# mmdagent/distantspeechrecognition-mirror

Measured on AMD Instinct MI355X. Metric: decoded_audio_hours_per_sec, higher is better.
Workload: dtype f32

## Files before the change

distantspeechrecognition-mirror_amd/csrc/decode_plan.h:

```cpp
#pragma once
#include <algorithm>
#include <cmath>
#include <cstddef>
#include <cstdlib>
#include <cstring>

namespace dsr {

struct VitEnv {
  int slots = 0;
  bool noFast = false;
  int seg = 125;
  double segSaveGB = 16.0;
  int segAny = 0;
  int segDrop = 0;
  bool segVerbose = false;
  bool pen = false;
  bool prof = false;
  bool noHash = false;
  bool noCnt = false;
  bool tableWide = false;
};

inline VitEnv read_vit_env()
{
  VitEnv e; const char* v;
  if ((v = getenv("DSR_VITERBI_SLOTS"))) e.slots = atoi(v);
  e.noFast = getenv("DSR_VITERBI_NOFAST") != nullptr;
  if ((v = getenv("DSR_VITERBI_SEG"))) e.seg = atoi(v);
  if ((v = getenv("DSR_VITERBI_SEG_SAVE_GB"))) e.segSaveGB = atof(v);
  if ((v = getenv("DSR_VITERBI_SEG_ANY"))) e.segAny = atoi(v) == 2 ? 2 : 1;
  if ((v = getenv("DSR_VITERBI_SEG_DROP"))) e.segDrop = (int) strtol(v, nullptr, 0);
  e.segVerbose = getenv("DSR_VITERBI_SEG_VERBOSE") != nullptr;
  e.pen = getenv("DSR_VITERBI_PEN") != nullptr;
  e.prof = getenv("DSR_VITERBI_PROF") != nullptr;
  e.noHash = getenv("DSR_VITERBI_NOHASH") != nullptr;
  e.noCnt = getenv("DSR_VITERBI_NOCNT") != nullptr;
  e.tableWide = (v = getenv("DSR_VITERBI_TABLE")) && !strcmp(v, "wide");
  return e;
}

struct PlanIn {
  int streams, maxActive; long long arenaTokens, latticeTokens; int topN; bool dumpOn;
  int nNodes, maxCnt;
  int U, Tmax, nDist;
  size_t staticLds;
};

struct DecodePlan {
  int slots, segFrames, segQueues, segCount, poolArenas; long arenaPer; int useLdsRow, hashN, cntCap, modes; size_t ldsBytes; bool narrow;
};

static constexpr size_t kPlanSideBytes = (size_t) 496 * 32;

inline int plan_base_modes(const PlanIn& in, const VitEnv& env) { return (env.prof ? 1 : 0) | ((in.latticeTokens > 0 || in.topN > 0 || in.dumpOn) ? 2 : 0); }

template <class RoundRobin> DecodePlan plan_decode(const PlanIn& in, const VitEnv& env, RoundRobin&& roundRobin)
{
  DecodePlan p;
  const int U = in.U, Tmax = in.Tmax, nDist = in.nDist;
  int slots = in.streams; if (slots > U) slots = U; if (in.dumpOn) slots = 1;
  const bool latOn = in.latticeTokens > 0;
  int segFrames = 0;
  if (!latOn && !in.dumpOn && in.topN <= 0 && U > slots) {
    segFrames = env.seg;
    if (segFrames < 0 || 2 * segFrames > Tmax + 1) segFrames = 0;
    const double saveGB = (double) U * (double) in.maxActive * 24.0 / 1e9;
    if (saveGB > env.segSaveGB) segFrames = 0;
  }
  int segQueues = 8;
  if (segFrames > 0 && !(slots >= 64 && slots % 8 == 0 && roundRobin())) { if (env.segAny) segQueues = 1; else segFrames = 0; }
  if (segFrames > 0 && env.segAny == 2) segQueues = 1;
  const long arenaPer = in.arenaTokens > 0 ? (long) in.arenaTokens : (long) 8192 * (long) (Tmax + 2);
  int poolArenas = 0;
  if (segFrames > 0) {
    const double want = (double) U * 1536.0 * (double) (Tmax + 2) / (double) arenaPer;
    poolArenas = (int) std::min<double>(std::ceil(want), (double) (0xFFFFFFF0u / (unsigned long long) arenaPer));
    if ((unsigned long long) std::max(poolArenas, slots) * (unsigned long long) arenaPer > 0xFFFFFFF0ull) segFrames = 0;
  }
  p.slots = slots; p.segFrames = segFrames; p.segQueues = segQueues; p.poolArenas = poolArenas; p.arenaPer = arenaPer;
  p.segCount = segFrames > 0 ? (Tmax + segFrames) / segFrames : 1;
  int modes = plan_base_modes(in, env);
  const size_t eoffB = kPlanSideBytes; const size_t ldsCap = (size_t) 160 * 1024 - in.staticLds;
  const int hashMax = 16384;
  int useLds = (size_t) nDist * sizeof(float) <= 64 * 1024;
  if (useLds && (size_t) ((nDist + 3) & ~3) * sizeof(float) + (size_t) hashMax * 8 + eoffB > ldsCap) useLds = 0;
  const size_t rowB = useLds ? (size_t) ((nDist + 3) & ~3) * sizeof(float) : 16;
  int hashN = hashMax; while (hashN > 0 && rowB + (size_t) hashN * 8 + eoffB > ldsCap) hashN >>= 1;
  if (env.noHash) hashN = 0;
  int cntCap = (hashN > 0 && in.maxCnt < 65536 && rowB + (size_t) hashN * 8 + eoffB + 4096 <= ldsCap) ? 2048 : 0;
  if (env.noCnt) cntCap = 0;
  p.ldsBytes = rowB + (size_t) hashN * 8 + eoffB + 2 * (size_t) cntCap;
  p.narrow = in.nNodes <= 65535 && hashN == hashMax && !env.tableWide;
  if (p.narrow) modes |= 4;
  p.useLdsRow = useLds; p.hashN = hashN; p.cntCap = cntCap; p.modes = modes;
  return p;
}

}
```

distantspeechrecognition-mirror_amd/csrc/decoder.cpp:

```cpp
#include "common.h"
#include "wfst_graph.h"
#include "lattice.h"
#include "lexicon.h"
#include "wordtrace.h"
#include "viterbi.h"
#include "decode_plan.h"
#include <algorithm>
#include <cmath>

namespace dsr {

static_assert(kPlanSideBytes == (size_t) kSideLds * sizeof(Side), "decode_plan.h budgets the side records of viterbi.h");

struct DecoderState {
  dsr_decoder_cfg cfg; bool haveGraph = false; int nSlots = 0; int nNodes = 0;
  WfstGraph::Csr csr; WfstGraph::Tables tab;
  DevBuf<int> d_xoff, d_xarc, d_xpathOff, d_eoff, d_path, d_nodeFinal, d_queue; DevBuf<float> d_pathCost;
  DevBuf<XRec> d_xrec; DevBuf<ERec> d_erec; DevBuf<float> d_arcCost, d_nodeCost; DevBuf<uint32_t> d_arcOut, d_arcIn;
  DevBuf<TokA> d_tokA, d_ctok; DevBuf<TokB> d_tokB; DevBuf<Side> d_side; DevBuf<XRecD> d_xrecD; DevBuf<XRecC> d_xrecC; double recLmScale = 0.0;  int fastOK = 0; int maxCnt = 0; DevBuf<int> d_tokOff, d_tokCnt, d_owner, d_rank, d_chead; DevBuf<unsigned> d_tags; DevBuf<CandA> d_cA; DevBuf<CandB> d_cB; DevBuf<unsigned> d_first; DevBuf<Bp> d_arena;
  DevBuf<long long> d_prof; DevBuf<dsr_decode_result> d_res; DevBuf<int> d_arcs; DevBuf<unsigned> d_words;
  long arenaCap = 0; int initial = 0; unsigned tokenMemoryLimit = 0;
  long lastPoolCap = 0;
  hipEvent_t evTrace = nullptr;
  DevBuf<TraceHead> d_heads; DevBuf<int> d_hopRec, d_hopOff;
  DevBuf<SegState> d_segState; DevBuf<int> d_segDone; DevBuf<unsigned long long> d_poolNext; DevBuf<TokA> d_saveA; DevBuf<TokB> d_saveB;
  DevBuf<WTok> w_tok; DevBuf<WCand> w_cand; DevBuf<int> w_tokOff, w_rank; DevBuf<unsigned long long> w_best; DevBuf<unsigned> w_first; DevBuf<int4> w_traces; size_t w_tablesFor = 0;
  bool costNegZero = false; double costMinAbs = HUGE_VAL;
  DevBuf<uint4> d_lat; DevBuf<double> d_latTtl; DevBuf<long> d_latFrameOff; DevBuf<int> d_arenaLat; DevBuf<int4> d_latFinal; DevBuf<int> d_latInfo;
  int latU = 0, latTmax = 0; long latArenaCap = 0; WfstGraph graphCopy; DevBuf<TokA> d_tokA3; DevBuf<TokB> d_tokB3;
  const dsr_lexicon* lexIn = nullptr; const dsr_lexicon* lexOut = nullptr; uint32_t eosX = 0; std::string eosSymbol;
  int lastU = 0; size_t lastMaxPath = 0; bool lastPaths = false;
  PinBuf<dsr_decode_result> h_res; PinBuf<int> h_arcs; PinBuf<unsigned> h_words; hipEvent_t evDone = nullptr;
  int pendingU = 0; size_t pendingPath = 0; int pendingSlots = 0; long long* pendingProf = nullptr;
  int dumpOn = 0; long dumpCap = 0; DevBuf<long> d_dumpFrameOff, d_dumpCount; DevBuf<int> d_dumpNode, d_dumpArc; DevBuf<float> d_dumpAc, d_dumpLm;
  std::vector<int64_t> h_dumpFrameOff; std::vector<int32_t> h_dumpNode, h_dumpArc; std::vector<float> h_dumpAc, h_dumpLm; int64_t h_dumpFrames = 0;
};

}

using namespace dsr;
struct dsr_decoder : DecoderState {};

extern "C" {

void dsr_decoder_default_cfg(dsr_decoder_cfg* c)
{ memset(c, 0, sizeof(*c)); c->beam = 100.0; c->lmScale = 12.0; c->lmPenalty = 0.0; c->silPenalty = 0.0; c->silenceX = 0xFFFFFFFFu;
  c->propagateN = 5; c->wordTraceLattice = 1; }

dsr_status dsr_decoder_create(const dsr_decoder_cfg* cfg, dsr_decoder** out)
{
  return guard([&] {
    if (!cfg || !out) throw Error(DSR_E_PARAMETER, "null argument");
    require_device();
    dsr_decoder* d = new dsr_decoder(); d->cfg = *cfg;
    if (d->cfg.maxActive <= 0) d->cfg.maxActive = 65536;
    if (d->cfg.maxCandidates <= 0) d->cfg.maxCandidates = 8 * d->cfg.maxActive;
    if (d->cfg.maxCandidates >= (1 << 24)) throw Error(DSR_E_PARAMETER, "maxCandidates must be < 2^24");
    if (d->cfg.streams <= 0) {
      hipDeviceProp_t prop; int dev = 0; DSR_HIP(hipGetDevice(&dev)); DSR_HIP(hipGetDeviceProperties(&prop, dev));
      d->cfg.streams = prop.multiProcessorCount;
      const int t = read_vit_env().slots; if (t > 0) d->cfg.streams = t;
    }
    *out = d;
  });
}
namespace {
std::mutex g_traceMu; std::map<int, std::pair<const dsr_decoder*, hipEvent_t>> g_lastTrace; std::map<int, int> g_cuCount;
void order_behind_last_traceback(int slots, hipStream_t st)
{
  std::lock_guard<std::mutex> lock(g_traceMu);
  int dev = 0; DSR_HIP(hipGetDevice(&dev));
  auto cu = g_cuCount.find(dev);
  if (cu == g_cuCount.end()) { int n = 0; DSR_HIP(hipDeviceGetAttribute(&n, hipDeviceAttributeMultiprocessorCount, dev)); cu = g_cuCount.emplace(dev, n).first; }
  if (slots < cu->second) return;
  const auto it = g_lastTrace.find(dev);
  if (it != g_lastTrace.end()) DSR_HIP(hipStreamWaitEvent(st, it->second.second, 0));
}
void publish_traceback(dsr_decoder* d, hipStream_t st)
{
  std::lock_guard<std::mutex> lock(g_traceMu);
  if (!d->evTrace) DSR_HIP(hipEventCreateWithFlags(&d->evTrace, hipEventDisableTiming));
  DSR_HIP(hipEventRecord(d->evTrace, st));
  int dev = 0; DSR_HIP(hipGetDevice(&dev));
  g_lastTrace[dev] = std::make_pair((const dsr_decoder*) d, d->evTrace);
}
void forget_traceback(const dsr_decoder* d)
{
  std::lock_guard<std::mutex> lock(g_traceMu);
  for (auto it = g_lastTrace.begin(); it != g_lastTrace.end(); ) { if (it->second.first == d) it = g_lastTrace.erase(it); else ++it; }
}
}

void dsr_decoder_destroy(dsr_decoder* d)
{
  if (!d) return;
  forget_traceback(d);
  if (d->evDone) (void) hipEventDestroy(d->evDone);
  if (d->evTrace) (void) hipEventDestroy(d->evTrace);
  delete d;
}

dsr_status dsr_decoder_set(dsr_decoder* d, const dsr_wfst* g)
{
  return guard([&] {
    if (!d || !g) throw Error(DSR_E_PARAMETER, "null argument");
    if (g->initial < 0) throw Error(DSR_E_CONSISTENCY, "the transducer has no arcs");
    d->csr = g->csr(); d->tab = g->tables(d->csr, (size_t) 1 << 28);
    d->nNodes = (int) g->nodes.size(); d->initial = g->initial; d->graphCopy = *g;
    std::vector<int> nf(d->nNodes); std::vector<float> nc(d->nNodes);
    for (int i = 0; i < d->nNodes; i++) { nf[i] = g->nodes[i].final_; nc[i] = g->nodes[i].cost; }
    d->d_xoff.upload(d->tab.xoff); d->d_eoff.upload(d->tab.eoff); d->d_path.upload(d->tab.path);
    if (d->tab.xrec.empty()) throw Error(DSR_E_CONSISTENCY, "the transducer has no emitting arcs");
    d->d_xrec.upload(d->tab.xrec); d->d_xarc.upload(d->tab.xarc); d->d_xpathOff.upload(d->tab.xpathOff);
    {
      const size_t nx = d->tab.xrec.size(); std::vector<XRecD> xd(nx); std::vector<XRecC> xc(nx); int maxCnt = 0; std::vector<float> pc(1, 0.0f);
      const double lmS = d->cfg.lmScale; d->recLmScale = lmS;
      for (size_t r = 0; r < nx; r++) {
        const XRec& x = d->tab.xrec[r]; XRecD& o = xd[r]; XRecC& oc = xc[r];
        o.dst = x.dst; o.dist = x.dist; o.lmCost = lmS * (double) x.cost; o.meta = x.meta;
        oc.dst = x.dst; oc.dstXoff = d->tab.xoff[x.dst]; oc.dstCnt = d->tab.xoff[x.dst + 1] - d->tab.xoff[x.dst]; oc.pad = 0;
        const int po = d->tab.xpathOff[r], plen = (int) (x.meta & 0xFFFFu); o.p2 = 0; float eps1 = 0.0f;
        if (x.meta >> 18) throw Error(DSR_E_CONSISTENCY, "expansion record %zu: meta bits above 17 are in use", r);
        if (plen) { const int a0 = d->tab.path[po]; eps1 = d->csr.cost[a0]; if (d->csr.out[a0] != 0) o.meta |= 0x20000u; }
        o.lmEps1 = lmS * (double) eps1;
        if (plen > 14) o.meta |= 0x80000000u;
        else if (plen > 1) {
          if (plen == 2) { const float c1 = d->csr.cost[d->tab.path[po + 1]]; memcpy(&o.p2, &c1, 4); }
          else { o.p2 = (int) pc.size(); for (int h = 1; h < plen; h++) pc.push_back(d->csr.cost[d->tab.path[po + h]]); }
          for (int h = 1; h < plen; h++) if (d->csr.out[d->tab.path[po + h]] != 0) o.meta |= 1u << (17 + h);
        }
        if (oc.dstCnt > maxCnt) maxCnt = oc.dstCnt;
      }
      d->d_xrecD.upload(xd); d->d_xrecC.upload(xc); d->d_pathCost.upload(pc);
      d->fastOK = (maxCnt < (1 << 19) && nx < ((size_t) 1 << 27)) ? 1 : 0; d->maxCnt = maxCnt;
      if (read_vit_env().noFast) d->fastOK = 0;
    }
    { std::vector<ERec> e = d->tab.erec; if (e.empty()) e.push_back(ERec{0, 0, 0, 0}); d->d_erec.upload(e); }
    d->d_arcCost.upload(d->csr.cost); d->d_arcOut.upload(d->csr.out); d->d_arcIn.upload(d->csr.in);
    d->costNegZero = false; d->costMinAbs = HUGE_VAL;
    for (size_t a = 0; a < d->csr.cost.size(); a++) {
      const float c = d->csr.cost[a]; uint32_t bits; memcpy(&bits, &c, 4);
      if (bits == 0x80000000u) d->costNegZero = true;
      if (c != 0.0f && std::fabs((double) c) < d->costMinAbs) d->costMinAbs = std::fabs((double) c);
    }
    d->d_nodeFinal.upload(nf); d->d_nodeCost.upload(nc);
    d->haveGraph = true; d->nSlots = 0;
  });
}
dsr_status dsr_decoder_set_symbols(dsr_decoder* d, const dsr_wfst* g, const char* silSymbol, const char* eosSymbol)
{
  return guard([&] {
    if (!d || !g) throw Error(DSR_E_PARAMETER, "null argument");
    uint32_t silX = d->cfg.silenceX, eosX = 0;
    if (silSymbol) { if (!g->lexIn) throw Error(DSR_E_KEY, "the transducer has no input lexicon to look '%s' up in", silSymbol); silX = g->lexIn->index(silSymbol); }
    if (eosSymbol) { if (!g->lexOut) throw Error(DSR_E_KEY, "the transducer has no output lexicon to look '%s' up in", eosSymbol); eosX = g->lexOut->index(eosSymbol); }
    const dsr_status s = dsr_decoder_set(d, g);
    if (s != DSR_OK) throw Error(s, "%s", dsr_last_error());
    d->cfg.silenceX = silX; d->eosX = eosX; d->lexIn = g->lexIn; d->lexOut = g->lexOut; d->eosSymbol = eosSymbol ? eosSymbol : "";
  });
}
uint32_t dsr_decoder_eos_index(const dsr_decoder* d) { return d ? d->eosX : 0; }

static void need_last(const dsr_decoder* d, int u, bool paths)
{
  if (!d) throw Error(DSR_E_PARAMETER, "null argument");
  if (d->lastU <= 0) throw Error(DSR_E_CONSISTENCY, "no decode has been collected yet");
  if (u < 0 || u >= d->lastU) throw Error(DSR_E_INDEX, "utterance %d of %d", u, d->lastU);
  if (paths && !d->lastPaths) throw Error(DSR_E_CONSISTENCY, "the last decode was collected without its paths");
  if (d->h_res.p[u].status != DSR_OK) throw Error(d->h_res.p[u].status, "utterance %d was not decoded (status %d)", u, d->h_res.p[u].status);
}
static std::vector<uint32_t> path_ids(const dsr_decoder* d, int u, int which)
{
  need_last(d, u, true);
  const dsr_decode_result& r = d->h_res.p[u];
  const int n = r.nArcs < (int) d->lastMaxPath ? r.nArcs : (int) d->lastMaxPath;
  const int* arcs = d->h_arcs.p + (size_t) u * d->lastMaxPath;
  std::vector<uint32_t> ids;
  if (which == 1) {
    uint32_t lastX = 0;
    for (int i = n - 1; i >= 0; i--) { const uint32_t inX = d->csr.in[arcs[i]]; if (inX != 0 && inX != lastX) { ids.push_back(inX); lastX = inX; } }
    std::reverse(ids.begin(), ids.end());
  } else for (int i = 0; i < n; i++) { const uint32_t v = which == 0 ? d->csr.out[arcs[i]] : d->csr.in[arcs[i]]; if (v != 0) ids.push_back(v); }
  return ids;
}
dsr_status dsr_decoder_path_ids(const dsr_decoder* d, int u, int which, uint32_t* ids, int cap, int* n)
{
  return guard([&] {
    if (!n || which < 0 || which > 2) throw Error(DSR_E_PARAMETER, "bad argument");
    const std::vector<uint32_t> v = path_ids(d, u, which);
    *n = (int) v.size();
    if (ids) { if ((int) v.size() > cap) throw Error(DSR_E_DIMENSION, "buffer holds %d ids, the path has %zu", cap, v.size()); if (!v.empty()) memcpy(ids, v.data(), 4 * v.size()); }
  });
}
static void put_string(const std::string& s, char* buf, size_t cap, size_t* need)
{
  if (need) *need = s.size() + 1;
  if (buf) { if (s.size() + 1 > cap) throw Error(DSR_E_DIMENSION, "buffer holds %zu bytes, the string needs %zu", cap, s.size() + 1); memcpy(buf, s.c_str(), s.size() + 1); }
}
dsr_status dsr_decoder_best_hypo(const dsr_decoder* d, int u, int useInputSymbols, char* buf, size_t cap, size_t* need)
{
  return guard([&] {
    const std::vector<uint32_t> v = path_ids(d, u, useInputSymbols ? 1 : 0);
    const dsr_lexicon* lex = useInputSymbols ? d->lexIn : d->lexOut;
    if (!lex) throw Error(DSR_E_KEY, "the transducer set on this decoder has no %s lexicon", useInputSymbols ? "input" : "output");
    std::string s; for (size_t i = 0; i < v.size(); i++) { s += lex->symbol(v[i]); s += " "; }
    put_string(s, buf, cap, need);
  });
}
dsr_status dsr_decoder_best_path(const dsr_decoder* d, int u, char* buf, size_t cap, size_t* need, int* count)
{
  return guard([&] {
    const std::vector<uint32_t> v = path_ids(d, u, 2);
    if (!d->lexIn) throw Error(DSR_E_KEY, "the transducer set on this decoder has no input lexicon");
    std::string s; for (size_t i = 0; i < v.size(); i++) { s += d->lexIn->symbol(v[i]); s += "\n"; }
    if (count) *count = (int) v.size();
    put_string(s, buf, cap, need);
  });
}
dsr_status dsr_decoder_final_states_n(const dsr_decoder* d, int u, int* n)
{ return guard([&] { if (!n) throw Error(DSR_E_PARAMETER, "null argument"); need_last(d, u, false); *n = d->h_res.p[u].finalStatesN; }); }
dsr_status dsr_decoder_trace_back_succeeded(const dsr_decoder* d, int u, int* ok)
{ return guard([&] { if (!ok) throw Error(DSR_E_PARAMETER, "null argument"); need_last(d, u, false); *ok = d->h_res.p[u].reachedFinal; }); }

dsr_status dsr_decoder_set_token_memory_limit(dsr_decoder* d, unsigned limit)
{ return guard([&] { if (!d) throw Error(DSR_E_PARAMETER, "null argument"); d->tokenMemoryLimit = limit; }); }
unsigned dsr_decoder_token_memory_limit(const dsr_decoder* d) { return d ? d->tokenMemoryLimit : 0u; }

dsr_status dsr_decoder_set_beam(dsr_decoder* d, double beam) { return guard([&] { if (!d) throw Error(DSR_E_PARAMETER, "null argument"); d->cfg.beam = beam; }); }

dsr_status dsr_decoder_enable_dump(dsr_decoder* d, int en) { return guard([&] { if (!d) throw Error(DSR_E_PARAMETER, "null argument"); d->dumpOn = en; }); }

static bool xcd_round_robin(hipStream_t st)
{
  static std::mutex mu; static std::map<int, bool> known;
  std::lock_guard<std::mutex> lock(mu);
  int dev = 0; DSR_HIP(hipGetDevice(&dev));
  const auto it = known.find(dev); if (it != known.end()) return it->second;
  DevBuf<int> o; o.reserve(64); int h[64];
  xcc_probe_launch(o.p, st);
  DSR_HIP(hipMemcpyAsync(h, o.p, sizeof(h), hipMemcpyDeviceToHost, st)); DSR_HIP(hipStreamSynchronize(st));
  bool ok = true; unsigned seen = 0;
  for (int i = 0; i < 64; i++) { if (h[i] < 0 || h[i] > 7 || h[i] != h[i & 7]) ok = false; }
  for (int i = 0; i < 8 && ok; i++) seen |= 1u << h[i];
  return known[dev] = ok && seen == 0xFFu;
}

static void ensure_scratch(dsr_decoder* d, int slots, int Tmax, int arenas)
{
  const dsr_decoder_cfg& c = d->cfg;
  long arena = c.arenaTokens > 0 ? (long) c.arenaTokens : (long) 8192 * (long) (Tmax + 2);
  if (arena > 0x7FFFFFF0L) arena = 0x7FFFFFF0L;
  if (slots <= d->nSlots && arena <= d->arenaCap && (size_t) (arenas > slots ? arenas : slots) * (size_t) d->arenaCap <= d->d_arena.n) return;
  if (slots < d->nSlots) slots = d->nSlots;
  if (arena < d->arenaCap) arena = d->arenaCap;
  const size_t S = (size_t) slots;
  d->d_tokA.reserve(S * 2 * c.maxActive); d->d_tokB.reserve(S * 2 * c.maxActive); d->d_ctok.reserve(S * 8192); d->d_side.reserve(S * kFastC);
  d->d_tokOff.reserve(S * (c.maxActive + 1));
  d->d_owner.reserve(S * c.maxCandidates); d->d_rank.reserve(S * c.maxCandidates);
  d->d_cA.reserve(S * c.maxCandidates); d->d_cB.reserve(S * c.maxCandidates);
  d->d_first.reserve(S * d->nNodes); d->d_tokCnt.reserve(S * (c.maxActive + 1)); d->d_chead.reserve(S * c.maxCandidates);
  d->d_tags.reserve(S); DSR_HIP(hipMemset(d->d_tags.p, 0, S * sizeof(unsigned)));
  d->d_arena.reserve((size_t) (arenas > slots ? arenas : slots) * (size_t) arena);
  d->d_queue.reserve(8);
  d->nSlots = slots; d->arenaCap = arena;
}

static void check_arc_inputs(const dsr_decoder* d, int nDist)
{ for (size_t a = 0; a < d->csr.in.size(); a++) if (d->csr.in[a] > (uint32_t) nDist) throw Error(DSR_E_INDEX, "arc input %u has no distribution (nDist=%d)", d->csr.in[a], nDist); }

static void enqueue_result_copies(dsr_decoder* d, int U, size_t nPath, hipStream_t st)
{
  d->h_res.reserve(U); d->h_arcs.reserve(nPath ? nPath : 1); d->h_words.reserve(nPath ? nPath : 1);
  DSR_HIP(hipMemcpyAsync(d->h_res.p, d->d_res.p, sizeof(dsr_decode_result) * U, hipMemcpyDeviceToHost, st));
  if (nPath) DSR_HIP(hipMemcpyAsync(d->h_arcs.p, d->d_arcs.p, sizeof(int) * nPath, hipMemcpyDeviceToHost, st));
  if (nPath) DSR_HIP(hipMemcpyAsync(d->h_words.p, d->d_words.p, sizeof(unsigned) * nPath, hipMemcpyDeviceToHost, st));
  if (!d->evDone) DSR_HIP(hipEventCreateWithFlags(&d->evDone, hipEventDisableTiming));
  DSR_HIP(hipEventRecord(d->evDone, st));
  d->pendingU = U; d->pendingPath = nPath;
}

static void launch_wordtrace(dsr_decoder* d, const float* score, const int32_t* nframes, int U, int Tmax, int nDist, int maxPath, int want_paths, hipStream_t st)
{
  if (d->cfg.wordTraceLattice) throw Error(DSR_E_CONSISTENCY, "DecoderWordTrace with generateLattice: not built (the shipped _placeOnList dereferences the null word trace of "
                                           "every token that has not crossed a word boundary, decoder.cc:239); construct it with generateLattice = false");
  if (d->cfg.topN > 0 || d->cfg.latticeTokens > 0 || d->dumpOn) throw Error(DSR_E_PARAMETER, "DecoderWordTrace: no topN (its frame loop has no such branch, decoder.cc:147-183), lattice bookkeeping or dump");
  check_arc_inputs(d, nDist);
  int slots = d->cfg.streams; if (slots > U) slots = U;
  const dsr_decoder_cfg& c = d->cfg; const size_t S = (size_t) slots;
  const long maxTraces = c.wordTraces > 0 ? (long) c.wordTraces : (long) 1 << 20;
  d->w_tok.reserve(S * 2 * c.maxActive); d->w_cand.reserve(S * c.maxCandidates); d->w_tokOff.reserve(S * (c.maxActive + 1)); d->w_rank.reserve(S * c.maxCandidates);
  d->w_traces.reserve((size_t) U * maxTraces); d->d_queue.reserve(8); d->d_res.reserve(U);
  if (d->w_tablesFor != S * d->nNodes) {
    d->w_best.reserve(S * d->nNodes); d->w_first.reserve(S * d->nNodes); d->w_tablesFor = S * d->nNodes;
    DSR_HIP(hipMemsetAsync(d->w_best.p, 0xFF, sizeof(unsigned long long) * S * d->nNodes, st)); DSR_HIP(hipMemsetAsync(d->w_first.p, 0xFF, sizeof(unsigned) * S * d->nNodes, st));
  }
  if (maxPath < 1) maxPath = 1;
  d->d_arcs.reserve((size_t) U * maxPath); d->d_words.reserve((size_t) U * maxPath);
  DSR_HIP(hipMemsetAsync(d->d_queue.p, 0, 8 * sizeof(int), st));
  WtArgs A; A.nNodes = d->nNodes; A.initial = d->initial; A.xoff = d->d_xoff.p; A.xrec = d->d_xrec.p; A.xarc = d->d_xarc.p; A.xpathOff = d->d_xpathOff.p; A.eoff = d->d_eoff.p;
  A.erec = d->d_erec.p; A.path = d->d_path.p; A.arcCost = d->d_arcCost.p; A.arcOut = d->d_arcOut.p; A.arcIn = d->d_arcIn.p; A.nodeFinal = d->d_nodeFinal.p; A.nodeCost = d->d_nodeCost.p;
  A.beam = c.beam; A.lmScale = c.lmScale; A.lmPenalty = c.lmPenalty; A.silPenalty = c.silPenalty; A.silenceX = c.silenceX; A.insertSilence = c.insertSilence;
  A.maxTok = c.maxActive; A.maxCand = c.maxCandidates; A.maxTraces = maxTraces;
  A.tok = d->w_tok.p; A.cand = d->w_cand.p; A.tokOff = d->w_tokOff.p; A.rank = d->w_rank.p; A.bestKey = d->w_best.p; A.firstSlot = d->w_first.p; A.traces = d->w_traces.p; A.queue = d->d_queue.p;
  A.scores = score; A.nframes = nframes; A.U = U; A.Tmax = Tmax; A.nDist = nDist; A.res = d->d_res.p; A.arcsOut = d->d_arcs.p; A.wordsOut = d->d_words.p; A.maxPath = maxPath;
  wordtrace_launch(A, slots, st);
  enqueue_result_copies(d, U, want_paths ? (size_t) U * maxPath : 0, st);
  d->pendingSlots = slots; d->pendingProf = nullptr; d->latU = 0;
}

static VitArgs fill_vit_args(dsr_decoder* d, const DecodePlan& P, const VitEnv& env, const float* score, const int32_t* nframes, int U, int Tmax, int nDist,
                             int maxPath, bool wantPaths, hipStream_t st)
{
  const int slots = P.slots; const bool latOn = d->cfg.latticeTokens > 0;
  d->d_res.reserve(U);
  if (wantPaths) { d->d_arcs.reserve((size_t) U * (maxPath > 0 ? maxPath : 1)); d->d_words.reserve((size_t) U * (maxPath > 0 ? maxPath : 1)); }
  DSR_HIP(hipMemsetAsync(d->d_queue.p, 0, 8 * sizeof(int), st));
  d->d_heads.reserve(U); DSR_HIP(hipMemsetAsync(d->d_heads.p, 0xFF, sizeof(TraceHead) * (size_t) U, st));
  if (d->dumpOn) {
    d->dumpCap = (long) d->cfg.maxActive * 64 < (long) 1 << 26 ? (long) 1 << 24 : (long) 1 << 26;
    d->d_dumpFrameOff.reserve(Tmax + 2); d->d_dumpCount.reserve(2);
    d->d_dumpNode.reserve(d->dumpCap); d->d_dumpArc.reserve(d->dumpCap); d->d_dumpAc.reserve(d->dumpCap); d->d_dumpLm.reserve(d->dumpCap);
    DSR_HIP(hipMemsetAsync(d->d_dumpCount.p, 0, 2 * sizeof(long), st));
  }
  VitArgs A; GraphDev& G = A.G; DecDev& D = A.D;
  G.nNodes = d->nNodes; G.initial = d->initial; G.xoff = d->d_xoff.p; G.xrec = d->d_xrec.p; G.xrecD = d->d_xrecD.p; G.xrecC = d->d_xrecC.p; G.xarc = d->d_xarc.p;
  G.xpathOff = d->d_xpathOff.p; G.eoff = d->d_eoff.p; G.erec = d->d_erec.p; G.path = d->d_path.p; G.pathCost = d->d_pathCost.p; G.arcCost = d->d_arcCost.p;
  G.arcOut = d->d_arcOut.p; G.arcIn = d->d_arcIn.p; G.nodeFinal = d->d_nodeFinal.p; G.nodeCost = d->d_nodeCost.p;
  if (memcmp(&d->recLmScale, &d->cfg.lmScale, sizeof(double)) != 0) throw Error(DSR_E_CONSISTENCY, "lmScale changed after the transducer was set");
  D.beam = d->cfg.beam; D.lmScale = d->cfg.lmScale; D.lmPenalty = d->cfg.lmPenalty; D.silPenalty = d->cfg.silPenalty;
  D.noPen = (d->cfg.lmScale > 0.0 && std::isfinite(d->cfg.lmScale) && d->cfg.lmScale * d->cfg.lmPenalty == 0.0 && d->cfg.lmScale * d->cfg.silPenalty == 0.0 &&
             !d->costNegZero && (d->costMinAbs == HUGE_VAL || d->cfg.lmScale * d->costMinAbs >= 0x1p-60) && !env.pen) ? 1 : 0;
  D.silenceX = d->cfg.silenceX; D.maxTok = d->cfg.maxActive; D.maxCand = d->cfg.maxCandidates; D.arenaCap = d->arenaCap;
  D.tokA = d->d_tokA.p; D.tokB = d->d_tokB.p; D.ctok = d->d_ctok.p; D.side = d->d_side.p; D.fastOK = d->fastOK; D.tokOff = d->d_tokOff.p; D.owner = d->d_owner.p; D.rank = d->d_rank.p; D.cA = d->d_cA.p; D.cB = d->d_cB.p;
  D.first = d->d_first.p; D.tags = d->d_tags.p; D.tokCnt = d->d_tokCnt.p; D.chead = d->d_chead.p; D.arena = d->d_arena.p; D.queue = d->d_queue.p;
  D.segDrop = env.segDrop; D.segQueues = P.segQueues; D.segFrames = P.segFrames; D.segCount = P.segCount;
  D.poolCap = 0; D.poolChunk = 0; D.poolNext = nullptr; D.segState = nullptr; D.segDone = nullptr; D.saveA = nullptr; D.saveB = nullptr;
  if (P.segFrames > 0) {
    d->d_segState.reserve(U); d->d_segDone.reserve(U); d->d_poolNext.reserve(1);
    d->d_saveA.reserve((size_t) U * d->cfg.maxActive); d->d_saveB.reserve((size_t) U * d->cfg.maxActive);
    DSR_HIP(hipMemsetAsync(d->d_segDone.p, 0, sizeof(int) * (size_t) U, st)); DSR_HIP(hipMemsetAsync(d->d_poolNext.p, 0, sizeof(unsigned long long), st));
    D.poolCap = (long) ((size_t) std::max(P.poolArenas, slots) * (size_t) d->arenaCap); if (D.poolCap > (long) 0xFFFFFFF0L) D.poolCap = (long) 0xFFFFFFF0L;
    D.poolChunk = std::min<long>(262144, std::max<long>(4096, D.poolCap / (4 * (long) U)));
    D.poolNext = d->d_poolNext.p; D.segState = d->d_segState.p; D.segDone = d->d_segDone.p; D.saveA = d->d_saveA.p; D.saveB = d->d_saveB.p;
  }
  d->lastPoolCap = D.poolCap;
  D.prof = nullptr;
  if (env.prof) { d->d_prof.reserve((size_t) slots * kProfN); D.prof = d->d_prof.p; }
  D.dumpOn = d->dumpOn; D.dumpCap = d->dumpCap; D.dumpFrameOff = d->d_dumpFrameOff.p; D.dumpNode = d->d_dumpNode.p; D.dumpAc = d->d_dumpAc.p;
  D.dumpLm = d->d_dumpLm.p; D.dumpArc = d->d_dumpArc.p; D.dumpCount = d->d_dumpCount.p;
  D.topN = d->cfg.topN > 0 ? d->cfg.topN : 0; D.tokA3 = nullptr; D.tokB3 = nullptr;
  if (D.topN > 0) { d->d_tokA3.reserve((size_t) slots * d->cfg.maxActive); d->d_tokB3.reserve((size_t) slots * d->cfg.maxActive); D.tokA3 = d->d_tokA3.p; D.tokB3 = d->d_tokB3.p; }
  D.latOn = latOn ? 1 : 0; D.latCap = 0; D.lat = nullptr; D.latTtl = nullptr; D.latFrameOff = nullptr; D.arenaLat = nullptr; D.latFinal = nullptr; D.latInfo = nullptr;
  if (latOn) {
    const size_t cap = (size_t) d->cfg.latticeTokens;
    d->d_lat.reserve((size_t) U * cap); d->d_latTtl.reserve((size_t) U * cap); d->d_latFrameOff.reserve((size_t) U * (Tmax + 3));
    d->d_arenaLat.reserve((size_t) U * (size_t) d->arenaCap); d->d_latFinal.reserve((size_t) U * d->cfg.maxActive); d->d_latInfo.reserve((size_t) 4 * U);
    DSR_HIP(hipMemsetAsync(d->d_latInfo.p, 0, sizeof(int) * 4 * (size_t) U, st));
    D.latCap = (long) cap; D.lat = d->d_lat.p; D.latTtl = d->d_latTtl.p; D.latFrameOff = d->d_latFrameOff.p; D.arenaLat = d->d_arenaLat.p; D.latFinal = d->d_latFinal.p; D.latInfo = d->d_latInfo.p;
    d->latU = U; d->latTmax = Tmax; d->latArenaCap = d->arenaCap;
  } else d->latU = 0;
  A.scores = score; A.nframesArr = nframes; A.U = U; A.Tmax = Tmax; A.nDist = nDist; A.res = d->d_res.p;
  A.arcsOut = wantPaths ? d->d_arcs.p : nullptr; A.wordsOut = wantPaths ? d->d_words.p : nullptr; A.maxPath = maxPath;
  A.useLdsRow = P.useLdsRow; A.hashN = P.hashN; A.regionB = (int) (kSideLds * sizeof(Side)); A.cntCap = P.cntCap;
  A.heads = d->d_heads.p;
  A.hopStride = std::max(1, std::min(2 * D.maxCand, Tmax + 2));
  d->d_hopRec.reserve((size_t) U * A.hopStride); d->d_hopOff.reserve((size_t) U * A.hopStride); A.hopRec = d->d_hopRec.p;
  A.oneEach = (P.segFrames == 0 && slots == U) ? 1 : 0;
  A.walkHere = (P.segFrames == 0 && !latOn && !A.oneEach) ? 1 : 0;
  return A;
}

static TraceArgs fill_trace_args(dsr_decoder* d, const VitArgs& V)
{
  TraceArgs A; A.hopCap = 2 * V.D.maxCand; A.hopStride = V.hopStride;
  A.heads = V.heads; A.arena = V.D.arena; A.arenaN = (unsigned long long) d->d_arena.n;
  A.xrec = V.G.xrec; A.erec = V.G.erec; A.xarc = V.G.xarc; A.xpathOff = V.G.xpathOff; A.path = V.G.path; A.arcOut = V.G.arcOut;
  A.hopRec = d->d_hopRec.p; A.hopOff = d->d_hopOff.p;
  A.res = V.res; A.arcsOut = V.arcsOut; A.wordsOut = V.wordsOut; A.maxPath = V.maxPath; A.U = V.U;
  return A;
}

dsr_status dsr_decoder_decode_launch(dsr_decoder* d, const float* score, const int32_t* nframes, int U, int Tmax, int nDist,
                                     int maxPath, int want_paths, void* stream)
{
  return guard([&] {
    if (!d || !score || !nframes) throw Error(DSR_E_PARAMETER, "null argument");
    if (!d->haveGraph) throw Error(DSR_E_INITIALIZATION, "call set() with a transducer first");
    if (d->pendingU > 0) throw Error(DSR_E_CONSISTENCY, "a decode is already in flight on this decoder: collect it first");
    if (U <= 0) return;
    hipStream_t st = (hipStream_t) stream;
    if (d->cfg.wordTrace) { launch_wordtrace(d, score, nframes, U, Tmax, nDist, maxPath, want_paths, st); return; }
    check_arc_inputs(d, nDist);
    const bool latOn = d->cfg.latticeTokens > 0;
    if (latOn && d->dumpOn) throw Error(DSR_E_PARAMETER, "lattice bookkeeping and the token dump are separate debugging aids: enable one");
    const VitEnv env = read_vit_env();
    PlanIn in; in.streams = d->cfg.streams; in.maxActive = d->cfg.maxActive; in.arenaTokens = d->cfg.arenaTokens; in.latticeTokens = d->cfg.latticeTokens;
    in.topN = d->cfg.topN; in.dumpOn = d->dumpOn != 0; in.nNodes = d->nNodes; in.maxCnt = d->maxCnt; in.U = U; in.Tmax = Tmax; in.nDist = nDist;
    in.staticLds = viterbi_static_lds(plan_base_modes(in, env));
    const DecodePlan P = plan_decode(in, env, [&] { return xcd_round_robin(st); });
    ensure_scratch(d, P.slots, Tmax, latOn ? U : (P.segFrames > 0 ? P.poolArenas : 0));
    if (maxPath < 0) maxPath = 0;
    const VitArgs A = fill_vit_args(d, P, env, score, nframes, U, Tmax, nDist, maxPath, want_paths != 0, st);
    if (env.segVerbose) fprintf(stderr, "[dsr viterbi] %d utterances on %d workgroups: %s, %s state table\n", U, P.slots, P.segFrames > 0 ? (P.segQueues == 8 ? "time-sliced, XCD-bound queues" : "time-sliced, one queue") : "run to completion", P.narrow ? "narrow" : "wide");
    const TraceArgs TA = fill_trace_args(d, A);
    order_behind_last_traceback(P.slots, st);
    viterbi_launch(P.modes, A, P.slots, P.ldsBytes, st);
    traceback_launch(TA, st);
    publish_traceback(d, st);
    enqueue_result_copies(d, U, want_paths ? (size_t) U * maxPath : 0, st);
    d->pendingSlots = P.slots; d->pendingProf = A.D.prof;
  });
}

static void report_profile(const long long* prof, int slots)
{
  std::vector<long long> hp((size_t) slots * kProfN); DSR_HIP(hipMemcpy(hp.data(), prof, hp.size() * sizeof(long long), hipMemcpyDeviceToHost));
  double acc[32] = {0}; for (int s2 = 0; s2 < slots; s2++) for (int i = 0; i < 32; i++) acc[i] += (double) hp[(size_t) s2 * kProfN + i];
  fprintf(stderr, "[dsr viterbi prof] mean us per slot:");
  for (int i = 0; i < 32; i++) if (i != 15) fprintf(stderr, " p%d=%.0f", i, acc[i] / slots / 100.0);
  fprintf(stderr, "\n");
  double tmin = 1e30, tmax = 0.0, tsum = 0.0;
  for (int s2 = 0; s2 < slots; s2++) { double t = 0.0; for (int i = 0; i < 32; i++) if (i != 15) t += (double) hp[(size_t) s2 * kProfN + i]; t /= 100.0; tsum += t; if (t < tmin) tmin = t; if (t > tmax) tmax = t; }
  {
    double h[12] = {0}; for (int s2 = 0; s2 < slots; s2++) for (int i = 0; i < 12; i++) h[i] += (double) hp[(size_t) s2 * kProfN + 32 + i];
    const double nf = h[0] + h[1] + h[2] + h[3], tk = h[4] + h[5] + h[6] + h[7];
    static const char* const cn[4] = {"<=8192", "<=12288", ">12288", "memory path"};
    for (int c = 0; c < 4; c++) if (h[c] > 0) fprintf(stderr, "[dsr viterbi prof] frames with %s placements: %.1f %% of the frames, %.1f %% of the frame time, %.1f us per frame, %.2f ns per placement\n",
                                                      cn[c], 100.0 * h[c] / nf, 100.0 * h[4 + c] / tk, h[4 + c] / 100.0 / h[c], h[4 + c] * 10.0 / h[8 + c]);
  }
  {
    double a = 0, b = 0; for (int s2 = 0; s2 < slots; s2++) { a += (double) hp[(size_t) s2 * kProfN + 44]; b += (double) hp[(size_t) s2 * kProfN + 45]; }
    if (a + b > 0) fprintf(stderr, "[dsr viterbi prof] register-path frames: %.1f %% start laid out, %.1f %% run P1/P2\n", 100.0 * a / (a + b), 100.0 * b / (a + b));
    double m1 = 0, m2 = 0, mAll = 0; for (int s2 = 0; s2 < slots; s2++) { m1 += (double) hp[(size_t) s2 * kProfN + 46]; m2 += (double) hp[(size_t) s2 * kProfN + 47]; mAll += (double) hp[(size_t) s2 * kProfN + 32 + 3]; }
    if (mAll > 0) fprintf(stderr, "[dsr viterbi prof] memory-path frames: %.0f, of them %.1f %% with at most 28672 placements, %.1f %% with at most 32767\n", mAll, 100.0 * m1 / mAll, 100.0 * m2 / mAll);
  }
  {
    double h[6] = {0}; for (int s2 = 0; s2 < slots; s2++) for (int i = 0; i < 6; i++) h[i] += (double) hp[(size_t) s2 * kProfN + 48 + i];
    if (h[0] > 0) fprintf(stderr, "[dsr viterbi prof] hops behind the first: %.0f wave-placements, %.1f %% with a path of two or more hops, %.1f %% load hop costs, %.1f %% run the hop loop; "
                                  "%.3f hop iterations per wave-placement for %.3f hops per lane (x 64: %.2f)\n",
                          h[0], 100.0 * h[1] / h[0], 100.0 * h[2] / h[0], 100.0 * h[3] / h[0], h[4] / h[0], h[5] / h[0] / 64.0, h[5] / h[0]);
  }
  fprintf(stderr, "[dsr viterbi prof] busy us per slot: mean %.0f min %.0f max %.0f\n", tsum / slots, tmin, tmax);
  if (slots >= 64 && slots % 8 == 0) {
    double bx[8] = {0}; for (int s2 = 0; s2 < slots; s2++) { double t = 0.0; for (int i = 0; i < 32; i++) if (i != 15) t += (double) hp[(size_t) s2 * kProfN + i]; bx[s2 & 7] += t / 100.0; }
    fprintf(stderr, "[dsr viterbi prof] busy us per slot, by XCD:"); for (int q = 0; q < 8; q++) fprintf(stderr, " %.0f", bx[q] / (slots / 8)); fprintf(stderr, "\n");
  }
}

dsr_status dsr_decoder_decode_collect(dsr_decoder* d, dsr_decode_result* res, int32_t* arcs_out, uint32_t* words_out)
{
  return guard([&] {
    if (!d || !res) throw Error(DSR_E_PARAMETER, "null argument");
    if (d->pendingU <= 0) throw Error(DSR_E_CONSISTENCY, "no decode in flight");
    const int U = d->pendingU; const size_t nPath = d->pendingPath; const int slots = d->pendingSlots; long long* prof = d->pendingProf;
    d->pendingU = 0; d->lastU = U; d->lastPaths = nPath > 0; d->lastMaxPath = nPath > 0 ? nPath / (size_t) U : 0;
    DSR_HIP(hipEventSynchronize(d->evDone));
    memcpy(res, d->h_res.p, sizeof(dsr_decode_result) * U);
    if (arcs_out && nPath) memcpy(arcs_out, d->h_arcs.p, sizeof(int) * nPath);
    if (words_out && nPath) memcpy(words_out, d->h_words.p, sizeof(unsigned) * nPath);
    if (read_vit_env().segVerbose && d->d_poolNext.p && d->lastPoolCap > 0) {
      unsigned long long used = 0; DSR_HIP(hipMemcpy(&used, d->d_poolNext.p, sizeof(used), hipMemcpyDeviceToHost));
      fprintf(stderr, "[dsr viterbi] pool of back-pointer records: %.1f M of %.1f M taken\n", used / 1e6, d->lastPoolCap / 1e6);
    }
    if (read_vit_env().segVerbose) {
      long long laid = 0, reg = 0, all = 0;
      for (int u = 0; u < U; u++) if (res[u].status == DSR_OK || res[u].status == DSR_E_DIMENSION) { laid += res[u].laidOutFrames_; reg += res[u].registerFrames; all += res[u].frames + 1; }
      fprintf(stderr, "[dsr viterbi] frames: %lld laid out by the frame before, %lld through P1/P2, %lld on the memory path\n", laid, reg - laid, all - reg);
    }
    if (prof) report_profile(prof, slots);
    if (d->dumpOn) {
      long cnt[2]; DSR_HIP(hipMemcpy(cnt, d->d_dumpCount.p, sizeof(cnt), hipMemcpyDeviceToHost));
      const long N = cnt[0] < d->dumpCap ? cnt[0] : d->dumpCap; d->h_dumpFrames = cnt[1];
      std::vector<long> fo(cnt[1] + 1); if (cnt[1] > 0) DSR_HIP(hipMemcpy(fo.data(), d->d_dumpFrameOff.p, sizeof(long) * (cnt[1] + 1), hipMemcpyDeviceToHost));
      d->h_dumpFrameOff.assign(fo.begin(), fo.end());
      d->h_dumpNode.resize(N); d->h_dumpArc.resize(N); d->h_dumpAc.resize(N); d->h_dumpLm.resize(N);
      if (N > 0) {
        DSR_HIP(hipMemcpy(d->h_dumpNode.data(), d->d_dumpNode.p, sizeof(int) * N, hipMemcpyDeviceToHost));
        DSR_HIP(hipMemcpy(d->h_dumpArc.data(), d->d_dumpArc.p, sizeof(int) * N, hipMemcpyDeviceToHost));
        DSR_HIP(hipMemcpy(d->h_dumpAc.data(), d->d_dumpAc.p, sizeof(float) * N, hipMemcpyDeviceToHost));
        DSR_HIP(hipMemcpy(d->h_dumpLm.data(), d->d_dumpLm.p, sizeof(float) * N, hipMemcpyDeviceToHost));
      }
    }
  });
}

dsr_status dsr_decoder_decode_batch(dsr_decoder* d, const float* score, const int32_t* nframes, int U, int Tmax, int nDist,
                                    dsr_decode_result* res, int32_t* arcs_out, uint32_t* words_out, int maxPath, void* stream)
{
  if (!res) return guard([&] { throw Error(DSR_E_PARAMETER, "null argument"); });
  if (U <= 0) return DSR_OK;
  const dsr_status s1 = dsr_decoder_decode_launch(d, score, nframes, U, Tmax, nDist, maxPath, (arcs_out || words_out) ? 1 : 0, stream);
  if (s1 != DSR_OK) return s1;
  return dsr_decoder_decode_collect(d, res, arcs_out, words_out);
}

namespace {
struct LatHost {
  std::vector<long> frameOff; std::vector<dsr::LatPlace> place; std::vector<double> ttl; std::vector<dsr::LatBp> arena; std::vector<int> arenaLat; std::vector<dsr::LatFinalTok> fin;
  dsr::LatInput in;
};
void load_lat(dsr_decoder* d, int u, uint32_t eosX, LatHost& H)
{
  if (d->latU <= 0) throw Error(DSR_E_CONSISTENCY, "Must enable lattice generation during decoding.");
  if (d->pendingU > 0) throw Error(DSR_E_CONSISTENCY, "a decode is in flight: collect it first");
  if (u < 0 || u >= d->latU) throw Error(DSR_E_INDEX, "utterance %d of %d", u, d->latU);
  int info[4]; DSR_HIP(hipMemcpy(info, d->d_latInfo.p + 4 * (size_t) u, sizeof(info), hipMemcpyDeviceToHost));
  const int finN = info[0], haveNext = info[1], T = info[3]; const long arenaN = info[2];
  if (T <= 0) throw Error(DSR_E_CONSISTENCY, "utterance %d was not decoded to its end (status of its decode result)", u);
  H.frameOff.assign((size_t) T + 2, 0);
  DSR_HIP(hipMemcpy(H.frameOff.data(), d->d_latFrameOff.p + (size_t) u * (d->latTmax + 3), sizeof(long) * ((size_t) T + 2), hipMemcpyDeviceToHost));
  const long nP = H.frameOff[(size_t) T + 1];
  H.place.resize((size_t) (nP > 0 ? nP : 1)); H.ttl.resize((size_t) (nP > 0 ? nP : 1));
  H.arena.resize((size_t) (arenaN > 0 ? arenaN : 1)); H.arenaLat.resize((size_t) (arenaN > 0 ? arenaN : 1)); H.fin.resize((size_t) (finN > 0 ? finN : 1));
  const size_t cap = (size_t) d->cfg.latticeTokens;
  if (nP > 0) { DSR_HIP(hipMemcpy(H.place.data(), d->d_lat.p + (size_t) u * cap, sizeof(LatPlace) * (size_t) nP, hipMemcpyDeviceToHost));
                DSR_HIP(hipMemcpy(H.ttl.data(), d->d_latTtl.p + (size_t) u * cap, sizeof(double) * (size_t) nP, hipMemcpyDeviceToHost)); }
  if (arenaN > 0) { DSR_HIP(hipMemcpy(H.arena.data(), d->d_arena.p + (size_t) u * (size_t) d->latArenaCap, sizeof(LatBp) * (size_t) arenaN, hipMemcpyDeviceToHost));
                    DSR_HIP(hipMemcpy(H.arenaLat.data(), d->d_arenaLat.p + (size_t) u * (size_t) d->latArenaCap, sizeof(int) * (size_t) arenaN, hipMemcpyDeviceToHost)); }
  if (finN > 0) DSR_HIP(hipMemcpy(H.fin.data(), d->d_latFinal.p + (size_t) u * d->cfg.maxActive, sizeof(LatFinalTok) * (size_t) finN, hipMemcpyDeviceToHost));
  LatInput& in = H.in; in.graph = &d->graphCopy; in.csr = &d->csr; in.tab = &d->tab; in.lmScale = d->cfg.lmScale; in.lmPenalty = d->cfg.lmPenalty; in.silPenalty = d->cfg.silPenalty;
  in.silenceX = d->cfg.silenceX; in.eosX = eosX; in.T = T; in.place = H.place.data(); in.ttl = H.ttl.data(); in.frameOff = H.frameOff.data();
  in.arena = H.arena.data(); in.arenaLat = H.arenaLat.data(); in.arenaN = arenaN; in.fin = H.fin.data(); in.finN = finN; in.haveNext = haveNext;
}
}

dsr_status dsr_decoder_lattice(dsr_decoder* d, int u, uint32_t eosX, dsr_lattice** out)
{
  return guard([&] {
    if (!d || !out) throw Error(DSR_E_PARAMETER, "null argument");
    LatHost H; load_lat(d, u, eosX, H);
    dsr_lattice* L = new dsr_lattice();
    try { build_lattice(H.in, *L); } catch (...) { delete L; throw; }
    *out = L;
  });
}

dsr_status dsr_decoder_write_gmm(dsr_decoder* d, int u, const char* conv, const char* channel, const char* spk, const char* utt, double cfrom, double score,
                                 const char* fileName, double frameInterval)
{
  return guard([&] {
    (void) spk;
    if (!d || !conv || !channel || !utt) throw Error(DSR_E_PARAMETER, "null argument");
    if (!d->lexIn) throw Error(DSR_E_KEY, "the transducer set on this decoder has no input lexicon");
    LatHost H; load_lat(d, u, 0u, H);
    std::vector<GmmRow> rows;
    if (!best_path_gmm(H.in, rows)) throw Error(DSR_E_CONSISTENCY, "no best token");
    FILE* fp = (!fileName || !*fileName) ? stdout : fopen(fileName, "a");
    if (!fp) throw Error(DSR_E_IO, "could not open %s", fileName);
    fprintf(fp, "# %s %10.4f %10.4f\n", utt, cfrom, score);
    for (int i = (int) rows.size() - 1; i >= 0; i--) {
      if (rows[i].inX >= d->lexIn->syms.size()) { if (fp != stdout) fclose(fp); throw Error(DSR_E_INDEX, "input symbol %u is not in the lexicon", rows[i].inX); }
      const std::string& lab = d->lexIn->symbol(rows[i].inX); const char* label = lab.c_str();
      if (lab == d->eosSymbol) continue;
      const double beg = cfrom + rows[i].startX * frameInterval, len = (rows[i].endX - rows[i].startX + 1) * frameInterval;
      fprintf(fp, "%s %s %7.2f %7.2f %-20s %7.2f\n", conv, channel, beg, len, label, rows[i].score);
    }
    if (fp != stdout) fclose(fp); else fflush(stdout);
  });
}
void dsr_lattice_destroy(dsr_lattice* L) { delete L; }
int dsr_lattice_num_nodes(const dsr_lattice* L) { return L ? (int) L->nodeFinal.size() : 0; }
int dsr_lattice_num_edges(const dsr_lattice* L) { return L ? (int) L->from.size() : 0; }
int dsr_lattice_final_states_n(const dsr_lattice* L) { return L ? L->finalStatesN : 0; }
dsr_status dsr_lattice_get(const dsr_lattice* L, int32_t* nodeFinal, int32_t* from, int32_t* to, uint32_t* in, uint32_t* out, int32_t* start, int32_t* end, double* ac, double* lm)
{
  return guard([&] {
    if (!L) throw Error(DSR_E_PARAMETER, "null argument");
    const size_t nE = L->from.size();
    if (nodeFinal) memcpy(nodeFinal, L->nodeFinal.data(), 4 * L->nodeFinal.size());
    if (from && nE) memcpy(from, L->from.data(), 4 * nE); if (to && nE) memcpy(to, L->to.data(), 4 * nE);
    if (in && nE) memcpy(in, L->in.data(), 4 * nE); if (out && nE) memcpy(out, L->out.data(), 4 * nE);
    if (start && nE) memcpy(start, L->start.data(), 4 * nE); if (end && nE) memcpy(end, L->end.data(), 4 * nE);
    if (ac && nE) memcpy(ac, L->ac.data(), 8 * nE); if (lm && nE) memcpy(lm, L->lm.data(), 8 * nE);
  });
}
dsr_status dsr_lattice_write(dsr_lattice* L, const char* fileName, int writeData)
{ return guard([&] { if (!L || !fileName) throw Error(DSR_E_PARAMETER, "null argument"); L->write(fileName, writeData != 0); }); }
size_t dsr_lattice_pack_size(const dsr_lattice* L) { return L ? 16 + 4 * L->nodeFinal.size() + 40 * L->from.size() : 0; }
dsr_status dsr_lattice_pack(const dsr_lattice* L, void* buf, size_t bufBytes)
{
  return guard([&] {
    if (!L || !buf) throw Error(DSR_E_PARAMETER, "null argument");
    const std::vector<unsigned char> b = L->pack();
    if (b.size() > bufBytes) throw Error(DSR_E_DIMENSION, "buffer holds %zu bytes, the lattice needs %zu", bufBytes, b.size());
    memcpy(buf, b.data(), b.size());
  });
}
dsr_status dsr_lattice_unpack(const void* buf, size_t bytes, dsr_lattice** out)
{
  return guard([&] {
    if (!buf || !out) throw Error(DSR_E_PARAMETER, "null argument");
    dsr_lattice* L = new dsr_lattice();
    try { static_cast<LatticeData&>(*L) = LatticeData::unpack((const unsigned char*) buf, bytes); } catch (...) { delete L; throw; }
    *out = L;
  });
}

dsr_status dsr_decoder_get_dump(dsr_decoder* d, int64_t* nFrames, const int64_t** frameOff, const int32_t** node,
                                const float** ac, const float** lm, const int32_t** arc)
{
  return guard([&] {
    if (!d) throw Error(DSR_E_PARAMETER, "null argument");
    if (nFrames) *nFrames = d->h_dumpFrames;
    if (frameOff) *frameOff = d->h_dumpFrameOff.data();
    if (node) *node = d->h_dumpNode.data(); if (arc) *arc = d->h_dumpArc.data();
    if (ac) *ac = d->h_dumpAc.data(); if (lm) *lm = d->h_dumpLm.data();
  });
}

}
```

distantspeechrecognition-mirror_amd/csrc/k_viterbi.hip:

```cpp
#include "launch.h"
#include "viterbi.h"
#include <algorithm>
#include <cmath>
#include <type_traits>

namespace dsr {

static constexpr uint32_t kNone = 0xFFFFFFFFu;
static constexpr uint32_t kEndBit = 0x80000000u;
static constexpr int kWaves = kThreads / 64;
static constexpr int kFastK = 8;
static constexpr int kB = 2;
static constexpr int kFastE = 8190;
static constexpr int kP1 = 16;
static constexpr int kW = 4;

typedef const __attribute__((address_space(4))) VitArgs* KP;

__device__ __forceinline__ unsigned ld_u32(const unsigned* p) { return __hip_atomic_load(p, __ATOMIC_RELAXED, __HIP_MEMORY_SCOPE_AGENT); }
__device__ __forceinline__ int ld_i32(const int* p) { return __hip_atomic_load(p, __ATOMIC_RELAXED, __HIP_MEMORY_SCOPE_AGENT); }
__device__ __forceinline__ void st_u32(unsigned* p, unsigned v) { __hip_atomic_store(p, v, __ATOMIC_RELAXED, __HIP_MEMORY_SCOPE_AGENT); }
__device__ __forceinline__ void st_i32(int* p, int v) { __hip_atomic_store(p, v, __ATOMIC_RELAXED, __HIP_MEMORY_SCOPE_AGENT); }
__device__ __forceinline__ void st_u64_dev(void* p, unsigned long long v) { __hip_atomic_store(reinterpret_cast<unsigned long long*>(p), v, __ATOMIC_RELAXED, __HIP_MEMORY_SCOPE_AGENT); }
__device__ __forceinline__ unsigned long long ld_u64_dev(const void* p) { return __hip_atomic_load(reinterpret_cast<const unsigned long long*>(p), __ATOMIC_RELAXED, __HIP_MEMORY_SCOPE_AGENT); }

__device__ __forceinline__ int wave_incl_scan(int v, int )
{
  v += __builtin_amdgcn_update_dpp(0, v, 0x111, 0xF, 0xF, true);
  v += __builtin_amdgcn_update_dpp(0, v, 0x112, 0xF, 0xF, true);
  v += __builtin_amdgcn_update_dpp(0, v, 0x114, 0xF, 0xF, true);
  v += __builtin_amdgcn_update_dpp(0, v, 0x118, 0xF, 0xF, true);
  v += __builtin_amdgcn_update_dpp(0, v, 0x142, 0xA, 0xF, false);
  v += __builtin_amdgcn_update_dpp(0, v, 0x143, 0xC, 0xF, false);
  return v;
}
__device__ __forceinline__ float wave_max_f_uni(float v)
{
#define DSR_DPP_F(ctrl, rm) { const float o = __int_as_float(__builtin_amdgcn_update_dpp(__float_as_int(v), __float_as_int(v), ctrl, rm, 0xF, false)); v = fmaxf(v, o); }
  DSR_DPP_F(0x111, 0xF) DSR_DPP_F(0x112, 0xF) DSR_DPP_F(0x114, 0xF) DSR_DPP_F(0x118, 0xF) DSR_DPP_F(0x142, 0xA) DSR_DPP_F(0x143, 0xC)
#undef DSR_DPP_F
  return __int_as_float(__builtin_amdgcn_readlane(__float_as_int(v), 63));
}
__device__ __forceinline__ double wave_min_d_uni(double v)
{
#define DSR_DPP_D(ctrl, rm) { const int lo = __double2loint(v), hi = __double2hiint(v); \
    const double o = __hiloint2double(__builtin_amdgcn_update_dpp(hi, hi, ctrl, rm, 0xF, false), __builtin_amdgcn_update_dpp(lo, lo, ctrl, rm, 0xF, false)); v = (o < v) ? o : v; }
  DSR_DPP_D(0x111, 0xF) DSR_DPP_D(0x112, 0xF) DSR_DPP_D(0x114, 0xF) DSR_DPP_D(0x118, 0xF) DSR_DPP_D(0x142, 0xA) DSR_DPP_D(0x143, 0xC)
#undef DSR_DPP_D
  return __hiloint2double(__builtin_amdgcn_readlane(__double2hiint(v), 63), __builtin_amdgcn_readlane(__double2loint(v), 63));
}
__device__ __forceinline__ double wave_min_d(double v)
{
#pragma unroll
  for (int d = 32; d >= 1; d >>= 1) { const double o = __shfl_xor(v, d, 64); v = (o < v) ? o : v; }
  return v;
}
__device__ __forceinline__ unsigned long long wave_min_u64(unsigned long long v)
{
#pragma unroll
  for (int d = 32; d >= 1; d >>= 1) { const unsigned long long o = __shfl_xor(v, d, 64); v = (o < v) ? o : v; }
  return v;
}
__device__ __forceinline__ float wave_max_f(float v)
{
#pragma unroll
  for (int d = 32; d >= 1; d >>= 1) v = fmaxf(v, __shfl_xor(v, d, 64));
  return v;
}
__device__ __forceinline__ void clear_result(dsr_decode_result* r)
{
  int z = 0; asm volatile("" : "+v"(z));
  int* p = reinterpret_cast<int*>(r);
#pragma unroll 1
  for (int i = 0; i < (int) (sizeof(dsr_decode_result) / 4); i++) p[i] = z;
}
typedef __attribute__((address_space(3))) float lds_float_t;
typedef __attribute__((address_space(3))) Side lds_side_t;
#define DSR_NO_MERGE() asm volatile("" ::: "memory")
__device__ __forceinline__ TokA ld_tok(const TokA* p)
{
  const unsigned long long a = reinterpret_cast<const volatile unsigned long long*>(p)[0], b = reinterpret_cast<const volatile unsigned long long*>(p)[1];
  TokA t; t.ac = __uint_as_float((unsigned) (a & 0xFFFFFFFFull)); t.lm = __uint_as_float((unsigned) (a >> 32)); t.bp = (uint32_t) (b & 0xFFFFFFFFull); t.xs = (uint32_t) (b >> 32);
  return t;
}
__device__ __forceinline__ void side_winner(const Side* sideL, const Side* side, int sideLds, int idx, float& ac, float& lm, int& rec)
{
  if (idx < sideLds) {
    const lds_side_t* p = (const lds_side_t*) sideL + idx;
    const unsigned long long a = *reinterpret_cast<const volatile __attribute__((address_space(3))) unsigned long long*>(&p->ac);
    rec = *reinterpret_cast<const volatile __attribute__((address_space(3))) int*>(&p->rec);
    ac = __uint_as_float((unsigned) (a & 0xFFFFFFFFull)); lm = __uint_as_float((unsigned) (a >> 32));
    DSR_NO_MERGE();
  } else {
    const Side* p = side + idx;
    const unsigned long long a = *reinterpret_cast<const volatile unsigned long long*>(&p->ac); rec = *reinterpret_cast<const volatile int*>(&p->rec);
    ac = __uint_as_float((unsigned) (a & 0xFFFFFFFFull)); lm = __uint_as_float((unsigned) (a >> 32));
  }
}
__device__ __forceinline__ void side_link(const Side* sideL, const Side* side, int sideLds, int idx, int& c, double& ttl, unsigned& next)
{
  if (idx < sideLds) { const lds_side_t* p = (const lds_side_t*) sideL + idx; c = p->c; ttl = p->ttl; next = p->next; DSR_NO_MERGE(); }
  else { const Side* p = side + idx; c = p->c; ttl = p->ttl; next = p->next; }
}
__device__ __forceinline__ float side_score(const Side* sideL, const Side* side, int sideLds, int idx)
{
  float r;
  if (idx < sideLds) { const lds_side_t* p = (const lds_side_t*) sideL + idx; r = __fadd_rn(p->ac, p->lm); DSR_NO_MERGE(); }
  else { const Side* p = side + idx; r = __fadd_rn(p->ac, p->lm); }
  return r;
}
template <class T> __device__ __forceinline__ const T* at32(const void* base, uint32_t byteOff) { return reinterpret_cast<const T*>(reinterpret_cast<const char*>(base) + byteOff); }
template <class T> __device__ __forceinline__ T* at32w(void* base, uint32_t byteOff) { return reinterpret_cast<T*>(reinterpret_cast<char*>(base) + byteOff); }
__device__ __forceinline__ int uni(int v) { return __builtin_amdgcn_readfirstlane(v); }
__device__ __forceinline__ double uni(double v) { return __hiloint2double(__builtin_amdgcn_readfirstlane(__double2hiint(v)), __builtin_amdgcn_readfirstlane(__double2loint(v))); }
__device__ __forceinline__ unsigned f2ord(float f) { const unsigned u = __float_as_uint(f); return (u & 0x80000000u) ? ~u : (u | 0x80000000u); }

template <int MODES>
__global__ __launch_bounds__(kThreads) void k_viterbi(const VitArgs argsInKernarg)
{
  (void) argsInKernarg;
  constexpr bool PROF = (MODES & 1) != 0, EXTRA = (MODES & 2) != 0;
  constexpr bool NARROW = (MODES & 4) != 0;
  const KP KA = (KP) __builtin_amdgcn_kernarg_segment_ptr();
  KP ka = KA;
#define RELOAD() do { ka = KA; asm volatile("" : "+s"(ka)); } while (0)
  RELOAD();
  extern __shared__ __attribute__((aligned(16))) unsigned char smem[];
  float* srow = reinterpret_cast<float*>(smem);
  const int useLdsRow = ka->useLdsRow, nDist = ka->nDist, hashN = ka->hashN, regionB = ka->regionB, cntCap = ka->cntCap;
  unsigned* hkey = reinterpret_cast<unsigned*>(srow + (useLdsRow ? ((nDist + 3) & ~3) : 4));
  unsigned* hfirst = hkey + hashN;
  unsigned* const tab = hkey; const int tabN = NARROW ? 2 * hashN : hashN;
  Side* sideL = reinterpret_cast<Side*>(hfirst + hashN);
  unsigned short* cntL = reinterpret_cast<unsigned short*>(reinterpret_cast<unsigned char*>(hfirst + hashN) + regionB);
  __shared__ int s_waveTot[kWaves];
  __shared__ int s_waveTotE[kWaves];
  __shared__ double s_waveMin[kWaves];
  __shared__ float s_waveMag[kWaves];
  __shared__ unsigned long long s_waveKey[kWaves];
  __shared__ int s_sideN;
  __shared__ unsigned s_bm[kFastC / 32];
  __shared__ unsigned s_gbase[kFastC / 64 + 4];
  __shared__ int s_cnt[(kFastK + 32) * kWaves];
  __shared__ int s_err;
  __shared__ long long s_prof[32]; __shared__ long long s_tlast;
  __shared__ long long s_hist[PROF ? 16 : 1]; __shared__ long long s_tfr;
  __shared__ unsigned long long s_hop[PROF ? 8 : 1];
  __shared__ long long s_stat[3];
  __shared__ int s_maxActive; __shared__ unsigned s_tag; __shared__ long long s_latOff;
  if (PROF && threadIdx.x < 32) s_prof[threadIdx.x] = 0;
  if (PROF && threadIdx.x < 16) s_hist[threadIdx.x] = 0;
  if (PROF && threadIdx.x < 8) s_hop[threadIdx.x] = 0ull;
#define TICK(ix) do { if (PROF && tid == 0) { const long long tn = (long long) wall_clock64(); s_prof[ix] += tn - s_tlast; s_tlast = tn; } } while (0)
  constexpr int nthr = kThreads, nw = kWaves;
  __shared__ int s_u, s_seg, s_help; __shared__ long long s_chunk;

  const int tid = threadIdx.x;
  const int slot = blockIdx.x;
#define TOKA(ix) ((EXTRA && (ix) == 2) ? ka->D.tokA3 + (size_t) slot * ka->D.maxTok : ka->D.tokA + ((size_t) slot * 2 + (size_t) (ix)) * ka->D.maxTok)
#define TOKB(ix) ((EXTRA && (ix) == 2) ? ka->D.tokB3 + (size_t) slot * ka->D.maxTok : ka->D.tokB + ((size_t) slot * 2 + (size_t) (ix)) * ka->D.maxTok)
#define curA TOKA(bufCur)
#define nxtA TOKA(bufNxt)
#define curB TOKB(bufCur)
#define nxtB TOKB(bufNxt)
#define sprA TOKA(bufSpr)
#define sprB TOKB(bufSpr)
#define ctok (ka->D.ctok + (size_t) slot * 8192)
#define side (ka->D.side + (size_t) slot * kFastC)
#define cA (ka->D.cA + (size_t) slot * ka->D.maxCand)
#define cB (ka->D.cB + (size_t) slot * ka->D.maxCand)
  if (tid == 0) s_tag = ka->D.tags[slot];
#define arena (ka->D.arena + (size_t) ((EXTRA && ka->D.latOn) ? u : (ka->D.segFrames > 0 ? 0 : slot)) * ka->D.arenaCap)
#define sc (ka->scores + (size_t) u * ka->Tmax * nDist)
  constexpr int fastCapC = ((kFastK + 32) * nthr < kFastC) ? (kFastK + 32) * nthr : kFastC;
  constexpr int fastCapN = kP1 * 64 * nw;
  const bool fastOK = ka->D.fastOK && hashN >= 8192;
  const int tableC = (tabN >> 1) + (tabN >> 2), regC = NARROW ? tableC : 2 * tableC, eCap = kFastE, sideLds = regionB >> 5;

  const int nq = (EXTRA || ka->D.segFrames <= 0) ? 1 : ka->D.segQueues;
  const int xcd = nq == 8 ? (int) (__builtin_amdgcn_s_getreg((3 << 11) | 20) & 7u) : 0;
  if (tid == 0) { s_help = (nq == 8 && ((ka->D.segDrop >> xcd) & 1)) ? 1 : 0; s_u = -2; }
  for (;;) {
    __syncthreads();
    if (tid == 0) {
      const int segS0 = EXTRA ? 0 : ka->D.segFrames; int help = s_help, uu = -1, sg = 0;
      for (;;) {
        const int qx = (xcd + help) & (nq - 1), Uq = (ka->U - qx + nq - 1) / nq;
        int it = -1;
        if (help == 0) { it = ka->oneEach ? (s_u == -2 ? slot : Uq) : atomicAdd(ka->D.queue + qx, 1); if (it >= (segS0 > 0 ? ka->D.segCount * Uq : Uq)) it = -1; }
        else {
          int c = ld_i32(ka->D.queue + qx);
          while (c < Uq) { const int prev = atomicCAS(ka->D.queue + qx, c, c + 1); if (prev == c) { it = c; break; } c = prev; }
        }
        if (it >= 0) { uu = segS0 > 0 ? qx + nq * (it % Uq) : it; sg = segS0 > 0 ? it / Uq : 0; break; }
        if (segS0 > 0 && nq == 8 && help < 7) help++; else break;
      }
      if (uu >= 0 && help > 0) { st_i32(&ka->D.segState[uu].status, -2); asm volatile("s_waitcnt vmcnt(0)" ::: "memory"); st_i32(&ka->D.segDone[uu], 0x7FFFFFFF); sg = -1; }
      s_help = help; s_u = uu; s_seg = sg;
    }
    __syncthreads();
    RELOAD();
    const int segS = EXTRA ? 0 : ka->D.segFrames;
    const int u = s_u; if (u < 0) break;
    const bool whole = s_seg < 0; const int seg = whole ? 0 : s_seg;
    const int T = ka->nframesArr[u] < ka->Tmax ? ka->nframesArr[u] : ka->Tmax;
    const int fr0 = seg * segS, frEnd = (segS > 0 && !whole) ? fr0 + segS : 0x7FFFFFFF;
    if (fr0 > T) continue;
    if (EXTRA && ka->D.latOn && tid == 0) ka->D.latFrameOff[(size_t) u * (ka->Tmax + 3)] = 0;
    if (PROF && tid == 0) { const long long tn = (long long) wall_clock64(); if (s_prof[15]) s_prof[10] += tn - s_prof[15]; s_tlast = tn; }
#define dump (EXTRA && ka->D.dumpOn && slot == 0)

    int status = DSR_OK;
    if (T <= 0) status = DSR_E_ITERATOR;

    int bufCur = 0, bufNxt = 1, bufSpr = 2;
    int n = 1; long arenaOff = 0, chunkEnd = 0, arenaUsed = 0;
    double thresh = HUGE_VAL, topScore = HUGE_VAL;
    for (int i = tid; i < 2 * hashN; i += nthr) hkey[i] = (NARROW || i < hashN) ? 0u : 0xFFFFFFFFu;
    if (seg == 0) {
      if (tid == 0) {
        s_stat[0] = 0; s_stat[1] = 0; s_stat[2] = 0; s_maxActive = 0; s_latOff = 0;
        TokA t0; t0.ac = 0.0f; t0.lm = 0.0f; t0.bp = kNone; t0.xs = (uint32_t) ka->G.xoff[ka->G.initial]; curA[0] = t0;
        TokB b0; b0.node = ka->G.initial; b0.cnt = ka->G.xoff[ka->G.initial + 1] - ka->G.xoff[ka->G.initial]; curB[0] = b0;
      }
    } else {
      if (tid == 0) { while (ld_i32(&ka->D.segDone[u]) < seg) __builtin_amdgcn_s_sleep(16); }
      __syncthreads();
      if (nq == 1) __builtin_amdgcn_fence(__ATOMIC_ACQUIRE, "agent");
      const SegState* const sst = ka->D.segState + u;
      status = ld_i32(&sst->status);
      if (status != DSR_OK) continue;
      n = ld_i32(&sst->n); arenaOff = (long) ld_u64_dev(&sst->arenaOff); chunkEnd = (long) ld_u64_dev(&sst->chunkEnd); arenaUsed = (long) ld_u64_dev(&sst->arenaUsed); thresh = __longlong_as_double((long long) ld_u64_dev(&sst->thresh));
      if (tid == 0) { s_stat[0] = (long long) ld_u64_dev(&sst->stat[0]); s_stat[1] = (long long) ld_u64_dev(&sst->stat[1]); s_stat[2] = (long long) ld_u64_dev(&sst->stat[2]); s_maxActive = ld_i32(&sst->maxActive); s_latOff = 0; }
      const TokA* const svA = ka->D.saveA + (size_t) u * ka->D.maxTok; const TokB* const svB = ka->D.saveB + (size_t) u * ka->D.maxTok;
      for (int i = tid; i < n; i += nthr) {
        const unsigned long long a0 = ld_u64_dev(&svA[i]), a1 = ld_u64_dev(reinterpret_cast<const unsigned long long*>(&svA[i]) + 1), b0 = ld_u64_dev(&svB[i]);
        unsigned long long* da = reinterpret_cast<unsigned long long*>(&curA[i]); da[0] = a0; da[1] = a1; *reinterpret_cast<unsigned long long*>(&curB[i]) = b0;
      }
    }
    __syncthreads();

    bool cntOK = false;
    int preC = -1;
    const bool preRow = useLdsRow && nDist <= 2 * nthr;
    float rowNext[2] = {0.0f, 0.0f};
    if (preRow && fr0 < T) {
      const float* r0 = sc + (size_t) fr0 * nDist; int tidU = (int) threadIdx.x; asm volatile("" : "+v"(tidU));
      if (tidU < nDist) rowNext[0] = r0[tidU]; if (tidU + nthr < nDist) rowNext[1] = r0[tidU + nthr];
    }
    TICK(11);
    int fr = fr0;
    for (; fr <= T && fr < frEnd && status == DSR_OK; fr++) {
      RELOAD();
      int tidO = (int) threadIdx.x; asm volatile("" : "+v"(tidO));
      const int tid = tidO, lane = tid & 63, wave = tid >> 6;
      const int mode = (fr == T) ? 1 : 0;
      if (mode == 0 && useLdsRow) {
        if (preRow) {
          if (tid < nDist) srow[tid] = rowNext[0];
          if (tid + nthr < nDist) srow[tid + nthr] = rowNext[1];
          if (fr + 1 < T) {
            const float* nr = sc + (size_t) (fr + 1) * nDist;
            if (tid < nDist) rowNext[0] = nr[tid];
            if (tid + nthr < nDist) rowNext[1] = nr[tid + nthr];
          }
        } else { for (int i = tid; i < nDist; i += nthr) srow[i] = sc[(size_t) fr * nDist + i]; }
      }
      const float* rowG = sc + (size_t) fr * nDist;
      int numNew = 0, numStat = -1;
      if (fr > 0) TICK(23);
      if (PROF && tid == 0) { s_tlast = (long long) wall_clock64(); s_tfr = s_tlast; }
      bool fast = fastOK && mode == 0 && n <= fastCapN && !(EXTRA && (ka->D.latOn || ka->D.topN > 0));
      int Cfr = 0;

      if (fast) {
        const bool pre = preC >= 0;
        const int chunkT = ((n + nw * 64 - 1) / (nw * 64)) * 64;
        int C = preC, E = n;
        if (!pre) {
        float psc[kP1]; int pcn[kP1]; unsigned pk[kP1];
        int runC = 0, runE = 0;
        {
          const int b0 = wave * chunkT, b1 = (b0 + chunkT < n) ? b0 + chunkT : n;
#pragma unroll
          for (int g = 0; g < kP1; g += 8) {
            if (g * 64 < chunkT && cntOK) {
#pragma unroll
              for (int it = g; it < g + 8; it++) { int i = b0 + it * 64 + lane; i = (i < n) ? i : n - 1; pcn[it] = (int) cntL[i]; psc[it] = -HUGE_VALF; }
            } else if (g * 64 < chunkT) {
#pragma unroll
              for (int it = g; it < g + 8; it++) {
                int i = b0 + it * 64 + lane; i = (i < n) ? i : n - 1;
                const float2 a = *reinterpret_cast<const float2*>(&curA[i].ac); pcn[it] = curB[i].cnt;
                psc[it] = __fadd_rn(a.x, a.y);
              }
            } else {
#pragma unroll
              for (int it = g; it < g + 8; it++) { pcn[it] = 0; psc[it] = 0.0f; }
            }
          }
          TICK(16);
          for (int i = tid; i < kFastC / 32; i += nthr) s_bm[i] = 0u;
          TICK(17);
#pragma unroll
          for (int it = 0; it < kP1; it++) {
            const int base = b0 + it * 64; pk[it] = 0u;
            if (base < b1) {
              const int i = base + lane; int cnt = 0;
              if (i < b1) {
                if (!((double) psc[it] > thresh)) cnt = pcn[it];
              }
              pcn[it] = cnt;
              const int incl = wave_incl_scan(cnt, lane);
              const unsigned long long bal = __ballot(cnt > 0);
              if (cnt > 0) pk[it] = 0x80000000u | (unsigned) ((runC + incl - cnt) & 0x7FFF) | ((unsigned) ((runE + __popcll(bal & ((1ull << lane) - 1ull))) & 0xFFFF) << 15);
              runC += __builtin_amdgcn_readlane(incl, 63); runE += __popcll(bal);
            }
          }
          TICK(18);
          if (lane == 0) { s_waveTot[wave] = runC; s_waveTotE[wave] = runE; }
          if (tid == 0) { s_sideN = 0; s_gbase[0] = 0; s_err = 0; }
        }
        __syncthreads();
        TICK(0);
        int cbase, ebase;
        {
          const int a = (lane < nw) ? s_waveTot[lane] : 0, b = (lane < nw) ? s_waveTotE[lane] : 0;
          const int sa = wave_incl_scan(a, lane), sb = wave_incl_scan(b, lane);
          C = __builtin_amdgcn_readlane(sa, 63); E = __builtin_amdgcn_readlane(sb, 63);
          const int wu = uni(wave);
          cbase = __builtin_amdgcn_readlane(sa - a, wu); ebase = __builtin_amdgcn_readlane(sb - b, wu);
        }
        TICK(19);
        if (!(C > fastCapC || E > eCap || C > regC)) {
          RELOAD();
          const bool ident = (E == n);
#pragma unroll
          for (int it = 0; it < kP1; it++) if (pk[it] & 0x80000000u) {
            const int e = ebase + (int) ((pk[it] >> 15) & 0xFFFFu); const int off = cbase + (int) (pk[it] & 0x7FFFu);
            if (!ident) ctok[e] = curA[wave * chunkT + it * 64 + lane];
            atomicOr(&s_bm[off >> 5], 1u << (off & 31));
            for (int g = (off >> 6) + 1; g <= ((off + pcn[it]) >> 6); g++) s_gbase[g] = (unsigned) (e + 1) | ((unsigned) (64 * g - off) << 13);
          }
          __syncthreads();
        }
        } else __syncthreads();
        if (C > fastCapC || E > eCap || C > regC) { fast = false; __syncthreads(); }
        else {
          RELOAD();
          const bool ident = (E == n);
          const TokA* __restrict__ ctk = ident ? curA : ctok;
          TICK(1);
          Cfr = C;
          if (pre && tid == nthr - 1) s_stat[2] += 1ll << 32;
          if (PROF && tid == 0) s_hist[pre ? 12 : 13] += 1;
          RELOAD();
          int tq = tid; asm volatile("" : "+v"(tq)); const int lq = tq & 63, wq = tq >> 6;
          const int K = (C + nthr - 1) / nthr;
          float qac[kFastK], qlm[kFastK]; int qrec[kFastK]; unsigned ek[kFastK];
          double* const ttlS = reinterpret_cast<double*>(cA);
          uint4* const ovf = reinterpret_cast<uint4*>(cB);
          const XRecD* const xrecD = ka->G.xrecD; const float* const pathCost = ka->G.pathCost; const uint32_t silenceX = ka->D.silenceX;
          double locMin = HUGE_VAL; float locMag = 0.0f;
          const bool prevNull0 = (fr == 0);
          const double lmS = ka->D.lmScale, lsPen = __dmul_rn(ka->D.lmScale, ka->D.lmPenalty), lsSil = __dmul_rn(ka->D.lmScale, ka->D.silPenalty);
          const bool sil0 = (0u == silenceX);
#pragma unroll
          for (int k = 0; k < kFastK; k++) { qac[k] = 0.0f; qlm[k] = 0.0f; qrec[k] = 0; ek[k] = 0u; }

          const int nPass = (!NARROW && C > tableC) ? 2 : 1;
          auto table_insert = [&](const unsigned dst, const unsigned prod, const int c) __attribute__((always_inline)) -> unsigned {
            const unsigned key = dst + 1u;
            unsigned h = (prod >> 7) & (unsigned) (tabN - 1); int probes = 0;
            if (NARROW) {
              const unsigned w = (key << 15) | (unsigned) c;
              for (;;) {
                const unsigned kk = atomicCAS(&tab[h], 0u, w);
                if (kk == 0u) break;
                if ((kk >> 15) == key) { atomicMin(&tab[h], w); break; }
                h = (h + 1u) & (unsigned) (tabN - 1);
                if (++probes > tabN) { s_err = 1; break; }
              }
              return h;
            }
            for (;;) {
              const unsigned kk = atomicCAS(&hkey[h], 0u, key);
              if (kk == 0u || kk == key) break;
              h = (h + 1u) & (unsigned) (hashN - 1);
              if (++probes > hashN) { s_err = 1; break; }
            }
            atomicMin(&hfirst[h], (unsigned) c);
            return h;
          };
          constexpr unsigned ekBucket = NARROW ? 0x7FFFu : 0x3FFFu;
          auto in_pass = [&](const unsigned e, const int pass) __attribute__((always_inline)) -> bool { return NARROW || (int) ((e >> 27) & 1u) == pass; };
          auto is_first = [&](const unsigned h, const int c) __attribute__((always_inline)) -> bool { return NARROW ? (tab[h] & 0x7FFFu) == (unsigned) c : hfirst[h] == (unsigned) c; };
          auto push_side = [&](const unsigned h, const int sx) __attribute__((always_inline)) -> unsigned {
            if (NARROW) {
              unsigned old = tab[h];
              for (;;) { const unsigned prev = atomicCAS(&tab[h], old, 0x80000000u | ((unsigned) sx << 15) | (old & 0x7FFFu)); if (prev == old) break; old = prev; }
              return (old & 0x80000000u) ? (0x80000000u | ((old >> 15) & 0xFFFFu)) : 0u;
            }
            return atomicExch(&hkey[h], 0x80000000u | (unsigned) sx);
          };
          auto chain_head = [&](const unsigned h) __attribute__((always_inline)) -> unsigned {
            if (NARROW) { const unsigned w = tab[h]; return (w & 0x80000000u) ? (0x80000000u | ((w >> 15) & 0xFFFFu)) : 0u; }
            return hkey[h];
          };
          auto locate = [&](const int k, int& rec, unsigned& ekk) __attribute__((always_inline)) {
            const int c = k * nthr + tq; const int grp = k * nw + wq;
            unsigned e = 0u; int j = 0;
            if (c < C) {
              const unsigned long long W = ((unsigned long long) s_bm[2 * grp + 1] << 32) | s_bm[2 * grp];
              const unsigned gb = s_gbase[grp]; const unsigned long long mine = W & ((2ull << lq) - 1ull);
              e = (gb & 0x1FFFu) + (unsigned) __popcll(mine) - 1u;
              j = mine ? lq - (63 - __clzll((long long) mine)) : lq + (int) (gb >> 13);
            }
            ekk = e; rec = j;
          };
          auto tokload = [&](float& ac, float& lm, int& rec, unsigned& ekk) __attribute__((always_inline)) {
            const TokA t = *at32<TokA>(ctk, ekk * 16u);
            ac = t.ac; lm = t.lm; rec += (int) (t.xs & 0x7FFFFFFFu); ekk |= (t.xs >> 31) << 29;
          };
          auto expandR = [&](auto NOPEN, const int g8, float* ac8, float* lm8, int* rec8, unsigned* ek8) __attribute__((always_inline)) {
            constexpr bool NP = decltype(NOPEN)::value;
            int4 xr[kB]; double2 xl[kB];
#pragma unroll
            for (int i = 0; i < kB; i++) {
              xr[i] = *at32<int4>(xrecD, (uint32_t) rec8[i] * 32u); xl[i] = *at32<double2>(xrecD, (uint32_t) rec8[i] * 32u + 16u);
            }
            if (PROF) { asm volatile("s_waitcnt vmcnt(0)" ::: "memory"); TICK(28); }
            float hc[kB][3]; int pls[kB]; bool more[kB];
#pragma unroll
            for (int i = 0; i < kB; i++) {
              const int c = (g8 + i) * nthr + tq; const uint32_t xmeta = (uint32_t) xr[i].y;
              const int pl = (c < C) ? (int) (xmeta & 0xFFFFu) : 0;
              pls[i] = (xmeta & 0x80000000u) ? 0 : pl; more[i] = pl > 4;
              hc[i][0] = hc[i][1] = hc[i][2] = __int_as_float(xr[i].w);
              if (pls[i] > 2) {
                const uint32_t o = (uint32_t) xr[i].w * 4u;
                hc[i][0] = *at32<float>(pathCost, o); hc[i][1] = *at32<float>(pathCost, o + 4u); hc[i][2] = *at32<float>(pathCost, o + (pls[i] > 3 ? 8u : 4u));
              }
            }
            if (PROF) { asm volatile("s_waitcnt vmcnt(0)" ::: "memory"); TICK(31); }
#pragma unroll
            for (int i = 0; i < kB; i++) {
              const uint32_t xmeta = (uint32_t) xr[i].y; const bool tsil = (ek8[i] >> 29) & 1u;
              float lmNode;
              {
                double l = __dadd_rn((double) lm8[i], xl[i].y);
                if (!NP) {
                  const double l1 = __dadd_rn(l, lsPen); l = (xmeta & 0x20000u) ? l1 : l;
                  const double l2 = __dadd_rn(l, lsSil); l = (sil0 && (prevNull0 || !tsil)) ? l2 : l;
                }
                lmNode = (xmeta & 0xFFFFu) ? (float) l : lm8[i];
              }
              if (PROF) {
                unsigned long long iters = 0ull, need = 0ull; const int pl = more[i] ? (int) (xmeta & 0xFFFFu) : pls[i];
                for (int k = 1; k < 0x10000; k++) { const unsigned long long b = __ballot(pl > k); if (!b) break; if (k > 3) iters++; need += (unsigned long long) __popcll(b); }
                const unsigned long long act = __ballot((g8 + i) * nthr + tq < C); const bool loads = __ballot(pls[i] > 2) != 0ull;
                if (act && lq == __ffsll((long long) act) - 1) {
                  atomicAdd(&s_hop[0], 1ull); if (need) { atomicAdd(&s_hop[1], 1ull); atomicAdd(&s_hop[5], need); }
                  if (loads) atomicAdd(&s_hop[2], 1ull);
                  if (iters) { atomicAdd(&s_hop[3], 1ull); atomicAdd(&s_hop[4], iters); }
                }
                asm volatile("s_waitcnt vmcnt(0) lgkmcnt(0)" ::: "memory"); TICK(29);
              }
#pragma unroll
              for (int h = 1; h < 4; h++) {
                double l = __dadd_rn((double) lmNode, __dmul_rn(lmS, (double) hc[i][h - 1]));
                if (!NP) { const double l1 = __dadd_rn(l, lsPen); l = ((xmeta >> (17 + h)) & 1u) ? l1 : l; }
                lmNode = (pls[i] > h) ? (float) l : lmNode;
              }
              if (PROF) TICK(31);
              lm8[i] = lmNode;
            }
            bool anyMore = false;
#pragma unroll
            for (int i = 0; i < kB; i++) anyMore = anyMore || more[i];
            if (__any(anyMore)) {
#pragma unroll
              for (int i = 0; i < kB; i++) if (more[i]) {
                const uint32_t xmeta = (uint32_t) xr[i].y; const int plen = (int) (xmeta & 0xFFFFu), xp2 = xr[i].w;
                double lmNode = (double) lm8[i];
                if (!(xmeta & 0x80000000u)) {
                  for (int h = 4; h < plen; h++) {
                    double l = __dadd_rn(lmNode, __dmul_rn(lmS, (double) pathCost[xp2 + h - 1]));
                    if (!NP && ((xmeta >> (17 + h)) & 1u)) l = __dadd_rn(l, lsPen);
                    lmNode = (double) (float) l;
                  }
                } else {
                  const int* pp = ka->G.path + ka->G.xpathOff[rec8[i]];
                  for (int h = 1; h < plen; h++) {
                    const int a = pp[h];
                    double l = __dadd_rn(lmNode, __dmul_rn(lmS, (double) ka->G.arcCost[a]));
                    if (!NP && ka->G.arcOut[a] != 0) l = __dadd_rn(l, lsPen);
                    lmNode = (double) (float) l;
                  }
                }
                lm8[i] = (float) lmNode;
              }
            }
            if (PROF) { asm volatile("s_waitcnt vmcnt(0)" ::: "memory"); TICK(31); }
#pragma unroll
            for (int i = 0; i < kB; i++) {
              const int c = (g8 + i) * nthr + tq;
              const bool tsil = (ek8[i] >> 29) & 1u; ek8[i] &= 0x1FFFu;
              if (c < C) {
                const int xdist = xr[i].x; const uint32_t xmeta = (uint32_t) xr[i].y; const int xdst = xr[i].z;
                const bool has = (xmeta & 0xFFFFu) != 0u;
                const bool pnull = has ? false : prevNull0;
                const bool pinSil = has ? sil0 : tsil;
                double lm = __dadd_rn((double) lm8[i], xl[i].x);
                if (!NP) { const double lm1 = __dadd_rn(lm, lsPen); lm = (xmeta & 0x10000u) ? lm1 : lm; }
                const bool silArc = ((uint32_t) (xdist + 1) == silenceX);
                if (!NP) { const double lm2 = __dadd_rn(lm, lsSil); lm = (silArc && (pnull || !pinSil)) ? lm2 : lm; }
                float rowv;
                if (useLdsRow) { rowv = ((const lds_float_t*) srow)[xdist]; DSR_NO_MERGE(); } else rowv = rowG[xdist];
                const double ac = __dadd_rn((double) ac8[i], (double) rowv);
                const double ttl = __dadd_rn(ac, lm);
                *at32w<double>(ttlS, (uint32_t) c * 8u) = ttl; ac8[i] = (float) ac; lm8[i] = (float) lm; rec8[i] |= (silArc ? 0x40000000 : 0);
                if (ttl < locMin) locMin = ttl;
                locMag = fmaxf(locMag, __fadd_rn(fabsf(ac8[i]), fabsf(lm8[i])));
                if (PROF) { asm volatile("s_waitcnt vmcnt(0) lgkmcnt(0)" ::: "memory"); TICK(29); }
                const unsigned prod = (unsigned) xdst * 2654435761u;
                if (!NARROW && nPass > 1 && (prod >> 31)) ek8[i] |= 1u << 27;
                else ek8[i] |= (table_insert((unsigned) xdst, prod, c) << 13) | (1u << 28);
                if (PROF) { asm volatile("s_waitcnt lgkmcnt(0)" ::: "memory"); TICK(30); }
              }
            }
          };
          auto expand8 = [&](auto NOPEN, const int g8, float* ac8, float* lm8, int* rec8, unsigned* ek8) __attribute__((always_inline)) {
#pragma unroll
            for (int i = 0; i < kB; i++) locate(g8 + i, rec8[i], ek8[i]);
            if (PROF) { asm volatile("s_waitcnt lgkmcnt(0)" ::: "memory"); TICK(26); }
#pragma unroll
            for (int i = 0; i < kB; i++) tokload(ac8[i], lm8[i], rec8[i], ek8[i]);
            if (PROF) { asm volatile("s_waitcnt vmcnt(0)" ::: "memory"); TICK(27); }
            expandR(NOPEN, g8, ac8, lm8, rec8, ek8);
          };
          auto park_store = [&](const int kb, const float* oac, const float* olm, const int* orec, const unsigned* oek) __attribute__((always_inline)) {
#pragma unroll
            for (int i = 0; i < kB; i++) { const int c = (kb + i) * nthr + tq; if (c < C) ovf[c - kFastK * nthr] = make_uint4(__float_as_uint(oac[i]), __float_as_uint(olm[i]), (unsigned) orec[i], oek[i]); }
          };
          auto park_load = [&](const int kb, float* oac, float* olm, int* orec, unsigned* oek) __attribute__((always_inline)) {
#pragma unroll
            for (int i = 0; i < kB; i++) {
              int c = (kb + i) * nthr + tq; c = (c < C) ? c : kFastK * nthr;
              const uint4 v = ovf[c - kFastK * nthr];
              oac[i] = __uint_as_float(v.x); olm[i] = __uint_as_float(v.y); orec[i] = (int) v.z; oek[i] = v.w;
            }
          };
          auto runP3 = [&](auto NOPEN) __attribute__((always_inline)) {
#pragma unroll
            for (int g8 = 0; g8 < kFastK; g8 += kB) if (g8 < K) expand8(NOPEN, g8, &qac[g8], &qlm[g8], &qrec[g8], &ek[g8]);
            for (int kb = kFastK; kb < K; kb += kB) {
              float oac[kB], olm[kB]; int orec[kB]; unsigned oek[kB];
              expand8(NOPEN, kb, oac, olm, orec, oek); park_store(kb, oac, olm, orec, oek);
            }
          };
          if (ka->D.noPen) runP3(std::true_type{}); else runP3(std::false_type{});
          TICK(2);
          locMin = wave_min_d_uni(locMin); locMag = wave_max_f_uni(locMag);
          if (lq == 0) { s_waveMin[wq] = locMin; s_waveMag[wq] = locMag; }
          TICK(3);
          __syncthreads();
          TICK(4);
          for (int i = tq; i < kFastC / 32; i += nthr) s_bm[i] = 0u;
          topScore = HUGE_VAL;
          float frameMag;
          { const double v = (lq < nw) ? s_waveMin[lq] : HUGE_VAL; const float g = (lq < nw) ? s_waveMag[lq] : 0.0f;
            topScore = wave_min_d_uni(v); frameMag = wave_max_f_uni(g); }
          RELOAD();
          const double threshNext = __dadd_rn(topScore, ka->D.beam);
          const bool prune = !dump && (fr + 1 < T);
          const double doomT = prune ? __dadd_rn(threshNext, (double) __fmul_rn(frameMag, 4.76837158203125e-07f)) : HUGE_VAL;
          unsigned long long firstMask = 0ull;
          auto later8 = [&](const int g8, const int pass, const float* ac8, const float* lm8, const int* rec8, const unsigned* ek8) __attribute__((always_inline)) {
            double tt[kB]; uint32_t pb[kB];
#pragma unroll
            for (int i = 0; i < kB; i++) {
              int c = (g8 + i) * nthr + tq; c = (c < C) ? c : 0;
              tt[i] = ttlS[c]; pb[i] = ctk[ek8[i] & 0x1FFFu].bp;
            }
#pragma unroll
            for (int i = 0; i < kB; i++) {
              const int c = (g8 + i) * nthr + tq;
              if (c < C && (ek8[i] & (1u << 28)) && in_pass(ek8[i], pass) && !((firstMask >> (g8 + i)) & 1ull)) {
                const unsigned h = (ek8[i] >> 13) & ekBucket;
                if (is_first(h, c)) firstMask |= 1ull << (g8 + i);
                else if (!((double) __fadd_rn(ac8[i], lm8[i]) > doomT)) {
                  const int sx = atomicAdd(&s_sideN, 1);
                  const unsigned nx = push_side(h, sx);
                  Side sd; sd.ttl = tt[i]; sd.ac = ac8[i]; sd.lm = lm8[i]; sd.rec = rec8[i]; sd.prevBp = pb[i]; sd.c = c; sd.next = nx;
                  if (sx < sideLds) sideL[sx] = sd; else side[sx] = sd;
                }
              }
            }
          };
          auto fold_multi = [&](const int wslot0, const unsigned head, const float ac, const float lm) __attribute__((always_inline)) -> int {
            int wslot = wslot0, wIdx = -1; double fw = (double) __fadd_rn(ac, lm);
            for (;;) {
              int best = 0x7FFFFFFF, bi = -1, steps = 0;
              for (unsigned p = head; (p & 0x80000000u) && steps <= C; steps++) {
                const int pi = (int) (p & 0x7FFFFFFFu);
                int pc; double pt; unsigned pn;
                side_link(sideL, side, sideLds, pi, pc, pt, pn);
                if (pc > wslot && pc < best && pt < fw) { best = pc; bi = pi; }
                p = pn;
              }
              if (bi < 0) break;
              wslot = best; wIdx = bi;
              fw = (double) side_score(sideL, side, sideLds, bi);
            }
            return wIdx;
          };
          auto fold1 = [&](const int k, const int pass, float& ac, float& lm, int& rec, unsigned& ekk, unsigned* defer) __attribute__((always_inline)) {
            const bool mine = ((firstMask >> k) & 1ull) && !(ekk & 0x80000000u) && (ekk & (1u << 28)) && in_pass(ekk, pass);
            if (mine) {
              const unsigned head = chain_head((ekk >> 13) & ekBucket);
              if (NARROW) tab[(ekk >> 13) & ekBucket] = 0u;
              ekk &= 0x1FFFu;
              if (head & 0x80000000u) {
                int wIdx = -1;
                const int hi = (int) (head & 0x7FFFFFFFu);
                unsigned hnext; double pt;
                { int cdummy; side_link(sideL, side, sideLds, hi, cdummy, pt, hnext); }
                if (!(hnext & 0x80000000u)) {
                  if (pt < (double) __fadd_rn(ac, lm)) wIdx = hi;
                } else if (defer) *defer = head;
                else wIdx = fold_multi(k * nthr + tq, head, ac, lm);
                if (wIdx >= 0) {
                  side_winner(sideL, side, sideLds, wIdx, ac, lm, rec);
                  ekk = 0x80000000u | (unsigned) wIdx;
                }
              }
            }
          };
          auto insert8 = [&](const int g8, const int* rec8, unsigned* ek8) __attribute__((always_inline)) {
            int xd[kB];
#pragma unroll
            for (int i = 0; i < kB; i++) xd[i] = ka->G.xrecC[rec8[i] & 0x3FFFFFFF].dst;
#pragma unroll
            for (int i = 0; i < kB; i++) {
              const int c = (g8 + i) * nthr + tq;
              if (c < C && (ek8[i] & (1u << 27)) && !(ek8[i] & 0x80000000u)) ek8[i] |= (table_insert((unsigned) xd[i], (unsigned) xd[i] * 2654435761u, c) << 13) | (1u << 28);
            }
          };
          for (int pass = 0; pass < nPass; pass++) {
            if (!NARROW && pass > 0) {
              __syncthreads();
              { uint4* h4 = reinterpret_cast<uint4*>(hkey); const int q4 = hashN >> 2;
                for (int i = tq; i < 2 * q4; i += nthr) { unsigned wv = (i < q4) ? 0u : 0xFFFFFFFFu; asm volatile("" : "+v"(wv)); h4[i] = make_uint4(wv, wv, wv, wv); }    }
              __syncthreads();
#pragma unroll
              for (int g8 = 0; g8 < kFastK; g8 += kB) if (g8 < K) insert8(g8, &qrec[g8], &ek[g8]);
              for (int kb = kFastK; kb < K; kb += kB) {
                float oac[kB], olm[kB]; int orec[kB]; unsigned oek[kB]; park_load(kb, oac, olm, orec, oek);
                insert8(kb, orec, oek); park_store(kb, oac, olm, orec, oek);
              }
              __syncthreads();
            }
            {
              unsigned later = 0u;
#pragma unroll
              for (int k = 0; k < kFastK; k++) {
                const bool cand = k < K && k * nthr + tq < C && (ek[k] & (1u << 28)) && in_pass(ek[k], pass) && !((firstMask >> k) & 1ull);
                if (cand) {
                  if (is_first((ek[k] >> 13) & ekBucket, k * nthr + tq)) firstMask |= 1ull << k;
                  else if (!((double) __fadd_rn(qac[k], qlm[k]) > doomT)) later |= 1u << k;
                }
              }
              asm volatile("" : "+v"(later));
              __builtin_amdgcn_sched_barrier(0);
              while (__any(later != 0u)) {
                if (later) {
                  const int k = __ffs((int) later) - 1; later &= later - 1u;
                  unsigned ekk = ek[0];
#pragma unroll
                  for (int j = 1; j < kFastK; j++) ekk = (k == j) ? ek[j] : ekk;
                  const int c = k * nthr + tq;
                  const double tt = ttlS[c]; const uint32_t pb = ctk[ekk & 0x1FFFu].bp;
                  const unsigned h = (ekk >> 13) & ekBucket;
                  const int sx = atomicAdd(&s_sideN, 1);
                  const unsigned nx = push_side(h, sx);
                  float ac = qac[0], lm = qlm[0]; int rec = qrec[0];
#pragma unroll
                  for (int j = 1; j < kFastK; j++) { const bool is = (k == j); ac = is ? qac[j] : ac; lm = is ? qlm[j] : lm; rec = is ? qrec[j] : rec; }
                  Side* dstS = (sx < sideLds) ? nullptr : &side[sx];
                  if (!dstS) { Side& q = sideL[sx]; q.ttl = tt; q.ac = ac; q.lm = lm; q.rec = rec; q.prevBp = pb; q.c = c; q.next = nx; }
                  else { dstS->ttl = tt; dstS->ac = ac; dstS->lm = lm; dstS->rec = rec; dstS->prevBp = pb; dstS->c = c; dstS->next = nx; }
                }
              }
            }
            for (int kb = kFastK; kb < K; kb += kB) { float oac[kB], olm[kB]; int orec[kB]; unsigned oek[kB]; park_load(kb, oac, olm, orec, oek); later8(kb, pass, oac, olm, orec, oek); }
            if (pass == 0) TICK(20);
            __syncthreads();
            if (pass == 0) TICK(5);
            {
              unsigned pend = 0u, dh[kFastK];
#pragma unroll
              for (int k = 0; k < kFastK; k++) { dh[k] = 0u; if (k < K) { fold1(k, pass, qac[k], qlm[k], qrec[k], ek[k], &dh[k]); if (dh[k]) pend |= 1u << k; } }
              if (pass == 0) TICK(24);
              while (__any(pend != 0u)) {
                if (pend) {
                  const int k = __ffs((int) pend) - 1; pend &= pend - 1u;
                  unsigned head = dh[0]; float ac = qac[0], lm = qlm[0];
#pragma unroll
                  for (int j = 1; j < kFastK; j++) { const bool is = (k == j); head = is ? dh[j] : head; ac = is ? qac[j] : ac; lm = is ? qlm[j] : lm; }
                  const int wIdx = fold_multi(k * nthr + tq, head, ac, lm);
                  if (wIdx >= 0) {
                    float wac, wlm; int wrec;
                    side_winner(sideL, side, sideLds, wIdx, wac, wlm, wrec);
#pragma unroll
                    for (int j = 0; j < kFastK; j++) if (k == j) { qac[j] = wac; qlm[j] = wlm; qrec[j] = wrec; ek[j] = 0x80000000u | (unsigned) wIdx; }
                  }
                }
              }
            }
            if (pass == 0) TICK(25);
            for (int kb = kFastK; kb < K; kb += kB) {
              float oac[kB], olm[kB]; int orec[kB]; unsigned oek[kB]; park_load(kb, oac, olm, orec, oek);
#pragma unroll
              for (int i = 0; i < kB; i++) if (kb + i < K) fold1(kb + i, pass, oac[i], olm[i], orec[i], oek[i], nullptr);
              park_store(kb, oac, olm, orec, oek);
            }
          }
          TICK(12);
          if (s_err) { status = DSR_E_ALLOCATION; break; }
          unsigned long long keepMask = 0ull;
#pragma unroll
          for (int k = 0; k < kFastK; k++) if (k < K && ((firstMask >> k) & 1ull)) {
            const float sc1 = __fadd_rn(qac[k], qlm[k]);
            if (!prune || !((double) sc1 > threshNext)) keepMask |= 1ull << k;
          }
          for (int kb = kFastK; kb < K; kb += kB) {
            float oac[kB], olm[kB]; int orec[kB]; unsigned oek[kB]; park_load(kb, oac, olm, orec, oek);
#pragma unroll
            for (int i = 0; i < kB; i++) if (kb + i < K && ((firstMask >> (kb + i)) & 1ull)) {
              const float sc1 = __fadd_rn(oac[i], olm[i]);
              if (!prune || !((double) sc1 > threshNext)) keepMask |= 1ull << (kb + i);
            }
          }
          int allFirst = 0;
          for (int k = 0; k < K; k++) {
            const unsigned long long bal = __ballot((keepMask >> k) & 1ull);
            if (lq == 0) s_cnt[k * nw + wq] = __popcll(bal);
            allFirst += __popcll(__ballot((firstMask >> k) & 1ull));
          }
          if (lq == 0) s_waveTotE[wq] = allFirst;
          TICK(13);
          __syncthreads();
          TICK(14);
          if (!NARROW) {
            uint4* h4 = reinterpret_cast<uint4*>(hkey); const int q4 = hashN >> 2;
            for (int i = tq; i < 2 * q4; i += nthr) { unsigned wv = (i < q4) ? 0u : 0xFFFFFFFFu; asm volatile("" : "+v"(wv)); h4[i] = make_uint4(wv, wv, wv, wv); }
          }
          if (wq == 0) {
            const int nG = K * nw;
            int a[6], tot = 0;
#pragma unroll
            for (int q = 0; q < 6; q++) { a[q] = (6 * lq + q < nG) ? s_cnt[6 * lq + q] : 0; tot += a[q]; }
            const int incl = wave_incl_scan(tot, lq); int run = incl - tot;
#pragma unroll
            for (int q = 0; q < 6; q++) { if (6 * lq + q < nG) s_cnt[6 * lq + q] = run; run += a[q]; }
            if (lq == 63) s_waveTot[0] = incl;
          }
          __syncthreads();
          TICK(6);
          numNew = uni(s_waveTot[0]);
          { const int a = (lq < nw) ? s_waveTotE[lq] : 0; numStat = __builtin_amdgcn_readlane(wave_incl_scan(a, lq), 63); }
          RELOAD();
          if (numNew > ka->D.maxTok || (segS > 0 ? arenaUsed : arenaOff) + numNew > ka->D.arenaCap) { status = DSR_E_ALLOCATION; break; }
          if (segS > 0 && arenaOff + numNew > chunkEnd) {
            const long need = numNew > ka->D.poolChunk ? (long) numNew : ka->D.poolChunk;
            __syncthreads();
            if (tid == 0) s_chunk = (long long) atomicAdd(ka->D.poolNext, (unsigned long long) need);
            __syncthreads();
            arenaOff = (long) s_chunk; chunkEnd = arenaOff + need;
            if (chunkEnd > ka->D.poolCap) { status = DSR_E_ALLOCATION; break; }
          }
          const XRecC* const xrecW = ka->G.xrecC; TokA* const outA = nxtA; TokB* const outB = nxtB; Bp* const outBp = arena + arenaOff;
          auto write4 = [&](auto NB, const int g4, const float* ac4, const float* lm4, const int* rec4, const unsigned* ek4) __attribute__((always_inline)) {
            constexpr int nb = decltype(NB)::value;
            int4 dx[nb]; uint32_t pv[nb];
#pragma unroll
            for (int i = 0; i < nb; i++) {
              const bool kp = (keepMask >> (g4 + i)) & 1ull;
              dx[i] = *reinterpret_cast<const int4*>(&xrecW[kp ? (rec4[i] & 0x3FFFFFFF) : 0]);
              const bool sw = kp && (ek4[i] & 0x80000000u) != 0u; const unsigned si = ek4[i] & 0x7FFFFFFFu;
              const uint32_t* pb = (sw && si >= (unsigned) sideLds) ? &side[si].prevBp : &ctk[(sw || !kp) ? 0u : (ek4[i] & 0x1FFFu)].bp;
              pv[i] = *pb;
              if (sw && si < (unsigned) sideLds) pv[i] = sideL[si].prevBp;
            }
#pragma unroll
            for (int i = 0; i < nb; i++) {
              const int k = g4 + i;
              if (k < K) {
                const bool isFirst = (keepMask >> k) & 1ull;
                const unsigned long long bal = __ballot(isFirst);
                if (isFirst) {
                  const int pos = numNew - 1 - (s_cnt[k * nw + wq] + __popcll(bal & ((1ull << lq) - 1ull)));
                  TokA na; na.ac = ac4[i]; na.lm = lm4[i]; na.bp = (uint32_t) (arenaOff + pos); na.xs = (uint32_t) dx[i].y | ((rec4[i] & 0x40000000) ? 0x80000000u : 0u);
                  TokB nb; nb.node = dx[i].x; nb.cnt = dx[i].z;
                  Bp bp; bp.prev = pv[i]; bp.rec = (uint32_t) (rec4[i] & 0x3FFFFFFF);
                  outA[pos] = na; outB[pos] = nb; outBp[pos] = bp;
                  if (pos < cntCap) cntL[pos] = (unsigned short) dx[i].z;
                }
              }
            }
          };
          const bool dense = numNew <= (hashN >> 1);
          if (dense) {
            uint4* const stage = reinterpret_cast<uint4*>(hkey);
            auto stage1 = [&](const int k, const float ac, const float lm, const int rec, const unsigned ekk) __attribute__((always_inline)) {
              const bool isFirst = (keepMask >> k) & 1ull;
              const unsigned long long bal = __ballot(isFirst);
              if (isFirst) stage[s_cnt[k * nw + wq] + __popcll(bal & ((1ull << lq) - 1ull))] = make_uint4(__float_as_uint(ac), __float_as_uint(lm), (unsigned) rec, ekk);
            };
#pragma unroll
            for (int k = 0; k < kFastK; k++) if (k < K) stage1(k, qac[k], qlm[k], qrec[k], ek[k]);
            for (int kb = kFastK; kb < K; kb += kB) {
              float oac[kB], olm[kB]; int orec[kB]; unsigned oek[kB]; park_load(kb, oac, olm, orec, oek);
#pragma unroll
              for (int i = 0; i < kB; i++) if (kb + i < K) stage1(kb + i, oac[i], olm[i], orec[i], oek[i]);
            }
            __syncthreads();
            TICK(21);
            const int q4 = hashN >> 2;
            const bool layNext = prune && numNew <= 4 * nthr;
            preC = -1;
            auto denseLoad = [&](const int f0, uint4* en, int4* dx, uint32_t* pv) __attribute__((always_inline)) {
#pragma unroll
              for (int i = 0; i < 2; i++) {
                const int f = f0 + i * nthr + tq; const bool on = f < numNew;
                en[i] = stage[on ? f : 0];
                if (on) { unsigned wv = (NARROW || f < q4) ? 0u : 0xFFFFFFFFu; asm volatile("" : "+v"(wv)); stage[f] = make_uint4(wv, wv, wv, wv); }
              }
#pragma unroll
              for (int i = 0; i < 2; i++) {
                const bool on = f0 + i * nthr + tq < numNew;
                dx[i] = *at32<int4>(xrecW, (on ? (en[i].z & 0x3FFFFFFFu) : 0u) * 16u);
                const bool sw = on && (en[i].w & 0x80000000u) != 0u; const unsigned si = en[i].w & 0x7FFFFFFFu;
                const uint32_t* pb = (sw && si >= (unsigned) sideLds) ? &side[si].prevBp : &ctk[(sw || !on) ? 0u : (en[i].w & 0x1FFFu)].bp;
                pv[i] = *pb;
                if (sw && si < (unsigned) sideLds) pv[i] = sideL[si].prevBp;
              }
            };
            auto denseStore = [&](const int f0, const uint4* en, const int4* dx, const uint32_t* pv) __attribute__((always_inline)) {
#pragma unroll
              for (int i = 0; i < 2; i++) {
                const int f = f0 + i * nthr + tq;
                if (f < numNew) {
                  const int pos = numNew - 1 - f;
                  TokA na; na.ac = __uint_as_float(en[i].x); na.lm = __uint_as_float(en[i].y); na.bp = (uint32_t) (arenaOff + pos); na.xs = (uint32_t) dx[i].y | ((en[i].z & 0x40000000u) ? 0x80000000u : 0u);
                  TokB nb; nb.node = dx[i].x; nb.cnt = dx[i].z;
                  Bp bp; bp.prev = pv[i]; bp.rec = (uint32_t) (en[i].z & 0x3FFFFFFFu);
                  outA[pos] = na; outB[pos] = nb; outBp[pos] = bp;
                  if (pos < cntCap) cntL[pos] = (unsigned short) dx[i].z;
                }
              }
            };
            auto layOut = [&](auto NE_, const int* cn) __attribute__((always_inline)) {
              constexpr int NE = decltype(NE_)::value;
              int in[NE]; bool bad = false;
#pragma unroll
              for (int i = 0; i < NE; i++) {
                in[i] = wave_incl_scan(cn[i], lq);
                bad = bad || (i * nthr + tq < numNew && cn[i] == 0);
              }
              const int badW = __any(bad) ? 1 : 0;
              if (lq == 63) {
#pragma unroll
                for (int i = 0; i < NE; i++) s_cnt[i * nw + wq] = in[i];
                s_waveTotE[wq] = badW;
              }
              __syncthreads();
              const int tg = (lq < NE * nw) ? s_cnt[lq] : 0;
              const int sg = wave_incl_scan(tg, lq);
              const int total = __builtin_amdgcn_readlane(sg, 63), wu = uni(wq);
              const bool anyBad = __any(((lq < nw) ? s_waveTotE[lq] : 0) != 0);
              const bool fits = total <= fastCapC;
#pragma unroll
              for (int i = 0; i < NE; i++) {
                const int f = i * nthr + tq; const int off = total - (__builtin_amdgcn_readlane(sg - tg, i * nw + wu) + in[i]);
                if (fits && f < numNew && cn[i] > 0) {
                  const int e = numNew - 1 - f;
                  atomicOr(&s_bm[off >> 5], 1u << (off & 31));
                  for (int g = (off >> 6) + 1; g <= ((off + cn[i]) >> 6); g++) s_gbase[g] = (unsigned) (e + 1) | ((unsigned) (64 * g - off) << 13);
                }
              }
              if (tq == 0) { s_sideN = 0; s_gbase[0] = 0; s_err = 0; }
              preC = (anyBad || !fits) ? -1 : total;
            };
            if (layNext && numNew > 2 * nthr) {
              int cn[4];
#pragma unroll
              for (int h = 0; h < 2; h++) {
                uint4 en[2]; int4 dx[2]; uint32_t pv[2];
                denseLoad(h * 2 * nthr, en, dx, pv); denseStore(h * 2 * nthr, en, dx, pv);
#pragma unroll
                for (int i = 0; i < 2; i++) cn[2 * h + i] = ((2 * h + i) * nthr + tq < numNew) ? dx[i].z : 0;
              }
              layOut(std::integral_constant<int, 4>{}, cn);
            } else {
              for (int f0 = 0; f0 < numNew; f0 += 2 * nthr) {
                uint4 en[2]; int4 dx[2]; uint32_t pv[2];
                denseLoad(f0, en, dx, pv);
                if (layNext) {
                  const int cn[2] = { (tq < numNew) ? dx[0].z : 0, (nthr + tq < numNew) ? dx[1].z : 0 };
                  layOut(std::integral_constant<int, 2>{}, cn);
                }
                denseStore(f0, en, dx, pv);
              }
            }
            TICK(22);
          } else
          {
#pragma unroll
          for (int g4 = 0; g4 < kFastK; g4 += kW) if (g4 < K) write4(std::integral_constant<int, kW>{}, g4, &qac[g4], &qlm[g4], &qrec[g4], &ek[g4]);
          for (int kb = kFastK; kb < K; kb += kB) {
            float oac[kB], olm[kB]; int orec[kB]; unsigned oek[kB]; park_load(kb, oac, olm, orec, oek);
            write4(std::integral_constant<int, kB>{}, kb, oac, olm, orec, oek);
          }
          TICK(21);
          TICK(22);
          preC = -1;
          }
          cntOK = prune && numNew <= cntCap;
        }
      }
      if (!fast) {
      cntOK = false; preC = -1;
      RELOAD();
      int* tokOff = ka->D.tokOff + (size_t) slot * (ka->D.maxTok + 1);
      int* tokCnt = ka->D.tokCnt + (size_t) slot * (ka->D.maxTok + 1);
      int* chead = ka->D.chead + (size_t) slot * ka->D.maxCand;
      int* owner = ka->D.owner + (size_t) slot * ka->D.maxCand;
      int* rank = ka->D.rank + (size_t) slot * ka->D.maxCand;
      unsigned* first = ka->D.first + (size_t) slot * ka->G.nNodes;
      unsigned tag = s_tag;
      __syncthreads();
      if (tag <= 1u) { for (int i = tid; i < ka->G.nNodes; i += nthr) first[i] = 0xFFFFFFFFu; tag = 255u; __syncthreads(); } else tag--;
      if (tid == 0) s_tag = tag;
      const unsigned tagw = tag << 24;
      const bool sorted = EXTRA && ka->D.topN > 0 && mode == 0 && fr > 0;
      if (sorted) {
        unsigned long long* keys = reinterpret_cast<unsigned long long*>(cA);
        for (int i = tid; i < n; i += nthr) { const TokA t = curA[i]; keys[i] = ((unsigned long long) f2ord(__fadd_rn(t.ac, t.lm)) << 32) | (unsigned) i; }
        __syncthreads();
        for (int i = tid; i < n; i += nthr) {
          const unsigned long long ki = keys[i]; int rk = 0;
          for (int j = 0; j < n; j++) rk += (keys[j] < ki) ? 1 : 0;
          if (rk < ka->D.topN) { sprA[rk] = curA[i]; sprB[rk] = curB[i]; }
        }
        __syncthreads();
        { const int t = bufCur; bufCur = bufSpr; bufSpr = t; }
        n = n < ka->D.topN ? n : ka->D.topN;
      }
      const double threshM = (EXTRA && ka->D.topN > 0) ? HUGE_VAL : thresh;
      const int chunkT = ((n + nw * 64 - 1) / (nw * 64)) * 64;
      {
        int running = 0;
        const int b0 = wave * chunkT, b1 = (b0 + chunkT < n) ? b0 + chunkT : n;
        for (int base = b0; base < b1; base += 64) {
          const int i = base + lane; int cnt = 0;
          if (i < b1) {
            const TokA ta = curA[i]; const TokB tb = curB[i];
            if (mode == 0) {
              const float s = __fadd_rn(ta.ac, ta.lm);
              if (!((double) s > threshM)) cnt = tb.cnt;
            } else cnt = (ka->G.nodeFinal[tb.node] ? 1 : 0) + (ka->G.eoff[tb.node + 1] - ka->G.eoff[tb.node]);
          }
          const int incl = wave_incl_scan(cnt, lane);
          if (i < b1) { tokOff[i] = running + incl - cnt; tokCnt[i] = cnt; }
          running += __shfl(incl, 63, 64);
        }
        if (lane == 0) s_waveTot[wave] = running;
      }
      __syncthreads();
      int C = 0;
      for (int w = 0; w < nw; w++) C += s_waveTot[w];
      if (C > ka->D.maxCand) { status = DSR_E_ALLOCATION; break; }
      if (EXTRA && ka->D.latOn && s_latOff + C > ka->D.latCap) { status = DSR_E_ALLOCATION; break; }
      Cfr = C;
      const bool useHash = hashN > 0 && C <= tableC;
      for (int i = tid; i < n; i += nthr) {
        const int cnt = tokCnt[i];
        if (cnt == 0) continue;
        const int w = i / chunkT; int base = 0;
        for (int q = 0; q < w; q++) base += s_waveTot[q];
        const int off = base + tokOff[i];
        tokOff[i] = off;
        for (int j = 0; j < cnt; j++) owner[off + j] = i;
      }
      __syncthreads();
      double locMin = HUGE_VAL;
      for (int c = tid; c < C; c += nthr) {
        const int i = owner[c]; const TokA ta = curA[i]; const int nd = curB[i].node; const bool tokSil = (ta.xs >> 31) != 0u;
        Tok t; t.node = nd; t.ac = ta.ac; t.lm = ta.lm; t.bp = ta.bp;
        const int j = c - tokOff[i];
        double ac = (double) t.ac, lm; int dst, recId; bool silArc = false;
        if (mode == 0) {
          recId = (int) (ta.xs & 0x7FFFFFFFu) + j; const XRec x = ka->G.xrec[recId];
          const int plen = (int) (x.meta & 0xFFFFu);
          double lmNode = (double) t.lm; uint32_t prevIn = tokSil ? ka->D.silenceX : (ka->D.silenceX + 1u);
          bool prevNull = (t.bp == kNone) && (fr == 0);
          if (plen) {
            const int* pp = ka->G.path + ka->G.xpathOff[recId];
            for (int h = 0; h < plen; h++) {
              const int a = pp[h];
              double l = __dadd_rn(lmNode, __dmul_rn(ka->D.lmScale, (double) ka->G.arcCost[a]));
              if (ka->G.arcOut[a] != 0) l = __dadd_rn(l, __dmul_rn(ka->D.lmScale, ka->D.lmPenalty));
              if (0u == ka->D.silenceX && (prevNull || prevIn != ka->D.silenceX)) l = __dadd_rn(l, __dmul_rn(ka->D.lmScale, ka->D.silPenalty));
              lmNode = (double) (float) l; prevIn = 0u; prevNull = false;
            }
          }
          lm = __dadd_rn(lmNode, __dmul_rn(ka->D.lmScale, (double) x.cost));
          if (x.meta & 0x10000u) lm = __dadd_rn(lm, __dmul_rn(ka->D.lmScale, ka->D.lmPenalty));
          if ((uint32_t) (x.dist + 1) == ka->D.silenceX && (prevNull || prevIn != ka->D.silenceX)) lm = __dadd_rn(lm, __dmul_rn(ka->D.lmScale, ka->D.silPenalty));
          ac = __dadd_rn(ac, (double) (useLdsRow ? srow[x.dist] : rowG[x.dist]));
          dst = x.dst; silArc = ((uint32_t) (x.dist + 1) == ka->D.silenceX);
        } else {
          const int hasSelf = ka->G.nodeFinal[nd] ? 1 : 0;
          if (hasSelf && j == 0) {
            const float lmf = (float) __dadd_rn((double) t.lm, __dmul_rn(ka->D.lmScale, (double) ka->G.nodeCost[nd]));
            lm = (double) lmf; dst = nd; recId = (int) 0x7FFFFFFE;
          } else {
            recId = ka->G.eoff[nd] + (j - hasSelf); const ERec e = ka->G.erec[recId];
            const int* pp = ka->G.path + e.pathOff; double lmNode = (double) t.lm; double l = lmNode;
            uint32_t prevIn = tokSil ? ka->D.silenceX : (ka->D.silenceX + 1u);
            for (int h = 0; h < e.pathLen; h++) {
              const int a = pp[h];
              l = __dadd_rn(lmNode, __dmul_rn(ka->D.lmScale, (double) ka->G.arcCost[a]));
              if (ka->G.arcOut[a] != 0) l = __dadd_rn(l, __dmul_rn(ka->D.lmScale, ka->D.lmPenalty));
              if (0u == ka->D.silenceX && prevIn != ka->D.silenceX) l = __dadd_rn(l, __dmul_rn(ka->D.lmScale, ka->D.silPenalty));
              lmNode = (double) (float) l; prevIn = 0u;
            }
            lm = __dadd_rn(l, __dmul_rn(ka->D.lmScale, (double) ka->G.nodeCost[e.lastSrc]));
            dst = e.dst; recId = (int) ((uint32_t) recId | kEndBit);
          }
        }
        const double ttl = __dadd_rn(ac, lm);
        CandA a2; a2.ttl = ttl; a2.ac = (float) ac; a2.lm = (float) lm; cA[c] = a2;
        if (useHash) {
          unsigned h = ((unsigned) dst * 2654435761u) >> 7 & (unsigned) (tabN - 1);
          if (NARROW) {
            const unsigned key = (unsigned) dst + 1u, w = (key << 15) | (unsigned) c;
            for (;;) {
              const unsigned k = atomicCAS(&tab[h], 0u, w);
              if (k == 0u) break;
              if ((k >> 15) == key) { atomicMin(&tab[h], w); break; }
              h = (h + 1u) & (unsigned) (tabN - 1);
            }
          } else {
            for (;;) {
              const unsigned k = atomicCAS(&hkey[h], 0u, (unsigned) dst + 1u);
              if (k == 0u || k == (unsigned) dst + 1u) break;
              h = (h + 1u) & (unsigned) (hashN - 1);
            }
            atomicMin(&hfirst[h], (unsigned) c);
          }
          rank[c] = (int) h;
        } else atomicMin(&first[dst], tagw | (unsigned) c);
        chead[c] = -1;
        if (silArc) recId |= 0x40000000;
        CandB b2; b2.dst = dst; b2.next = -1; b2.rec = recId; b2.prevBp = t.bp; cB[c] = b2;
        if (mode == 0 && ttl < locMin) locMin = ttl;
      }
      locMin = wave_min_d(locMin);
      if (lane == 0) s_waveMin[wave] = locMin;
      __syncthreads();
      topScore = HUGE_VAL;
      for (int w = 0; w < nw; w++) { const double v = s_waveMin[w]; if (v < topScore) topScore = v; }
      for (int c = tid; c < C; c += nthr) {
        int f;
        if (useHash) f = NARROW ? (int) (tab[rank[c]] & 0x7FFFu) : (int) hfirst[rank[c]];
        else { const int dst = cB[c].dst; f = (int) (ld_u32(&first[dst]) & 0x00FFFFFFu); }
        if (f != c) { const int nx = atomicExch(&chead[f], c); cB[c].next = nx; chead[c] = -2; }
      }
      __syncthreads();
      if (useHash) for (int i = tid; i < 2 * hashN; i += nthr) hkey[i] = (NARROW || i < hashN) ? 0u : 0xFFFFFFFFu;
      const int chunkC = ((C + nw * 64 - 1) / (nw * 64)) * 64;
      const double threshNextM = __dadd_rn(topScore, ka->D.beam);
      const bool pruneM = !dump && mode == 0 && (fr + 1 < T) && !(EXTRA && ka->D.topN > 0);
      {
        int running = 0, runAll = 0;
        const int b0 = wave * chunkC, b1 = (b0 + chunkC < C) ? b0 + chunkC : C;
        for (int base = b0; base < b1; base += 64) {
          const int c = base + lane; bool isFirst = false, isAny = false;
          if (c < b1) {
            const int h0 = ld_i32(&chead[c]);
            isFirst = (h0 != -2);
            if (isFirst) {
              int w = c; CandA aw = cA[w];
              double fw = (double) __fadd_rn(aw.ac, aw.lm);
              for (;;) {
                int best = 0x7FFFFFFF;
                int steps = 0;
                for (int p = h0; p >= 0 && steps <= C; p = cB[p].next, steps++) if (p > w && p < best && cA[p].ttl < fw) best = p;
                if (best == 0x7FFFFFFF) break;
                w = best; aw = cA[w]; fw = (double) __fadd_rn(aw.ac, aw.lm);
              }
              isAny = true;
              if (pruneM && ((double) __fadd_rn(aw.ac, aw.lm) > threshNextM)) { isFirst = false; w = -3; }
              chead[c] = w;
            }
          }
          const unsigned long long bal = __ballot(isFirst);
          if (isFirst) rank[c] = running + __popcll(bal & ((1ull << lane) - 1ull));
          running += __popcll(bal); runAll += __popcll(__ballot(isAny));
        }
        if (lane == 0) { s_waveTot[wave] = running; s_waveTotE[wave] = runAll; }
      }
      __syncthreads();
      numStat = 0;
      for (int w = 0; w < nw; w++) { numNew += s_waveTot[w]; numStat += s_waveTotE[w]; }
      if (numNew > ka->D.maxTok || (segS > 0 ? arenaUsed : arenaOff) + numNew > ka->D.arenaCap) { status = DSR_E_ALLOCATION; break; }
      if (segS > 0 && arenaOff + numNew > chunkEnd) {
        const long need = numNew > ka->D.poolChunk ? (long) numNew : ka->D.poolChunk;
        __syncthreads();
        if (tid == 0) s_chunk = (long long) atomicAdd(ka->D.poolNext, (unsigned long long) need);
        __syncthreads();
        arenaOff = (long) s_chunk; chunkEnd = arenaOff + need;
        if (chunkEnd > ka->D.poolCap) { status = DSR_E_ALLOCATION; break; }
      }
      {
        int wbase = 0; for (int q = 0; q < wave; q++) wbase += s_waveTot[q];
        const int b0 = wave * chunkC, b1 = (b0 + chunkC < C) ? b0 + chunkC : C;
        for (int base = b0; base < b1; base += 64) {
          const int c = base + lane;
          if (c < b1) {
            const int w = chead[c];
            if (w >= 0) {
              const CandB bc = cB[c];
              const int pos = numNew - 1 - (wbase + rank[c]);
              const CandA aw = cA[w]; const CandB bw = (w == c) ? bc : cB[w]; const int recW = (bw.rec & 0x3FFFFFFF) | (bw.rec & (int) 0x80000000);
              const int xo = ka->G.xoff[bc.dst];
              TokA na; na.ac = aw.ac; na.lm = aw.lm; na.bp = (uint32_t) (arenaOff + pos); na.xs = (uint32_t) xo;
              TokB nb; nb.node = bc.dst; nb.cnt = ka->G.xoff[bc.dst + 1] - xo;
              Bp bp;
              if (mode == 0) {
                if (bw.rec & 0x40000000) na.xs |= 0x80000000u;
                bp.prev = bw.prevBp; bp.rec = (uint32_t) recW;
              } else {
                if (bw.rec == (int) 0x7FFFFFFE) { if (segS > 0) { const unsigned long long v = ld_u64_dev(&arena[bw.prevBp]); bp.prev = (uint32_t) v; bp.rec = (uint32_t) (v >> 32); } else { const Bp o = arena[bw.prevBp]; bp = o; } }
                else { bp.prev = bw.prevBp; bp.rec = (uint32_t) bw.rec; }
              }
              nxtA[pos] = na; nxtB[pos] = nb; arena[arenaOff + pos] = bp;
              if (EXTRA && ka->D.latOn) ka->D.arenaLat[(size_t) u * ka->D.arenaCap + arenaOff + pos] = (int) (s_latOff + w);
            }
          }
        }
      }
      if (EXTRA && ka->D.latOn) {
        uint4* lat = ka->D.lat + (size_t) u * ka->D.latCap; double* ltt = ka->D.latTtl + (size_t) u * ka->D.latCap;
        const long latOff = (long) s_latOff;
        for (int c = tid; c < C; c += nthr) {
          const CandA a = cA[c]; const CandB b = cB[c];
          lat[latOff + c] = make_uint4(__float_as_uint(a.ac), __float_as_uint(a.lm), (unsigned) b.rec, b.prevBp); ltt[latOff + c] = a.ttl;
        }
        __syncthreads();
        if (tid == 0) { s_latOff = latOff + C; ka->D.latFrameOff[(size_t) u * (ka->Tmax + 3) + fr + 1] = latOff + C; }
      }
      }
      __syncthreads();
      TICK(fast ? 7 : 8);
      if (PROF && tid == 0 && mode == 0) { const int cls = !fast ? 3 : Cfr <= kFastK * nthr ? 0 : Cfr <= 12288 ? 1 : 2; s_hist[cls] += 1; s_hist[4 + cls] += s_tlast - s_tfr; s_hist[8 + cls] += Cfr; if (!fast && Cfr <= 28672) s_hist[14] += 1; if (!fast && Cfr <= 32767) s_hist[15] += 1; }
      RELOAD();
      if (mode == 0) {
        if (dump) {
          long* cnt = ka->D.dumpCount; const long o = cnt[0];
          if (o + numNew <= ka->D.dumpCap) {
            for (int i = tid; i < numNew; i += nthr) {
              const TokA t = ld_tok(&nxtA[i]); ka->D.dumpNode[o + i] = nxtB[i].node; ka->D.dumpAc[o + i] = t.ac; ka->D.dumpLm[o + i] = t.lm;
              ka->D.dumpArc[o + i] = ka->G.xarc[arena[t.bp].rec];
            }
          }
          __syncthreads();
          if (tid == 0) { ka->D.dumpFrameOff[fr] = o; ka->D.dumpFrameOff[fr + 1] = o + numNew; cnt[0] = o + numNew; cnt[1] = fr + 1; }
        }
        if (numStat < 0) numStat = numNew;
        if (numStat == 0 || numNew == 0) { status = DSR_E_CONSISTENCY; break; }
        { const int t = bufCur; bufCur = bufNxt; bufNxt = t; }
        n = numNew; arenaOff += numNew; arenaUsed += numNew;
        if (tid == nthr - 1) { s_stat[0] += numStat; s_stat[1] += Cfr; if (fast) s_stat[2] += 1; if (numStat > s_maxActive) s_maxActive = numStat; }
        thresh = __dadd_rn(topScore, ka->D.beam);
      } else {
        const TokA* lst = numNew > 0 ? nxtA : curA; const int cntL = numNew > 0 ? numNew : n;
        unsigned long long key = ~0ull;
        for (int i = tid; i < cntL; i += nthr) {
          const TokA t = lst[i]; const float s = __fadd_rn(t.ac, t.lm);
          if (s == s) { const unsigned long long k = ((unsigned long long) f2ord(s) << 32) | (unsigned) i; if (k < key) key = k; }
        }
        key = wave_min_u64(key);
        if (lane == 0) s_waveKey[wave] = key;
        if (EXTRA && ka->D.latOn) {
          const TokB* lstB = numNew > 0 ? nxtB : curB; int4* lf = ka->D.latFinal + (size_t) u * ka->D.maxTok;
          for (int i = tid; i < cntL; i += nthr) { const TokA t = ld_tok(&lst[i]); lf[i] = make_int4(lstB[i].node, (int) t.bp, __float_as_int(t.ac), __float_as_int(t.lm)); }
          if (tid == 0) { int* li = ka->D.latInfo + 4 * (size_t) u; li[0] = cntL; li[1] = numNew > 0 ? 1 : 0; li[2] = (int) (arenaOff + (numNew > 0 ? numNew : 0)); li[3] = T; }
        }
        __syncthreads();
        if (tid == 0) {
          dsr_decode_result* const res = ka->res;
          clear_result(&res[u]); dsr_decode_result& r = res[u];
          unsigned long long k = ~0ull; for (int w = 0; w < nw; w++) if (s_waveKey[w] < k) k = s_waveKey[w];
          r.frames = T - 1; r.reachedFinal = numNew > 0 ? 1 : 0; r.finalStatesN = numNew;  r.activeHypos = (long) s_stat[0]; r.placements = (long) s_stat[1] + Cfr; r.registerFrames = (long) (s_stat[2] & 0xFFFFFFFFll); r.laidOutFrames_ = (int) (s_stat[2] >> 32); r.maxActiveSeen = s_maxActive; r.status = DSR_OK;
          TraceHead hd; hd.arenaOff = (unsigned long long) ((size_t) ((EXTRA && ka->D.latOn) ? u : (ka->D.segFrames > 0 ? 0 : slot)) * ka->D.arenaCap);  hd.bp = kNone; hd.hops = kNone;
          if (k != ~0ull) {
            const TokA bt = ld_tok(&lst[(unsigned) (k & 0xFFFFFFFFu)]);
            r.ac = bt.ac; r.lm = bt.lm; r.score = __dadd_rn((double) bt.ac, (double) bt.lm);
            hd.bp = bt.bp;
            if (ka->walkHere) {
              int* const hopRec = ka->hopRec + (size_t) u * ka->hopStride; const int walkCap = 2 * ka->D.maxCand < ka->hopStride ? 2 * ka->D.maxCand : ka->hopStride; int nH = 0;
              for (uint32_t bq = bt.bp; bq != kNone && nH < walkCap; ) { const uint2 e = *reinterpret_cast<const uint2*>(&arena[bq]); hopRec[nH++] = (int) e.y; bq = e.x; }
              hd.hops = (uint32_t) nH;
            }
          } else r.status = DSR_E_CONSISTENCY;
          ka->heads[u] = hd;
        }
        __syncthreads();
        TICK(9);
      }
    }

    RELOAD();
    if (PROF && tid == 0) s_prof[15] = (long long) wall_clock64();
    if (segS > 0 && status == DSR_OK && fr <= T) {
      TokA* const svA = ka->D.saveA + (size_t) u * ka->D.maxTok; TokB* const svB = ka->D.saveB + (size_t) u * ka->D.maxTok;
      for (int i = tid; i < n; i += nthr) { svA[i] = curA[i]; svB[i] = curB[i]; }
      if (tid == 0) {
        SegState* const sst = ka->D.segState + u;
        st_i32(&sst->n, n); st_i32(&sst->status, DSR_OK); st_i32(&sst->maxActive, s_maxActive); st_u64_dev(&sst->arenaOff, (unsigned long long) arenaOff); st_u64_dev(&sst->chunkEnd, (unsigned long long) chunkEnd); st_u64_dev(&sst->arenaUsed, (unsigned long long) arenaUsed);
        st_u64_dev(&sst->thresh, (unsigned long long) __double_as_longlong(thresh));
        st_u64_dev(&sst->stat[0], (unsigned long long) s_stat[0]); st_u64_dev(&sst->stat[1], (unsigned long long) s_stat[1]); st_u64_dev(&sst->stat[2], (unsigned long long) s_stat[2]);
      }
      if (nq == 1) __builtin_amdgcn_fence(__ATOMIC_RELEASE, "agent");
      else __builtin_amdgcn_fence(__ATOMIC_RELEASE, "workgroup");
      __syncthreads();
      if (tid == 0) st_i32(&ka->D.segDone[u], seg + 1);
      continue;
    }
    if (status != DSR_OK) {
      if (tid == 0) {
        dsr_decode_result* const res = ka->res; clear_result(&res[u]); res[u].status = status; res[u].frames = T - 1;
        { TraceHead hd; hd.arenaOff = 0ull; hd.bp = kNone; hd.hops = kNone; ka->heads[u] = hd; }
        if (segS > 0) { st_i32(&ka->D.segState[u].status, status); asm volatile("s_waitcnt vmcnt(0)" ::: "memory"); st_i32(&ka->D.segDone[u], 0x7FFFFFFF); }
      }
    }
  }
  RELOAD();
  if (tid == 0) ka->D.tags[slot] = s_tag;
  if (PROF && tid < 32) ka->D.prof[slot * kProfN + tid] = s_prof[tid];
  if (PROF && tid < 16) ka->D.prof[slot * kProfN + 32 + tid] = s_hist[tid];
  if (PROF && tid < 8) ka->D.prof[slot * kProfN + 48 + tid] = (long long) s_hop[tid];
#undef TICK
#undef RELOAD
#undef TOKA
#undef TOKB
#undef curA
#undef nxtA
#undef curB
#undef nxtB
#undef sprA
#undef sprB
#undef ctok
#undef side
#undef cA
#undef cB
#undef arena
#undef sc
#undef dump
}

}

extern "C" __global__ void k_xcc_probe(int* out) { if (threadIdx.x == 0) out[blockIdx.x] = (int) (__builtin_amdgcn_s_getreg((3 << 11) | 20) & 15u); }

namespace dsr {

void xcc_probe_launch(int* out64, hipStream_t st) { launch(k_xcc_probe, dim3(64), dim3(64), 0, st, out64); }

typedef void (*VitKernel)(const VitArgs);
static constexpr VitKernel kVitKernels[8] = { k_viterbi<0>, k_viterbi<1>, k_viterbi<2>, k_viterbi<3>, k_viterbi<4>, k_viterbi<5>, k_viterbi<6>, k_viterbi<7> };

size_t viterbi_static_lds(int modes)
{
  hipFuncAttributes fattr; DSR_HIP(hipFuncGetAttributes(&fattr, (const void*) kVitKernels[modes & 7]));
  return fattr.sharedSizeBytes;
}
void viterbi_launch(int modes, const VitArgs& A, int slots, size_t ldsBytes, hipStream_t st)
{
  const VitKernel k = kVitKernels[modes & 7];
  launch(k, dim3(slots), dim3(kThreads), ldsBytes, st, A);
}

}
```

distantspeechrecognition-mirror_amd/csrc/viterbi.h:

```cpp
#pragma once
#include "common.h"
#include "wfst_graph.h"

namespace dsr {

struct Tok { int32_t node; float ac; float lm; uint32_t bp; };
struct TokA { float ac; float lm; uint32_t bp; uint32_t xs; };
struct TokB { int32_t node; int32_t cnt; };
struct XRecD { int32_t dist; uint32_t meta; int32_t dst; int32_t p2; double lmCost; double lmEps1; };
struct XRecC { int32_t dst; int32_t dstXoff; int32_t dstCnt; int32_t pad; };
struct Side { double ttl; float ac; float lm; int32_t rec; uint32_t prevBp; int32_t c; uint32_t next; };
struct CandA { double ttl; float ac; float lm; };
struct CandB { int32_t dst; int32_t next; int32_t rec; uint32_t prevBp; };
struct Bp { uint32_t prev; uint32_t rec; };
struct TraceHead { unsigned long long arenaOff; uint32_t bp; uint32_t hops; };
static_assert(sizeof(TokA) == 16 && sizeof(TokB) == 8 && sizeof(XRecD) == 32 && sizeof(XRecC) == 16 && sizeof(Side) == 32 && sizeof(CandA) == 16 && sizeof(CandB) == 16 && sizeof(Bp) == 8 && sizeof(TraceHead) == 16,
              "record layouts shared by the host and k_viterbi");

static constexpr int kThreads = 1024;
static constexpr int kFastC = 24576;
static constexpr int kProfN = 56;
static constexpr int kSideLds = 496;

struct GraphDev {
  int nNodes, initial;
  const int* xoff; const XRec* xrec; const XRecD* xrecD; const XRecC* xrecC; const int* xarc; const int* xpathOff;
  const int* eoff; const ERec* erec; const int* path; const float* pathCost;
  const float* arcCost; const uint32_t* arcOut; const uint32_t* arcIn;
  const int* nodeFinal; const float* nodeCost;
};

struct SegState { int n, status, maxActive, pad; long arenaOff, chunkEnd, arenaUsed; double thresh; long long stat[3]; };

struct DecDev {
  double beam, lmScale, lmPenalty, silPenalty; uint32_t silenceX; int noPen;
  int segFrames, segCount, segQueues, segDrop; long poolCap, poolChunk;    unsigned long long* poolNext; SegState* segState; int* segDone; TokA* saveA; TokB* saveB;
  int maxTok, maxCand; long arenaCap;
  TokA* tokA; TokB* tokB; TokA* ctok; Side* side; int fastOK; int* tokOff; int* tokCnt; int* owner; int* rank; int* chead; CandA* cA; CandB* cB; unsigned* first; unsigned* tags; Bp* arena;
  int* queue; long long* prof;
  int dumpOn; long dumpCap; long* dumpFrameOff; int* dumpNode; float* dumpAc; float* dumpLm; int* dumpArc; long* dumpCount;
  int latOn; long latCap; uint4* lat; double* latTtl; long* latFrameOff; int* arenaLat; int4* latFinal; int* latInfo;
  int topN; TokA* tokA3; TokB* tokB3;
};

struct VitArgs {
  GraphDev G; DecDev D;
  const float* scores; const int* nframesArr; int U, Tmax, nDist;
  dsr_decode_result* res; int* arcsOut; unsigned* wordsOut; int maxPath, useLdsRow, hashN, regionB, cntCap;
  TraceHead* heads;
  int* hopRec; int hopStride, walkHere;
  int oneEach;
};

struct TraceArgs {
  const TraceHead* heads; const Bp* arena; unsigned long long arenaN;
  const XRec* xrec; const ERec* erec; const int* xarc; const int* xpathOff; const int* path; const uint32_t* arcOut;
  int* hopRec; int* hopOff; int hopStride, hopCap;
  dsr_decode_result* res; int* arcsOut; unsigned* wordsOut; int maxPath, U;
};

size_t viterbi_static_lds(int modes);
void viterbi_launch(int modes, const VitArgs& A, int slots, size_t ldsBytes, hipStream_t st);
void traceback_launch(const TraceArgs& A, hipStream_t st);
void xcc_probe_launch(int* out64, hipStream_t st);

}
```

Before: 28.61.

## Move end-of-utterance expansion and best-token search into a separate k_finish kernel

When time-sliced segmentation is active, the main Viterbi kernel now stops at the last frame and saves state. A new lightweight 256-thread k_finish kernel then performs the final end-state expansion and best-token selection for every utterance. The shared frame-expansion and best-token code is factored into a common header so both kernels can use it. The aim is to keep the heavy 1024-thread persistent kernel from spending its tail on this per-utterance final step, at the cost of one extra launch and a reload of the saved tokens.

Measured after the change: 28.72 (median of 6 runs). No clear change (+0.4%).

```diff
diff --git a/distantspeechrecognition-mirror_amd/csrc/decode_plan.h b/distantspeechrecognition-mirror_amd/csrc/decode_plan.h
--- a/distantspeechrecognition-mirror_amd/csrc/decode_plan.h
+++ b/distantspeechrecognition-mirror_amd/csrc/decode_plan.h
@@ -20,6 +20,7 @@
   bool noHash = false;
   bool noCnt = false;
   bool tableWide = false;
+  bool finish = true;
 };
 
 inline VitEnv read_vit_env()
@@ -37,6 +38,7 @@
   e.noHash = getenv("DSR_VITERBI_NOHASH") != nullptr;
   e.noCnt = getenv("DSR_VITERBI_NOCNT") != nullptr;
   e.tableWide = (v = getenv("DSR_VITERBI_TABLE")) && !strcmp(v, "wide");
+  e.finish = !((v = getenv("DSR_VITERBI_FINISH")) && atoi(v) == 0);
   return e;
 }
 
@@ -49,6 +51,7 @@
 
 struct DecodePlan {
   int slots, segFrames, segQueues, segCount, poolArenas; long arenaPer; int useLdsRow, hashN, cntCap, modes; size_t ldsBytes; bool narrow;
+  bool finishLater;
 };
 
 static constexpr size_t kPlanSideBytes = (size_t) 496 * 32;
@@ -80,6 +83,7 @@
   }
   p.slots = slots; p.segFrames = segFrames; p.segQueues = segQueues; p.poolArenas = poolArenas; p.arenaPer = arenaPer;
   p.segCount = segFrames > 0 ? (Tmax + segFrames) / segFrames : 1;
+  p.finishLater = segFrames > 0 && env.finish;
   int modes = plan_base_modes(in, env);
   const size_t eoffB = kPlanSideBytes; const size_t ldsCap = (size_t) 160 * 1024 - in.staticLds;
   const int hashMax = 16384;
diff --git a/distantspeechrecognition-mirror_amd/csrc/decoder.cpp b/distantspeechrecognition-mirror_amd/csrc/decoder.cpp
--- a/distantspeechrecognition-mirror_amd/csrc/decoder.cpp
+++ b/distantspeechrecognition-mirror_amd/csrc/decoder.cpp
@@ -22,6 +22,7 @@
   long arenaCap = 0; int initial = 0; unsigned tokenMemoryLimit = 0;
   long lastPoolCap = 0;
   hipEvent_t evTrace = nullptr;
+  hipEvent_t evFin0 = nullptr, evFin1 = nullptr; bool profFinish = false;
   DevBuf<TraceHead> d_heads; DevBuf<int> d_hopRec, d_hopOff;
   DevBuf<SegState> d_segState; DevBuf<int> d_segDone; DevBuf<unsigned long long> d_poolNext; DevBuf<TokA> d_saveA; DevBuf<TokB> d_saveB;
   DevBuf<WTok> w_tok; DevBuf<WCand> w_cand; DevBuf<int> w_tokOff, w_rank; DevBuf<unsigned long long> w_best; DevBuf<unsigned> w_first; DevBuf<int4> w_traces; size_t w_tablesFor = 0;
@@ -97,6 +98,8 @@
   forget_traceback(d);
   if (d->evDone) (void) hipEventDestroy(d->evDone);
   if (d->evTrace) (void) hipEventDestroy(d->evTrace);
+  if (d->evFin0) (void) hipEventDestroy(d->evFin0);
+  if (d->evFin1) (void) hipEventDestroy(d->evFin1);
   delete d;
 }
 
@@ -367,6 +370,7 @@
   d->d_hopRec.reserve((size_t) U * A.hopStride); d->d_hopOff.reserve((size_t) U * A.hopStride); A.hopRec = d->d_hopRec.p;
   A.oneEach = (P.segFrames == 0 && slots == U) ? 1 : 0;
   A.walkHere = (P.segFrames == 0 && !latOn && !A.oneEach) ? 1 : 0;
+  A.finishLater = P.finishLater ? 1 : 0;
   return A;
 }
 
@@ -401,10 +405,16 @@
     ensure_scratch(d, P.slots, Tmax, latOn ? U : (P.segFrames > 0 ? P.poolArenas : 0));
     if (maxPath < 0) maxPath = 0;
     const VitArgs A = fill_vit_args(d, P, env, score, nframes, U, Tmax, nDist, maxPath, want_paths != 0, st);
-    if (env.segVerbose) fprintf(stderr, "[dsr viterbi] %d utterances on %d workgroups: %s, %s state table\n", U, P.slots, P.segFrames > 0 ? (P.segQueues == 8 ? "time-sliced, XCD-bound queues" : "time-sliced, one queue") : "run to completion", P.narrow ? "narrow" : "wide");
+    if (env.segVerbose) fprintf(stderr, "[dsr viterbi] %d utterances on %d workgroups: %s, %s state table, end expansion in %s\n", U, P.slots, P.segFrames > 0 ? (P.segQueues == 8 ? "time-sliced, XCD-bound queues" : "time-sliced, one queue") : "run to completion", P.narrow ? "narrow" : "wide", P.finishLater ? "k_finish" : "k_viterbi");
     const TraceArgs TA = fill_trace_args(d, A);
     order_behind_last_traceback(P.slots, st);
     viterbi_launch(P.modes, A, P.slots, P.ldsBytes, st);
+    d->profFinish = false;
+    if (P.finishLater) {
+      if (env.prof) { for (hipEvent_t* e : { &d->evFin0, &d->evFin1 }) if (!*e) DSR_HIP(hipEventCreate(e)); DSR_HIP(hipEventRecord(d->evFin0, st)); }
+      finish_launch(A, P.slots, st);
+      if (env.prof) { DSR_HIP(hipEventRecord(d->evFin1, st)); d->profFinish = true; }
+    }
     traceback_launch(TA, st);
     publish_traceback(d, st);
     enqueue_result_copies(d, U, want_paths ? (size_t) U * maxPath : 0, st);
@@ -468,6 +478,10 @@
       fprintf(stderr, "[dsr viterbi] frames: %lld laid out by the frame before, %lld through P1/P2, %lld on the memory path\n", laid, reg - laid, all - reg);
     }
     if (prof) report_profile(prof, slots);
+    if (prof && d->profFinish) {
+      float ms = 0.0f; DSR_HIP(hipEventElapsedTime(&ms, d->evFin0, d->evFin1));
+      fprintf(stderr, "[dsr viterbi prof] k_finish (end expansion and best token, behind the decode): %.0f us for %d utterances on %d workgroups\n", ms * 1e3, U, slots);
+    }
     if (d->dumpOn) {
       long cnt[2]; DSR_HIP(hipMemcpy(cnt, d->d_dumpCount.p, sizeof(cnt), hipMemcpyDeviceToHost));
       const long N = cnt[0] < d->dumpCap ? cnt[0] : d->dumpCap; d->h_dumpFrames = cnt[1];
diff --git a/distantspeechrecognition-mirror_amd/csrc/k_viterbi.hip b/distantspeechrecognition-mirror_amd/csrc/k_viterbi.hip
--- a/distantspeechrecognition-mirror_amd/csrc/k_viterbi.hip
+++ b/distantspeechrecognition-mirror_amd/csrc/k_viterbi.hip
@@ -1,13 +1,12 @@
 #include "launch.h"
 #include "viterbi.h"
+#include "viterbi_end.h"
 #include <algorithm>
 #include <cmath>
 #include <type_traits>
 
 namespace dsr {
 
-static constexpr uint32_t kNone = 0xFFFFFFFFu;
-static constexpr uint32_t kEndBit = 0x80000000u;
 static constexpr int kWaves = kThreads / 64;
 static constexpr int kFastK = 8;
 static constexpr int kB = 2;
@@ -15,25 +14,8 @@
 static constexpr int kP1 = 16;
 static constexpr int kW = 4;
 
-typedef const __attribute__((address_space(4))) VitArgs* KP;
-
-__device__ __forceinline__ unsigned ld_u32(const unsigned* p) { return __hip_atomic_load(p, __ATOMIC_RELAXED, __HIP_MEMORY_SCOPE_AGENT); }
-__device__ __forceinline__ int ld_i32(const int* p) { return __hip_atomic_load(p, __ATOMIC_RELAXED, __HIP_MEMORY_SCOPE_AGENT); }
-__device__ __forceinline__ void st_u32(unsigned* p, unsigned v) { __hip_atomic_store(p, v, __ATOMIC_RELAXED, __HIP_MEMORY_SCOPE_AGENT); }
-__device__ __forceinline__ void st_i32(int* p, int v) { __hip_atomic_store(p, v, __ATOMIC_RELAXED, __HIP_MEMORY_SCOPE_AGENT); }
-__device__ __forceinline__ void st_u64_dev(void* p, unsigned long long v) { __hip_atomic_store(reinterpret_cast<unsigned long long*>(p), v, __ATOMIC_RELAXED, __HIP_MEMORY_SCOPE_AGENT); }
-__device__ __forceinline__ unsigned long long ld_u64_dev(const void* p) { return __hip_atomic_load(reinterpret_cast<const unsigned long long*>(p), __ATOMIC_RELAXED, __HIP_MEMORY_SCOPE_AGENT); }
-
-__device__ __forceinline__ int wave_incl_scan(int v, int )
-{
-  v += __builtin_amdgcn_update_dpp(0, v, 0x111, 0xF, 0xF, true);
-  v += __builtin_amdgcn_update_dpp(0, v, 0x112, 0xF, 0xF, true);
-  v += __builtin_amdgcn_update_dpp(0, v, 0x114, 0xF, 0xF, true);
-  v += __builtin_amdgcn_update_dpp(0, v, 0x118, 0xF, 0xF, true);
-  v += __builtin_amdgcn_update_dpp(0, v, 0x142, 0xA, 0xF, false);
-  v += __builtin_amdgcn_update_dpp(0, v, 0x143, 0xC, 0xF, false);
-  return v;
-}
+
+
 __device__ __forceinline__ float wave_max_f_uni(float v)
 {
 #define DSR_DPP_F(ctrl, rm) { const float o = __int_as_float(__builtin_amdgcn_update_dpp(__float_as_int(v), __float_as_int(v), ctrl, rm, 0xF, false)); v = fmaxf(v, o); }
@@ -49,40 +31,15 @@
 #undef DSR_DPP_D
   return __hiloint2double(__builtin_amdgcn_readlane(__double2hiint(v), 63), __builtin_amdgcn_readlane(__double2loint(v), 63));
 }
-__device__ __forceinline__ double wave_min_d(double v)
-{
-#pragma unroll
-  for (int d = 32; d >= 1; d >>= 1) { const double o = __shfl_xor(v, d, 64); v = (o < v) ? o : v; }
-  return v;
-}
-__device__ __forceinline__ unsigned long long wave_min_u64(unsigned long long v)
-{
-#pragma unroll
-  for (int d = 32; d >= 1; d >>= 1) { const unsigned long long o = __shfl_xor(v, d, 64); v = (o < v) ? o : v; }
-  return v;
-}
 __device__ __forceinline__ float wave_max_f(float v)
 {
 #pragma unroll
   for (int d = 32; d >= 1; d >>= 1) v = fmaxf(v, __shfl_xor(v, d, 64));
   return v;
-}
-__device__ __forceinline__ void clear_result(dsr_decode_result* r)
-{
-  int z = 0; asm volatile("" : "+v"(z));
-  int* p = reinterpret_cast<int*>(r);
-#pragma unroll 1
-  for (int i = 0; i < (int) (sizeof(dsr_decode_result) / 4); i++) p[i] = z;
 }
 typedef __attribute__((address_space(3))) float lds_float_t;
 typedef __attribute__((address_space(3))) Side lds_side_t;
 #define DSR_NO_MERGE() asm volatile("" ::: "memory")
-__device__ __forceinline__ TokA ld_tok(const TokA* p)
-{
-  const unsigned long long a = reinterpret_cast<const volatile unsigned long long*>(p)[0], b = reinterpret_cast<const volatile unsigned long long*>(p)[1];
-  TokA t; t.ac = __uint_as_float((unsigned) (a & 0xFFFFFFFFull)); t.lm = __uint_as_float((unsigned) (a >> 32)); t.bp = (uint32_t) (b & 0xFFFFFFFFull); t.xs = (uint32_t) (b >> 32);
-  return t;
-}
 __device__ __forceinline__ void side_winner(const Side* sideL, const Side* side, int sideLds, int idx, float& ac, float& lm, int& rec)
 {
   if (idx < sideLds) {
@@ -113,7 +70,6 @@
 template <class T> __device__ __forceinline__ T* at32w(void* base, uint32_t byteOff) { return reinterpret_cast<T*>(reinterpret_cast<char*>(base) + byteOff); }
 __device__ __forceinline__ int uni(int v) { return __builtin_amdgcn_readfirstlane(v); }
 __device__ __forceinline__ double uni(double v) { return __hiloint2double(__builtin_amdgcn_readfirstlane(__double2hiint(v)), __builtin_amdgcn_readfirstlane(__double2loint(v))); }
-__device__ __forceinline__ unsigned f2ord(float f) { const unsigned u = __float_as_uint(f); return (u & 0x80000000u) ? ~u : (u | 0x80000000u); }
 
 template <int MODES>
 __global__ __launch_bounds__(kThreads) void k_viterbi(const VitArgs argsInKernarg)
@@ -157,20 +113,9 @@
 
   const int tid = threadIdx.x;
   const int slot = blockIdx.x;
-#define TOKA(ix) ((EXTRA && (ix) == 2) ? ka->D.tokA3 + (size_t) slot * ka->D.maxTok : ka->D.tokA + ((size_t) slot * 2 + (size_t) (ix)) * ka->D.maxTok)
-#define TOKB(ix) ((EXTRA && (ix) == 2) ? ka->D.tokB3 + (size_t) slot * ka->D.maxTok : ka->D.tokB + ((size_t) slot * 2 + (size_t) (ix)) * ka->D.maxTok)
-#define curA TOKA(bufCur)
-#define nxtA TOKA(bufNxt)
-#define curB TOKB(bufCur)
-#define nxtB TOKB(bufNxt)
-#define sprA TOKA(bufSpr)
-#define sprB TOKB(bufSpr)
 #define ctok (ka->D.ctok + (size_t) slot * 8192)
 #define side (ka->D.side + (size_t) slot * kFastC)
-#define cA (ka->D.cA + (size_t) slot * ka->D.maxCand)
-#define cB (ka->D.cB + (size_t) slot * ka->D.maxCand)
   if (tid == 0) s_tag = ka->D.tags[slot];
-#define arena (ka->D.arena + (size_t) ((EXTRA && ka->D.latOn) ? u : (ka->D.segFrames > 0 ? 0 : slot)) * ka->D.arenaCap)
 #define sc (ka->scores + (size_t) u * ka->Tmax * nDist)
   constexpr int fastCapC = ((kFastK + 32) * nthr < kFastC) ? (kFastK + 32) * nthr : kFastC;
   constexpr int fastCapN = kP1 * 64 * nw;
@@ -204,11 +149,11 @@
     const int u = s_u; if (u < 0) break;
     const bool whole = s_seg < 0; const int seg = whole ? 0 : s_seg;
     const int T = ka->nframesArr[u] < ka->Tmax ? ka->nframesArr[u] : ka->Tmax;
-    const int fr0 = seg * segS, frEnd = (segS > 0 && !whole) ? fr0 + segS : 0x7FFFFFFF;
-    if (fr0 > T) continue;
+    const bool later = segS > 0 && !whole && ka->finishLater != 0;
+    const int fr0 = seg * segS, frEnd = (segS > 0 && !whole) ? ((later && fr0 + segS > T) ? T : fr0 + segS) : 0x7FFFFFFF;
+    if (fr0 > T || (later && seg > 0 && fr0 == T)) continue;
     if (EXTRA && ka->D.latOn && tid == 0) ka->D.latFrameOff[(size_t) u * (ka->Tmax + 3)] = 0;
     if (PROF && tid == 0) { const long long tn = (long long) wall_clock64(); if (s_prof[15]) s_prof[10] += tn - s_prof[15]; s_tlast = tn; }
-#define dump (EXTRA && ka->D.dumpOn && slot == 0)
 
     int status = DSR_OK;
     if (T <= 0) status = DSR_E_ITERATOR;
@@ -933,17 +878,6 @@
       if (!fast) {
       cntOK = false; preC = -1;
       RELOAD();
-      int* tokOff = ka->D.tokOff + (size_t) slot * (ka->D.maxTok + 1);
-      int* tokCnt = ka->D.tokCnt + (size_t) slot * (ka->D.maxTok + 1);
-      int* chead = ka->D.chead + (size_t) slot * ka->D.maxCand;
-      int* owner = ka->D.owner + (size_t) slot * ka->D.maxCand;
-      int* rank = ka->D.rank + (size_t) slot * ka->D.maxCand;
-      unsigned* first = ka->D.first + (size_t) slot * ka->G.nNodes;
-      unsigned tag = s_tag;
-      __syncthreads();
-      if (tag <= 1u) { for (int i = tid; i < ka->G.nNodes; i += nthr) first[i] = 0xFFFFFFFFu; tag = 255u; __syncthreads(); } else tag--;
-      if (tid == 0) s_tag = tag;
-      const unsigned tagw = tag << 24;
       const bool sorted = EXTRA && ka->D.topN > 0 && mode == 0 && fr > 0;
       if (sorted) {
         unsigned long long* keys = reinterpret_cast<unsigned long long*>(cA);
@@ -959,210 +893,8 @@
         n = n < ka->D.topN ? n : ka->D.topN;
       }
       const double threshM = (EXTRA && ka->D.topN > 0) ? HUGE_VAL : thresh;
-      const int chunkT = ((n + nw * 64 - 1) / (nw * 64)) * 64;
-      {
-        int running = 0;
-        const int b0 = wave * chunkT, b1 = (b0 + chunkT < n) ? b0 + chunkT : n;
-        for (int base = b0; base < b1; base += 64) {
-          const int i = base + lane; int cnt = 0;
-          if (i < b1) {
-            const TokA ta = curA[i]; const TokB tb = curB[i];
-            if (mode == 0) {
-              const float s = __fadd_rn(ta.ac, ta.lm);
-              if (!((double) s > threshM)) cnt = tb.cnt;
-            } else cnt = (ka->G.nodeFinal[tb.node] ? 1 : 0) + (ka->G.eoff[tb.node + 1] - ka->G.eoff[tb.node]);
-          }
-          const int incl = wave_incl_scan(cnt, lane);
-          if (i < b1) { tokOff[i] = running + incl - cnt; tokCnt[i] = cnt; }
-          running += __shfl(incl, 63, 64);
-        }
-        if (lane == 0) s_waveTot[wave] = running;
-      }
-      __syncthreads();
-      int C = 0;
-      for (int w = 0; w < nw; w++) C += s_waveTot[w];
-      if (C > ka->D.maxCand) { status = DSR_E_ALLOCATION; break; }
-      if (EXTRA && ka->D.latOn && s_latOff + C > ka->D.latCap) { status = DSR_E_ALLOCATION; break; }
-      Cfr = C;
-      const bool useHash = hashN > 0 && C <= tableC;
-      for (int i = tid; i < n; i += nthr) {
-        const int cnt = tokCnt[i];
-        if (cnt == 0) continue;
-        const int w = i / chunkT; int base = 0;
-        for (int q = 0; q < w; q++) base += s_waveTot[q];
-        const int off = base + tokOff[i];
-        tokOff[i] = off;
-        for (int j = 0; j < cnt; j++) owner[off + j] = i;
-      }
-      __syncthreads();
-      double locMin = HUGE_VAL;
-      for (int c = tid; c < C; c += nthr) {
-        const int i = owner[c]; const TokA ta = curA[i]; const int nd = curB[i].node; const bool tokSil = (ta.xs >> 31) != 0u;
-        Tok t; t.node = nd; t.ac = ta.ac; t.lm = ta.lm; t.bp = ta.bp;
-        const int j = c - tokOff[i];
-        double ac = (double) t.ac, lm; int dst, recId; bool silArc = false;
-        if (mode == 0) {
-          recId = (int) (ta.xs & 0x7FFFFFFFu) + j; const XRec x = ka->G.xrec[recId];
-          const int plen = (int) (x.meta & 0xFFFFu);
-          double lmNode = (double) t.lm; uint32_t prevIn = tokSil ? ka->D.silenceX : (ka->D.silenceX + 1u);
-          bool prevNull = (t.bp == kNone) && (fr == 0);
-          if (plen) {
-            const int* pp = ka->G.path + ka->G.xpathOff[recId];
-            for (int h = 0; h < plen; h++) {
-              const int a = pp[h];
-              double l = __dadd_rn(lmNode, __dmul_rn(ka->D.lmScale, (double) ka->G.arcCost[a]));
-              if (ka->G.arcOut[a] != 0) l = __dadd_rn(l, __dmul_rn(ka->D.lmScale, ka->D.lmPenalty));
-              if (0u == ka->D.silenceX && (prevNull || prevIn != ka->D.silenceX)) l = __dadd_rn(l, __dmul_rn(ka->D.lmScale, ka->D.silPenalty));
-              lmNode = (double) (float) l; prevIn = 0u; prevNull = false;
-            }
-          }
-          lm = __dadd_rn(lmNode, __dmul_rn(ka->D.lmScale, (double) x.cost));
-          if (x.meta & 0x10000u) lm = __dadd_rn(lm, __dmul_rn(ka->D.lmScale, ka->D.lmPenalty));
-          if ((uint32_t) (x.dist + 1) == ka->D.silenceX && (prevNull || prevIn != ka->D.silenceX)) lm = __dadd_rn(lm, __dmul_rn(ka->D.lmScale, ka->D.silPenalty));
-          ac = __dadd_rn(ac, (double) (useLdsRow ? srow[x.dist] : rowG[x.dist]));
-          dst = x.dst; silArc = ((uint32_t) (x.dist + 1) == ka->D.silenceX);
-        } else {
-          const int hasSelf = ka->G.nodeFinal[nd] ? 1 : 0;
-          if (hasSelf && j == 0) {
-            const float lmf = (float) __dadd_rn((double) t.lm, __dmul_rn(ka->D.lmScale, (double) ka->G.nodeCost[nd]));
-            lm = (double) lmf; dst = nd; recId = (int) 0x7FFFFFFE;
-          } else {
-            recId = ka->G.eoff[nd] + (j - hasSelf); const ERec e = ka->G.erec[recId];
-            const int* pp = ka->G.path + e.pathOff; double lmNode = (double) t.lm; double l = lmNode;
-            uint32_t prevIn = tokSil ? ka->D.silenceX : (ka->D.silenceX + 1u);
-            for (int h = 0; h < e.pathLen; h++) {
-              const int a = pp[h];
-              l = __dadd_rn(lmNode, __dmul_rn(ka->D.lmScale, (double) ka->G.arcCost[a]));
-              if (ka->G.arcOut[a] != 0) l = __dadd_rn(l, __dmul_rn(ka->D.lmScale, ka->D.lmPenalty));
-              if (0u == ka->D.silenceX && prevIn != ka->D.silenceX) l = __dadd_rn(l, __dmul_rn(ka->D.lmScale, ka->D.silPenalty));
-              lmNode = (double) (float) l; prevIn = 0u;
-            }
-            lm = __dadd_rn(l, __dmul_rn(ka->D.lmScale, (double) ka->G.nodeCost[e.lastSrc]));
-            dst = e.dst; recId = (int) ((uint32_t) recId | kEndBit);
-          }
-        }
-        const double ttl = __dadd_rn(ac, lm);
-        CandA a2; a2.ttl = ttl; a2.ac = (float) ac; a2.lm = (float) lm; cA[c] = a2;
-        if (useHash) {
-          unsigned h = ((unsigned) dst * 2654435761u) >> 7 & (unsigned) (tabN - 1);
-          if (NARROW) {
-            const unsigned key = (unsigned) dst + 1u, w = (key << 15) | (unsigned) c;
-            for (;;) {
-              const unsigned k = atomicCAS(&tab[h], 0u, w);
-              if (k == 0u) break;
-              if ((k >> 15) == key) { atomicMin(&tab[h], w); break; }
-              h = (h + 1u) & (unsigned) (tabN - 1);
-            }
-          } else {
-            for (;;) {
-              const unsigned k = atomicCAS(&hkey[h], 0u, (unsigned) dst + 1u);
-              if (k == 0u || k == (unsigned) dst + 1u) break;
-              h = (h + 1u) & (unsigned) (hashN - 1);
-            }
-            atomicMin(&hfirst[h], (unsigned) c);
-          }
-          rank[c] = (int) h;
-        } else atomicMin(&first[dst], tagw | (unsigned) c);
-        chead[c] = -1;
-        if (silArc) recId |= 0x40000000;
-        CandB b2; b2.dst = dst; b2.next = -1; b2.rec = recId; b2.prevBp = t.bp; cB[c] = b2;
-        if (mode == 0 && ttl < locMin) locMin = ttl;
-      }
-      locMin = wave_min_d(locMin);
-      if (lane == 0) s_waveMin[wave] = locMin;
-      __syncthreads();
-      topScore = HUGE_VAL;
-      for (int w = 0; w < nw; w++) { const double v = s_waveMin[w]; if (v < topScore) topScore = v; }
-      for (int c = tid; c < C; c += nthr) {
-        int f;
-        if (useHash) f = NARROW ? (int) (tab[rank[c]] & 0x7FFFu) : (int) hfirst[rank[c]];
-        else { const int dst = cB[c].dst; f = (int) (ld_u32(&first[dst]) & 0x00FFFFFFu); }
-        if (f != c) { const int nx = atomicExch(&chead[f], c); cB[c].next = nx; chead[c] = -2; }
-      }
-      __syncthreads();
-      if (useHash) for (int i = tid; i < 2 * hashN; i += nthr) hkey[i] = (NARROW || i < hashN) ? 0u : 0xFFFFFFFFu;
-      const int chunkC = ((C + nw * 64 - 1) / (nw * 64)) * 64;
-      const double threshNextM = __dadd_rn(topScore, ka->D.beam);
-      const bool pruneM = !dump && mode == 0 && (fr + 1 < T) && !(EXTRA && ka->D.topN > 0);
-      {
-        int running = 0, runAll = 0;
-        const int b0 = wave * chunkC, b1 = (b0 + chunkC < C) ? b0 + chunkC : C;
-        for (int base = b0; base < b1; base += 64) {
-          const int c = base + lane; bool isFirst = false, isAny = false;
-          if (c < b1) {
-            const int h0 = ld_i32(&chead[c]);
-            isFirst = (h0 != -2);
-            if (isFirst) {
-              int w = c; CandA aw = cA[w];
-              double fw = (double) __fadd_rn(aw.ac, aw.lm);
-              for (;;) {
-                int best = 0x7FFFFFFF;
-                int steps = 0;
-                for (int p = h0; p >= 0 && steps <= C; p = cB[p].next, steps++) if (p > w && p < best && cA[p].ttl < fw) best = p;
-                if (best == 0x7FFFFFFF) break;
-                w = best; aw = cA[w]; fw = (double) __fadd_rn(aw.ac, aw.lm);
-              }
-              isAny = true;
-              if (pruneM && ((double) __fadd_rn(aw.ac, aw.lm) > threshNextM)) { isFirst = false; w = -3; }
-              chead[c] = w;
-            }
-          }
-          const unsigned long long bal = __ballot(isFirst);
-          if (isFirst) rank[c] = running + __popcll(bal & ((1ull << lane) - 1ull));
-          running += __popcll(bal); runAll += __popcll(__ballot(isAny));
-        }
-        if (lane == 0) { s_waveTot[wave] = running; s_waveTotE[wave] = runAll; }
-      }
-      __syncthreads();
-      numStat = 0;
-      for (int w = 0; w < nw; w++) { numNew += s_waveTot[w]; numStat += s_waveTotE[w]; }
-      if (numNew > ka->D.maxTok || (segS > 0 ? arenaUsed : arenaOff) + numNew > ka->D.arenaCap) { status = DSR_E_ALLOCATION; break; }
-      if (segS > 0 && arenaOff + numNew > chunkEnd) {
-        const long need = numNew > ka->D.poolChunk ? (long) numNew : ka->D.poolChunk;
-        __syncthreads();
-        if (tid == 0) s_chunk = (long long) atomicAdd(ka->D.poolNext, (unsigned long long) need);
-        __syncthreads();
-        arenaOff = (long) s_chunk; chunkEnd = arenaOff + need;
-        if (chunkEnd > ka->D.poolCap) { status = DSR_E_ALLOCATION; break; }
-      }
-      {
-        int wbase = 0; for (int q = 0; q < wave; q++) wbase += s_waveTot[q];
-        const int b0 = wave * chunkC, b1 = (b0 + chunkC < C) ? b0 + chunkC : C;
-        for (int base = b0; base < b1; base += 64) {
-          const int c = base + lane;
-          if (c < b1) {
-            const int w = chead[c];
-            if (w >= 0) {
-              const CandB bc = cB[c];
-              const int pos = numNew - 1 - (wbase + rank[c]);
-              const CandA aw = cA[w]; const CandB bw = (w == c) ? bc : cB[w]; const int recW = (bw.rec & 0x3FFFFFFF) | (bw.rec & (int) 0x80000000);
-              const int xo = ka->G.xoff[bc.dst];
-              TokA na; na.ac = aw.ac; na.lm = aw.lm; na.bp = (uint32_t) (arenaOff + pos); na.xs = (uint32_t) xo;
-              TokB nb; nb.node = bc.dst; nb.cnt = ka->G.xoff[bc.dst + 1] - xo;
-              Bp bp;
-              if (mode == 0) {
-                if (bw.rec & 0x40000000) na.xs |= 0x80000000u;
-                bp.prev = bw.prevBp; bp.rec = (uint32_t) recW;
-              } else {
-                if (bw.rec == (int) 0x7FFFFFFE) { if (segS > 0) { const unsigned long long v = ld_u64_dev(&arena[bw.prevBp]); bp.prev = (uint32_t) v; bp.rec = (uint32_t) (v >> 32); } else { const Bp o = arena[bw.prevBp]; bp = o; } }
-                else { bp.prev = bw.prevBp; bp.rec = (uint32_t) bw.rec; }
-              }
-              nxtA[pos] = na; nxtB[pos] = nb; arena[arenaOff + pos] = bp;
-              if (EXTRA && ka->D.latOn) ka->D.arenaLat[(size_t) u * ka->D.arenaCap + arenaOff + pos] = (int) (s_latOff + w);
-            }
-          }
-        }
-      }
-      if (EXTRA && ka->D.latOn) {
-        uint4* lat = ka->D.lat + (size_t) u * ka->D.latCap; double* ltt = ka->D.latTtl + (size_t) u * ka->D.latCap;
-        const long latOff = (long) s_latOff;
-        for (int c = tid; c < C; c += nthr) {
-          const CandA a = cA[c]; const CandB b = cB[c];
-          lat[latOff + c] = make_uint4(__float_as_uint(a.ac), __float_as_uint(a.lm), (unsigned) b.rec, b.prevBp); ltt[latOff + c] = a.ttl;
-        }
-        __syncthreads();
-        if (tid == 0) { s_latOff = latOff + C; ka->D.latFrameOff[(size_t) u * (ka->Tmax + 3) + fr + 1] = latOff + C; }
-      }
+      if (!vit_memory_frame<kThreads, EXTRA, NARROW, true>(ka, slot, u, tid, mode, fr, T, segS, bufCur, bufNxt, n, threshM, arenaUsed, useLdsRow, srow, rowG, hkey, hashN,
+                                                          s_waveTot, s_waveTotE, s_waveMin, &s_tag, &s_chunk, &s_latOff, status, arenaOff, chunkEnd, numNew, numStat, Cfr, topScore)) break;
       }
       __syncthreads();
       TICK(fast ? 7 : 8);
@@ -1187,39 +919,7 @@
         if (tid == nthr - 1) { s_stat[0] += numStat; s_stat[1] += Cfr; if (fast) s_stat[2] += 1; if (numStat > s_maxActive) s_maxActive = numStat; }
         thresh = __dadd_rn(topScore, ka->D.beam);
       } else {
-        const TokA* lst = numNew > 0 ? nxtA : curA; const int cntL = numNew > 0 ? numNew : n;
-        unsigned long long key = ~0ull;
-        for (int i = tid; i < cntL; i += nthr) {
-          const TokA t = lst[i]; const float s = __fadd_rn(t.ac, t.lm);
-          if (s == s) { const unsigned long long k = ((unsigned long long) f2ord(s) << 32) | (unsigned) i; if (k < key) key = k; }
-        }
-        key = wave_min_u64(key);
-        if (lane == 0) s_waveKey[wave] = key;
-        if (EXTRA && ka->D.latOn) {
-          const TokB* lstB = numNew > 0 ? nxtB : curB; int4* lf = ka->D.latFinal + (size_t) u * ka->D.maxTok;
-          for (int i = tid; i < cntL; i += nthr) { const TokA t = ld_tok(&lst[i]); lf[i] = make_int4(lstB[i].node, (int) t.bp, __float_as_int(t.ac), __float_as_int(t.lm)); }
-          if (tid == 0) { int* li = ka->D.latInfo + 4 * (size_t) u; li[0] = cntL; li[1] = numNew > 0 ? 1 : 0; li[2] = (int) (arenaOff + (numNew > 0 ? numNew : 0)); li[3] = T; }
-        }
-        __syncthreads();
-        if (tid == 0) {
-          dsr_decode_result* const res = ka->res;
-          clear_result(&res[u]); dsr_decode_result& r = res[u];
-          unsigned long long k = ~0ull; for (int w = 0; w < nw; w++) if (s_waveKey[w] < k) k = s_waveKey[w];
-          r.frames = T - 1; r.reachedFinal = numNew > 0 ? 1 : 0; r.finalStatesN = numNew;  r.activeHypos = (long) s_stat[0]; r.placements = (long) s_stat[1] + Cfr; r.registerFrames = (long) (s_stat[2] & 0xFFFFFFFFll); r.laidOutFrames_ = (int) (s_stat[2] >> 32); r.maxActiveSeen = s_maxActive; r.status = DSR_OK;
-          TraceHead hd; hd.arenaOff = (unsigned long long) ((size_t) ((EXTRA && ka->D.latOn) ? u : (ka->D.segFrames > 0 ? 0 : slot)) * ka->D.arenaCap);  hd.bp = kNone; hd.hops = kNone;
-          if (k != ~0ull) {
-            const TokA bt = ld_tok(&lst[(unsigned) (k & 0xFFFFFFFFu)]);
-            r.ac = bt.ac; r.lm = bt.lm; r.score = __dadd_rn((double) bt.ac, (double) bt.lm);
-            hd.bp = bt.bp;
-            if (ka->walkHere) {
-              int* const hopRec = ka->hopRec + (size_t) u * ka->hopStride; const int walkCap = 2 * ka->D.maxCand < ka->hopStride ? 2 * ka->D.maxCand : ka->hopStride; int nH = 0;
-              for (uint32_t bq = bt.bp; bq != kNone && nH < walkCap; ) { const uint2 e = *reinterpret_cast<const uint2*>(&arena[bq]); hopRec[nH++] = (int) e.y; bq = e.x; }
-              hd.hops = (uint32_t) nH;
-            }
-          } else r.status = DSR_E_CONSISTENCY;
-          ka->heads[u] = hd;
-        }
-        __syncthreads();
+        vit_best_token<kThreads, EXTRA>(ka, slot, u, tid, bufCur, bufNxt, numNew, n, T, Cfr, arenaOff, s_waveKey, s_stat, &s_maxActive);
         TICK(9);
       }
     }
@@ -1243,8 +943,7 @@
     }
     if (status != DSR_OK) {
       if (tid == 0) {
-        dsr_decode_result* const res = ka->res; clear_result(&res[u]); res[u].status = status; res[u].frames = T - 1;
-        { TraceHead hd; hd.arenaOff = 0ull; hd.bp = kNone; hd.hops = kNone; ka->heads[u] = hd; }
+        vit_failed_result(ka, u, T, status);
         if (segS > 0) { st_i32(&ka->D.segState[u].status, status); asm volatile("s_waitcnt vmcnt(0)" ::: "memory"); st_i32(&ka->D.segDone[u], 0x7FFFFFFF); }
       }
     }
diff --git a/distantspeechrecognition-mirror_amd/csrc/viterbi.h b/distantspeechrecognition-mirror_amd/csrc/viterbi.h
--- a/distantspeechrecognition-mirror_amd/csrc/viterbi.h
+++ b/distantspeechrecognition-mirror_amd/csrc/viterbi.h
@@ -50,6 +50,7 @@
   TraceHead* heads;
   int* hopRec; int hopStride, walkHere;
   int oneEach;
+  int finishLater;
 };
 
 struct TraceArgs {
@@ -61,6 +62,7 @@
 
 size_t viterbi_static_lds(int modes);
 void viterbi_launch(int modes, const VitArgs& A, int slots, size_t ldsBytes, hipStream_t st);
+void finish_launch(const VitArgs& A, int slots, hipStream_t st);
 void traceback_launch(const TraceArgs& A, hipStream_t st);
 void xcc_probe_launch(int* out64, hipStream_t st);
 
diff --git a/distantspeechrecognition-mirror_amd/csrc/viterbi_end.h b/distantspeechrecognition-mirror_amd/csrc/viterbi_end.h
--- /dev/null
+++ b/distantspeechrecognition-mirror_amd/csrc/viterbi_end.h
@@ -0,0 +1,344 @@
+#pragma once
+#include "viterbi.h"
+
+namespace dsr {
+
+static constexpr uint32_t kNone = 0xFFFFFFFFu;
+static constexpr uint32_t kEndBit = 0x80000000u;
+
+typedef const __attribute__((address_space(4))) VitArgs* KP;
+
+__device__ __forceinline__ unsigned ld_u32(const unsigned* p) { return __hip_atomic_load(p, __ATOMIC_RELAXED, __HIP_MEMORY_SCOPE_AGENT); }
+__device__ __forceinline__ int ld_i32(const int* p) { return __hip_atomic_load(p, __ATOMIC_RELAXED, __HIP_MEMORY_SCOPE_AGENT); }
+__device__ __forceinline__ void st_u32(unsigned* p, unsigned v) { __hip_atomic_store(p, v, __ATOMIC_RELAXED, __HIP_MEMORY_SCOPE_AGENT); }
+__device__ __forceinline__ void st_i32(int* p, int v) { __hip_atomic_store(p, v, __ATOMIC_RELAXED, __HIP_MEMORY_SCOPE_AGENT); }
+__device__ __forceinline__ void st_u64_dev(void* p, unsigned long long v) { __hip_atomic_store(reinterpret_cast<unsigned long long*>(p), v, __ATOMIC_RELAXED, __HIP_MEMORY_SCOPE_AGENT); }
+__device__ __forceinline__ unsigned long long ld_u64_dev(const void* p) { return __hip_atomic_load(reinterpret_cast<const unsigned long long*>(p), __ATOMIC_RELAXED, __HIP_MEMORY_SCOPE_AGENT); }
+
+__device__ __forceinline__ int wave_incl_scan(int v, int )
+{
+  v += __builtin_amdgcn_update_dpp(0, v, 0x111, 0xF, 0xF, true);
+  v += __builtin_amdgcn_update_dpp(0, v, 0x112, 0xF, 0xF, true);
+  v += __builtin_amdgcn_update_dpp(0, v, 0x114, 0xF, 0xF, true);
+  v += __builtin_amdgcn_update_dpp(0, v, 0x118, 0xF, 0xF, true);
+  v += __builtin_amdgcn_update_dpp(0, v, 0x142, 0xA, 0xF, false);
+  v += __builtin_amdgcn_update_dpp(0, v, 0x143, 0xC, 0xF, false);
+  return v;
+}
+__device__ __forceinline__ double wave_min_d(double v)
+{
+#pragma unroll
+  for (int d = 32; d >= 1; d >>= 1) { const double o = __shfl_xor(v, d, 64); v = (o < v) ? o : v; }
+  return v;
+}
+__device__ __forceinline__ unsigned long long wave_min_u64(unsigned long long v)
+{
+#pragma unroll
+  for (int d = 32; d >= 1; d >>= 1) { const unsigned long long o = __shfl_xor(v, d, 64); v = (o < v) ? o : v; }
+  return v;
+}
+__device__ __forceinline__ void clear_result(dsr_decode_result* r)
+{
+  int z = 0; asm volatile("" : "+v"(z));
+  int* p = reinterpret_cast<int*>(r);
+#pragma unroll 1
+  for (int i = 0; i < (int) (sizeof(dsr_decode_result) / 4); i++) p[i] = z;
+}
+__device__ __forceinline__ TokA ld_tok(const TokA* p)
+{
+  const unsigned long long a = reinterpret_cast<const volatile unsigned long long*>(p)[0], b = reinterpret_cast<const volatile unsigned long long*>(p)[1];
+  TokA t; t.ac = __uint_as_float((unsigned) (a & 0xFFFFFFFFull)); t.lm = __uint_as_float((unsigned) (a >> 32)); t.bp = (uint32_t) (b & 0xFFFFFFFFull); t.xs = (uint32_t) (b >> 32);
+  return t;
+}
+__device__ __forceinline__ unsigned f2ord(float f) { const unsigned u = __float_as_uint(f); return (u & 0x80000000u) ? ~u : (u | 0x80000000u); }
+
+#define TOKA(ix) ((EXTRA && (ix) == 2) ? ka->D.tokA3 + (size_t) slot * ka->D.maxTok : ka->D.tokA + ((size_t) slot * 2 + (size_t) (ix)) * ka->D.maxTok)
+#define TOKB(ix) ((EXTRA && (ix) == 2) ? ka->D.tokB3 + (size_t) slot * ka->D.maxTok : ka->D.tokB + ((size_t) slot * 2 + (size_t) (ix)) * ka->D.maxTok)
+#define curA TOKA(bufCur)
+#define nxtA TOKA(bufNxt)
+#define curB TOKB(bufCur)
+#define nxtB TOKB(bufNxt)
+#define sprA TOKA(bufSpr)
+#define sprB TOKB(bufSpr)
+#define cA (ka->D.cA + (size_t) slot * ka->D.maxCand)
+#define cB (ka->D.cB + (size_t) slot * ka->D.maxCand)
+#define arena (ka->D.arena + (size_t) ((EXTRA && ka->D.latOn) ? u : (ka->D.segFrames > 0 ? 0 : slot)) * ka->D.arenaCap)
+#define dump (EXTRA && ka->D.dumpOn && slot == 0)
+
+template <int NTHR, bool EXTRA, bool NARROW, bool TABLE>
+__device__ __forceinline__ bool vit_memory_frame(KP ka, const int slot, const int u, const int tid, const int mode, const int fr, const int T, const int segS,
+                                                 const int bufCur, const int bufNxt, const int n, const double threshM, const long arenaUsed,
+                                                 const int useLdsRow, const float* srow, const float* rowG, unsigned* hkey, const int hashN,
+                                                 int* s_waveTot, int* s_waveTotE, double* s_waveMin, unsigned* s_tag, long long* s_chunk, long long* s_latOff,
+                                                 int& status, long& arenaOff, long& chunkEnd, int& numNew, int& numStat, int& Cfr, double& topScore)
+{
+  constexpr int nthr = NTHR, nw = NTHR / 64;
+  const int lane = tid & 63, wave = tid >> 6;
+  unsigned* const hfirst = hkey + hashN; unsigned* const tab = hkey; const int tabN = NARROW ? 2 * hashN : hashN;
+  const int tableC = (tabN >> 1) + (tabN >> 2);
+  int* tokOff = ka->D.tokOff + (size_t) slot * (ka->D.maxTok + 1);
+  int* tokCnt = ka->D.tokCnt + (size_t) slot * (ka->D.maxTok + 1);
+  int* chead = ka->D.chead + (size_t) slot * ka->D.maxCand;
+  int* owner = ka->D.owner + (size_t) slot * ka->D.maxCand;
+  int* rank = ka->D.rank + (size_t) slot * ka->D.maxCand;
+  unsigned* first = ka->D.first + (size_t) slot * ka->G.nNodes;
+  unsigned tag = *s_tag;
+  __syncthreads();
+  if (tag <= 1u) { for (int i = tid; i < ka->G.nNodes; i += nthr) first[i] = 0xFFFFFFFFu; tag = 255u; __syncthreads(); } else tag--;
+  if (tid == 0) *s_tag = tag;
+  const unsigned tagw = tag << 24;
+  const int chunkT = ((n + nw * 64 - 1) / (nw * 64)) * 64;
+  {
+    int running = 0;
+    const int b0 = wave * chunkT, b1 = (b0 + chunkT < n) ? b0 + chunkT : n;
+    for (int base = b0; base < b1; base += 64) {
+      const int i = base + lane; int cnt = 0;
+      if (i < b1) {
+        const TokA ta = curA[i]; const TokB tb = curB[i];
+        if (mode == 0) {
+          const float s = __fadd_rn(ta.ac, ta.lm);
+          if (!((double) s > threshM)) cnt = tb.cnt;
+        } else cnt = (ka->G.nodeFinal[tb.node] ? 1 : 0) + (ka->G.eoff[tb.node + 1] - ka->G.eoff[tb.node]);
+      }
+      const int incl = wave_incl_scan(cnt, lane);
+      if (i < b1) { tokOff[i] = running + incl - cnt; tokCnt[i] = cnt; }
+      running += __shfl(incl, 63, 64);
+    }
+    if (lane == 0) s_waveTot[wave] = running;
+  }
+  __syncthreads();
+  int C = 0;
+  for (int w = 0; w < nw; w++) C += s_waveTot[w];
+  if (C > ka->D.maxCand) { status = DSR_E_ALLOCATION; return false; }
+  if (EXTRA && ka->D.latOn && *s_latOff + C > ka->D.latCap) { status = DSR_E_ALLOCATION; return false; }
+  Cfr = C;
+  const bool useHash = TABLE && hashN > 0 && C <= tableC;
+  for (int i = tid; i < n; i += nthr) {
+    const int cnt = tokCnt[i];
+    if (cnt == 0) continue;
+    const int w = i / chunkT; int base = 0;
+    for (int q = 0; q < w; q++) base += s_waveTot[q];
+    const int off = base + tokOff[i];
+    tokOff[i] = off;
+    for (int j = 0; j < cnt; j++) owner[off + j] = i;
+  }
+  __syncthreads();
+  double locMin = HUGE_VAL;
+  for (int c = tid; c < C; c += nthr) {
+    const int i = owner[c]; const TokA ta = curA[i]; const int nd = curB[i].node; const bool tokSil = (ta.xs >> 31) != 0u;
+    Tok t; t.node = nd; t.ac = ta.ac; t.lm = ta.lm; t.bp = ta.bp;
+    const int j = c - tokOff[i];
+    double ac = (double) t.ac, lm; int dst, recId; bool silArc = false;
+    if (mode == 0) {
+      recId = (int) (ta.xs & 0x7FFFFFFFu) + j; const XRec x = ka->G.xrec[recId];
+      const int plen = (int) (x.meta & 0xFFFFu);
+      double lmNode = (double) t.lm; uint32_t prevIn = tokSil ? ka->D.silenceX : (ka->D.silenceX + 1u);
+      bool prevNull = (t.bp == kNone) && (fr == 0);
+      if (plen) {
+        const int* pp = ka->G.path + ka->G.xpathOff[recId];
+        for (int h = 0; h < plen; h++) {
+          const int a = pp[h];
+          double l = __dadd_rn(lmNode, __dmul_rn(ka->D.lmScale, (double) ka->G.arcCost[a]));
+          if (ka->G.arcOut[a] != 0) l = __dadd_rn(l, __dmul_rn(ka->D.lmScale, ka->D.lmPenalty));
+          if (0u == ka->D.silenceX && (prevNull || prevIn != ka->D.silenceX)) l = __dadd_rn(l, __dmul_rn(ka->D.lmScale, ka->D.silPenalty));
+          lmNode = (double) (float) l; prevIn = 0u; prevNull = false;
+        }
+      }
+      lm = __dadd_rn(lmNode, __dmul_rn(ka->D.lmScale, (double) x.cost));
+      if (x.meta & 0x10000u) lm = __dadd_rn(lm, __dmul_rn(ka->D.lmScale, ka->D.lmPenalty));
+      if ((uint32_t) (x.dist + 1) == ka->D.silenceX && (prevNull || prevIn != ka->D.silenceX)) lm = __dadd_rn(lm, __dmul_rn(ka->D.lmScale, ka->D.silPenalty));
+      ac = __dadd_rn(ac, (double) (useLdsRow ? srow[x.dist] : rowG[x.dist]));
+      dst = x.dst; silArc = ((uint32_t) (x.dist + 1) == ka->D.silenceX);
+    } else {
+      const int hasSelf = ka->G.nodeFinal[nd] ? 1 : 0;
+      if (hasSelf && j == 0) {
+        const float lmf = (float) __dadd_rn((double) t.lm, __dmul_rn(ka->D.lmScale, (double) ka->G.nodeCost[nd]));
+        lm = (double) lmf; dst = nd; recId = (int) 0x7FFFFFFE;
+      } else {
+        recId = ka->G.eoff[nd] + (j - hasSelf); const ERec e = ka->G.erec[recId];
+        const int* pp = ka->G.path + e.pathOff; double lmNode = (double) t.lm; double l = lmNode;
+        uint32_t prevIn = tokSil ? ka->D.silenceX : (ka->D.silenceX + 1u);
+        for (int h = 0; h < e.pathLen; h++) {
+          const int a = pp[h];
+          l = __dadd_rn(lmNode, __dmul_rn(ka->D.lmScale, (double) ka->G.arcCost[a]));
+          if (ka->G.arcOut[a] != 0) l = __dadd_rn(l, __dmul_rn(ka->D.lmScale, ka->D.lmPenalty));
+          if (0u == ka->D.silenceX && prevIn != ka->D.silenceX) l = __dadd_rn(l, __dmul_rn(ka->D.lmScale, ka->D.silPenalty));
+          lmNode = (double) (float) l; prevIn = 0u;
+        }
+        lm = __dadd_rn(l, __dmul_rn(ka->D.lmScale, (double) ka->G.nodeCost[e.lastSrc]));
+        dst = e.dst; recId = (int) ((uint32_t) recId | kEndBit);
+      }
+    }
+    const double ttl = __dadd_rn(ac, lm);
+    CandA a2; a2.ttl = ttl; a2.ac = (float) ac; a2.lm = (float) lm; cA[c] = a2;
+    if (useHash) {
+      unsigned h = ((unsigned) dst * 2654435761u) >> 7 & (unsigned) (tabN - 1);
+      if (NARROW) {
+        const unsigned key = (unsigned) dst + 1u, w = (key << 15) | (unsigned) c;
+        for (;;) {
+          const unsigned k = atomicCAS(&tab[h], 0u, w);
+          if (k == 0u) break;
+          if ((k >> 15) == key) { atomicMin(&tab[h], w); break; }
+          h = (h + 1u) & (unsigned) (tabN - 1);
+        }
+      } else {
+        for (;;) {
+          const unsigned k = atomicCAS(&hkey[h], 0u, (unsigned) dst + 1u);
+          if (k == 0u || k == (unsigned) dst + 1u) break;
+          h = (h + 1u) & (unsigned) (hashN - 1);
+        }
+        atomicMin(&hfirst[h], (unsigned) c);
+      }
+      rank[c] = (int) h;
+    } else atomicMin(&first[dst], tagw | (unsigned) c);
+    chead[c] = -1;
+    if (silArc) recId |= 0x40000000;
+    CandB b2; b2.dst = dst; b2.next = -1; b2.rec = recId; b2.prevBp = t.bp; cB[c] = b2;
+    if (mode == 0 && ttl < locMin) locMin = ttl;
+  }
+  locMin = wave_min_d(locMin);
+  if (lane == 0) s_waveMin[wave] = locMin;
+  __syncthreads();
+  topScore = HUGE_VAL;
+  for (int w = 0; w < nw; w++) { const double v = s_waveMin[w]; if (v < topScore) topScore = v; }
+  for (int c = tid; c < C; c += nthr) {
+    int f;
+    if (useHash) f = NARROW ? (int) (tab[rank[c]] & 0x7FFFu) : (int) hfirst[rank[c]];
+    else { const int dst = cB[c].dst; f = (int) (ld_u32(&first[dst]) & 0x00FFFFFFu); }
+    if (f != c) { const int nx = atomicExch(&chead[f], c); cB[c].next = nx; chead[c] = -2; }
+  }
+  __syncthreads();
+  if (useHash) for (int i = tid; i < 2 * hashN; i += nthr) hkey[i] = (NARROW || i < hashN) ? 0u : 0xFFFFFFFFu;
+  const int chunkC = ((C + nw * 64 - 1) / (nw * 64)) * 64;
+  const double threshNextM = __dadd_rn(topScore, ka->D.beam);
+  const bool pruneM = !dump && mode == 0 && (fr + 1 < T) && !(EXTRA && ka->D.topN > 0);
+  {
+    int running = 0, runAll = 0;
+    const int b0 = wave * chunkC, b1 = (b0 + chunkC < C) ? b0 + chunkC : C;
+    for (int base = b0; base < b1; base += 64) {
+      const int c = base + lane; bool isFirst = false, isAny = false;
+      if (c < b1) {
+        const int h0 = ld_i32(&chead[c]);
+        isFirst = (h0 != -2);
+        if (isFirst) {
+          int w = c; CandA aw = cA[w];
+          double fw = (double) __fadd_rn(aw.ac, aw.lm);
+          for (;;) {
+            int best = 0x7FFFFFFF;
+            int steps = 0;
+            for (int p = h0; p >= 0 && steps <= C; p = cB[p].next, steps++) if (p > w && p < best && cA[p].ttl < fw) best = p;
+            if (best == 0x7FFFFFFF) break;
+            w = best; aw = cA[w]; fw = (double) __fadd_rn(aw.ac, aw.lm);
+          }
+          isAny = true;
+          if (pruneM && ((double) __fadd_rn(aw.ac, aw.lm) > threshNextM)) { isFirst = false; w = -3; }
+          chead[c] = w;
+        }
+      }
+      const unsigned long long bal = __ballot(isFirst);
+      if (isFirst) rank[c] = running + __popcll(bal & ((1ull << lane) - 1ull));
+      running += __popcll(bal); runAll += __popcll(__ballot(isAny));
+    }
+    if (lane == 0) { s_waveTot[wave] = running; s_waveTotE[wave] = runAll; }
+  }
+  __syncthreads();
+  numStat = 0;
+  for (int w = 0; w < nw; w++) { numNew += s_waveTot[w]; numStat += s_waveTotE[w]; }
+  if (numNew > ka->D.maxTok || (segS > 0 ? arenaUsed : arenaOff) + numNew > ka->D.arenaCap) { status = DSR_E_ALLOCATION; return false; }
+  if (segS > 0 && arenaOff + numNew > chunkEnd) {
+    const long need = numNew > ka->D.poolChunk ? (long) numNew : ka->D.poolChunk;
+    __syncthreads();
+    if (tid == 0) *s_chunk = (long long) atomicAdd(ka->D.poolNext, (unsigned long long) need);
+    __syncthreads();
+    arenaOff = (long) *s_chunk; chunkEnd = arenaOff + need;
+    if (chunkEnd > ka->D.poolCap) { status = DSR_E_ALLOCATION; return false; }
+  }
+  {
+    int wbase = 0; for (int q = 0; q < wave; q++) wbase += s_waveTot[q];
+    const int b0 = wave * chunkC, b1 = (b0 + chunkC < C) ? b0 + chunkC : C;
+    for (int base = b0; base < b1; base += 64) {
+      const int c = base + lane;
+      if (c < b1) {
+        const int w = chead[c];
+        if (w >= 0) {
+          const CandB bc = cB[c];
+          const int pos = numNew - 1 - (wbase + rank[c]);
+          const CandA aw = cA[w]; const CandB bw = (w == c) ? bc : cB[w]; const int recW = (bw.rec & 0x3FFFFFFF) | (bw.rec & (int) 0x80000000);
+          const int xo = ka->G.xoff[bc.dst];
+          TokA na; na.ac = aw.ac; na.lm = aw.lm; na.bp = (uint32_t) (arenaOff + pos); na.xs = (uint32_t) xo;
+          TokB nb; nb.node = bc.dst; nb.cnt = ka->G.xoff[bc.dst + 1] - xo;
+          Bp bp;
+          if (mode == 0) {
+            if (bw.rec & 0x40000000) na.xs |= 0x80000000u;
+            bp.prev = bw.prevBp; bp.rec = (uint32_t) recW;
+          } else {
+            if (bw.rec == (int) 0x7FFFFFFE) { if (segS > 0) { const unsigned long long v = ld_u64_dev(&arena[bw.prevBp]); bp.prev = (uint32_t) v; bp.rec = (uint32_t) (v >> 32); } else { const Bp o = arena[bw.prevBp]; bp = o; } }
+            else { bp.prev = bw.prevBp; bp.rec = (uint32_t) bw.rec; }
+          }
+          nxtA[pos] = na; nxtB[pos] = nb; arena[arenaOff + pos] = bp;
+          if (EXTRA && ka->D.latOn) ka->D.arenaLat[(size_t) u * ka->D.arenaCap + arenaOff + pos] = (int) (*s_latOff + w);
+        }
+      }
+    }
+  }
+  if (EXTRA && ka->D.latOn) {
+    uint4* lat = ka->D.lat + (size_t) u * ka->D.latCap; double* ltt = ka->D.latTtl + (size_t) u * ka->D.latCap;
+    const long latOff = (long) *s_latOff;
+    for (int c = tid; c < C; c += nthr) {
+      const CandA a = cA[c]; const CandB b = cB[c];
+      lat[latOff + c] = make_uint4(__float_as_uint(a.ac), __float_as_uint(a.lm), (unsigned) b.rec, b.prevBp); ltt[latOff + c] = a.ttl;
+    }
+    __syncthreads();
+    if (tid == 0) { *s_latOff = latOff + C; ka->D.latFrameOff[(size_t) u * (ka->Tmax + 3) + fr + 1] = latOff + C; }
+  }
+  return true;
+}
+
+template <int NTHR, bool EXTRA>
+__device__ __forceinline__ void vit_best_token(KP ka, const int slot, const int u, const int tid, const int bufCur, const int bufNxt, const int numNew, const int n,
+                                               const int T, const int Cfr, const long arenaOff, unsigned long long* s_waveKey, const long long* s_stat, const int* s_maxActive)
+{
+  constexpr int nthr = NTHR, nw = NTHR / 64;
+  const int lane = tid & 63, wave = tid >> 6;
+  const TokA* lst = numNew > 0 ? nxtA : curA; const int cntL = numNew > 0 ? numNew : n;
+  unsigned long long key = ~0ull;
+  for (int i = tid; i < cntL; i += nthr) {
+    const TokA t = lst[i]; const float s = __fadd_rn(t.ac, t.lm);
+    if (s == s) { const unsigned long long k = ((unsigned long long) f2ord(s) << 32) | (unsigned) i; if (k < key) key = k; }
+  }
+  key = wave_min_u64(key);
+  if (lane == 0) s_waveKey[wave] = key;
+  if (EXTRA && ka->D.latOn) {
+    const TokB* lstB = numNew > 0 ? nxtB : curB; int4* lf = ka->D.latFinal + (size_t) u * ka->D.maxTok;
+    for (int i = tid; i < cntL; i += nthr) { const TokA t = ld_tok(&lst[i]); lf[i] = make_int4(lstB[i].node, (int) t.bp, __float_as_int(t.ac), __float_as_int(t.lm)); }
+    if (tid == 0) { int* li = ka->D.latInfo + 4 * (size_t) u; li[0] = cntL; li[1] = numNew > 0 ? 1 : 0; li[2] = (int) (arenaOff + (numNew > 0 ? numNew : 0)); li[3] = T; }
+  }
+  __syncthreads();
+  if (tid == 0) {
+    dsr_decode_result* const res = ka->res;
+    clear_result(&res[u]); dsr_decode_result& r = res[u];
+    unsigned long long k = ~0ull; for (int w = 0; w < nw; w++) if (s_waveKey[w] < k) k = s_waveKey[w];
+    r.frames = T - 1; r.reachedFinal = numNew > 0 ? 1 : 0; r.finalStatesN = numNew;  r.activeHypos = (long) s_stat[0]; r.placements = (long) s_stat[1] + Cfr; r.registerFrames = (long) (s_stat[2] & 0xFFFFFFFFll); r.laidOutFrames_ = (int) (s_stat[2] >> 32); r.maxActiveSeen = *s_maxActive; r.status = DSR_OK;
+    TraceHead hd; hd.arenaOff = (unsigned long long) ((size_t) ((EXTRA && ka->D.latOn) ? u : (ka->D.segFrames > 0 ? 0 : slot)) * ka->D.arenaCap);  hd.bp = kNone; hd.hops = kNone;
+    if (k != ~0ull) {
+      const TokA bt = ld_tok(&lst[(unsigned) (k & 0xFFFFFFFFu)]);
+      r.ac = bt.ac; r.lm = bt.lm; r.score = __dadd_rn((double) bt.ac, (double) bt.lm);
+      hd.bp = bt.bp;
+      if (ka->walkHere) {
+        int* const hopRec = ka->hopRec + (size_t) u * ka->hopStride; const int walkCap = 2 * ka->D.maxCand < ka->hopStride ? 2 * ka->D.maxCand : ka->hopStride; int nH = 0;
+        for (uint32_t bq = bt.bp; bq != kNone && nH < walkCap; ) { const uint2 e = *reinterpret_cast<const uint2*>(&arena[bq]); hopRec[nH++] = (int) e.y; bq = e.x; }
+        hd.hops = (uint32_t) nH;
+      }
+    } else r.status = DSR_E_CONSISTENCY;
+    ka->heads[u] = hd;
+  }
+  __syncthreads();
+}
+
+__device__ __forceinline__ void vit_failed_result(KP ka, const int u, const int T, const int status)
+{
+  dsr_decode_result* const res = ka->res; clear_result(&res[u]); res[u].status = status; res[u].frames = T - 1;
+  TraceHead hd; hd.arenaOff = 0ull; hd.bp = kNone; hd.hops = kNone; ka->heads[u] = hd;
+}
+
+}
diff --git a/distantspeechrecognition-mirror_amd/csrc/viterbi_finish.hip b/distantspeechrecognition-mirror_amd/csrc/viterbi_finish.hip
--- /dev/null
+++ b/distantspeechrecognition-mirror_amd/csrc/viterbi_finish.hip
@@ -0,0 +1,48 @@
+#include "launch.h"
+#include "viterbi.h"
+#include "viterbi_end.h"
+
+namespace dsr {
+
+static constexpr int kFinishThreads = 256;
+
+__global__ __launch_bounds__(kFinishThreads) void k_finish(const VitArgs argsInKernarg)
+{
+  (void) argsInKernarg;
+  constexpr bool EXTRA = false;
+  constexpr int nthr = kFinishThreads, nw = kFinishThreads / 64;
+  const KP ka = (KP) __builtin_amdgcn_kernarg_segment_ptr();
+  __shared__ int s_waveTot[nw]; __shared__ int s_waveTotE[nw]; __shared__ double s_waveMin[nw]; __shared__ unsigned long long s_waveKey[nw];
+  __shared__ long long s_stat[3]; __shared__ int s_maxActive; __shared__ unsigned s_tag; __shared__ long long s_chunk; __shared__ long long s_latOff;
+  const int tid = threadIdx.x, slot = blockIdx.x;
+  const int bufCur = 0, bufNxt = 1;
+  if (tid == 0) { s_tag = ka->D.tags[slot]; s_latOff = 0; }
+  for (int u = slot; u < ka->U; u += (int) gridDim.x) {
+    __syncthreads();
+    const SegState* const sst = ka->D.segState + u;
+    if (sst->status != DSR_OK) continue;
+    const int T = ka->nframesArr[u] < ka->Tmax ? ka->nframesArr[u] : ka->Tmax;
+    const int n = sst->n; long arenaOff = sst->arenaOff, chunkEnd = sst->chunkEnd; const long arenaUsed = sst->arenaUsed;
+    if (n < 1 || n > ka->D.maxTok) { if (tid == 0) vit_failed_result(ka, u, T, DSR_E_CONSISTENCY); continue; }
+    if (tid == 0) { s_stat[0] = sst->stat[0]; s_stat[1] = sst->stat[1]; s_stat[2] = sst->stat[2]; s_maxActive = sst->maxActive; }
+    const TokA* const svA = ka->D.saveA + (size_t) u * ka->D.maxTok; const TokB* const svB = ka->D.saveB + (size_t) u * ka->D.maxTok;
+    for (int i = tid; i < n; i += nthr) { curA[i] = svA[i]; curB[i] = svB[i]; }
+    __syncthreads();
+    int status = DSR_OK, numNew = 0, numStat = -1, Cfr = 0; double topScore = HUGE_VAL;
+    const bool ok = vit_memory_frame<kFinishThreads, EXTRA, false, false>(ka, slot, u, tid, 1, T, T, ka->D.segFrames, bufCur, bufNxt, n, HUGE_VAL, arenaUsed, 0, nullptr, nullptr, nullptr, 0,
+                                                                          s_waveTot, s_waveTotE, s_waveMin, &s_tag, &s_chunk, &s_latOff, status, arenaOff, chunkEnd, numNew, numStat, Cfr, topScore);
+    __syncthreads();
+    if (ok) vit_best_token<kFinishThreads, EXTRA>(ka, slot, u, tid, bufCur, bufNxt, numNew, n, T, Cfr, arenaOff, s_waveKey, s_stat, &s_maxActive);
+    else if (tid == 0) vit_failed_result(ka, u, T, status);
+  }
+  __syncthreads();
+  if (tid == 0) ka->D.tags[slot] = s_tag;
+}
+
+void finish_launch(const VitArgs& A, int slots, hipStream_t st)
+{
+  if (A.U <= 0 || slots <= 0) return;
+  launch(k_finish, dim3(slots), dim3(kFinishThreads), 0, st, A);
+}
+
+}
```
